# microsoft/ConfigNet

Measured on AMD Instinct MI355X. Metric: train-step images/sec at 256x256 (G+D fwd+bwd), higher is better.
Workload: dtype f32; 1 GPU; ConfigNet second-stage iteration (D + synth-D + latent-D + G + EMA), 256x256, batch 16 per GPU, fp32, Keras-Adam; global_batch=16, resolution=256, latent_dim=145, parallelism=dp1, losses_finite=True

## Files before the change

### confignet_amd/_lib.py

```python
import ctypes
import os

_HERE = os.path.dirname(os.path.abspath(__file__))
LIB_PATH = os.environ.get("CN_LIB") or os.path.join(_HERE, "libconfignet_hip.so")


class CnSumJob(ctypes.Structure):
    _fields_ = [("src", ctypes.c_void_p), ("dst", ctypes.c_void_p), ("count", ctypes.c_longlong), ("parts", ctypes.c_int),
                ("accumulate", ctypes.c_int)]


class CnDepthJob(ctypes.Structure):
    _fields_ = [("a", ctypes.c_void_p), ("b", ctypes.c_void_p), ("c", ctypes.c_void_p), ("m", ctypes.c_int), ("n", ctypes.c_int),
                ("k", ctypes.c_int), ("lda", ctypes.c_int), ("ldb", ctypes.c_int), ("ldc", ctypes.c_int)]


class CnRowsJob(ctypes.Structure):
    _fields_ = [("a", ctypes.c_void_p), ("b", ctypes.c_void_p), ("c", ctypes.c_void_p), ("bias", ctypes.c_void_p), ("mask", ctypes.c_void_p)] + \
               [(n_, ctypes.c_int) for n_ in ("m", "n", "k", "lda", "ldb", "ldc", "tb", "act", "accumulate")] + [("slope", ctypes.c_float)]


class CnGanJob(ctypes.Structure):
    _fields_ = [("s", ctypes.c_void_p), ("out", ctypes.c_void_p), ("gout", ctypes.c_void_p), ("n", ctypes.c_int), ("label", ctypes.c_float)]


class CnConvGeom(ctypes.Structure):
    _fields_ = [(n, ctypes.c_int) for n in (
        "nd", "n", "in_d", "in_h", "in_w", "cin", "out_d", "out_h", "out_w", "cout",
        "k_d", "k_h", "k_w", "s_d", "s_h", "s_w", "dl_d", "dl_h", "dl_w", "p_d", "p_h", "p_w", "up")]


CN_F32, CN_BF16 = 0, 1
CN_U8 = 2
CN_EUNSUPPORTED = -3


class ConfigNetHipError(RuntimeError):
    pass


if not os.path.exists(LIB_PATH):
    raise ImportError(
        "confignet_amd: %s is missing -- build it with `python confignet_amd/build.py` "
        "(or __graft_entry__.build()).  There is no CPU/PyTorch fallback." % LIB_PATH)

lib = ctypes.CDLL(LIB_PATH)

_p = ctypes.c_void_p
_i = ctypes.c_int
_f = ctypes.c_float
_z = ctypes.c_size_t
_G = ctypes.POINTER(CnConvGeom)

SIGNATURES = {
    "cn_version": [],
    "cn_conv_fwd": [_G, _p, _p, _p, _p, _i, _f, _p],
    "cn_conv_fwd_res": [_G, _p, _p, _p, _p, _p, _i, _f, _p],
    "cn_conv_fwd_stats": [_G, _p, _p, _p, _p, _i, _f, _p, _i, _f, _p],
    "cn_scale_columns_segments": [_p, _p, _p, _p, _i, _z, _p],
    "cn_conv_weight_tflip": [_p, _p, _i, _i, _i, _p],
    "cn_conv_dgrad": [_G, _p, _p, _p, _p],
    "cn_conv_dgrad_w": [_G, _p, _p, _p, _p],
    "cn_conv_dgrad_w_res": [_G, _p, _p, _p, _p, _p],
    "cn_bn_fold_bwd_chunks": [],
    "cn_bn_fold_bwd": [_p, _i, _i, _p, _p, _p, _p, _p, _p, _p, _p, _i, _p],
    "cn_conv_wgrad_thin_partials": [],
    "cn_conv_wgrad_thin": [_G, _p, _p, _p, _p, _i, _p],
    "cn_conv_wgrad": [_G, _p, _p, _p, _i, _p],
    "cn_conv_wgrad_workspace_bytes": [_G],
    "cn_conv_wgrad_ws": [_G, _p, _p, _p, _i, _p, _z, _p],
    "cn_conv_wgrad_ws_slabs": [_G, _p, _p, _p, _i, _p, _z, ctypes.POINTER(_i), _p],
    "cn_conv_wgrad_dt_workspace_bytes": [_G, _i, _i, ctypes.POINTER(_z)],
    "cn_conv_wgrad_dt": [_G, _p, _i, _p, _i, _p, _i, _p, _z, ctypes.POINTER(_i), _p],
    "cn_conv_wgrad_plan": [_G, _i, _i, _i, ctypes.c_uint, _i, ctypes.POINTER(ctypes.c_longlong)],
    "cn_conv_wgrad_grouped": [_i, _p, _p, _p, _p, _p, _p, _p, _i, _p, _p],
    "cn_conv_wgrad_grouped_plan": [_i, _p, _i, _p, _p],
    "cn_sum_parts_grouped": [_p, _i, _p],
    "cn_gemm_depth_grouped": [_p, _i, _p],
    "cn_gan_loss_grouped": [_p, _i, _i, _p],
    "cn_gemm_rows_grouped": [_p, _i, _p],
    "cn_gemm_rows_grouped_k": [_p, _i, _p],
    "cn_gemm_rows_grouped_plan": [_p, _i, ctypes.POINTER(_i), _i, ctypes.POINTER(_i)],
    "cn_conv_tune": [_i, _i, ctypes.c_long],
    "cn_conv_fwd_plan": [_G, _i, _i, _i, _i, _i, _i, _i, ctypes.POINTER(ctypes.c_int * 8)],
    "cn_conv_loop_select": [_i, _i, _i, _i],
    "cn_fwd2_col_block": [_i, _i, _i, _i, _i, _i],
    "cn_conv_fwd_dt": [_p, _p, _i, _p, _p, _p, _i, _i, _f, _p],
    "cn_conv_dgrad_dt": [_p, _p, _i, _p, _p, _i, _p],
    "cn_conv_wgrad_c3_partials": [],
    "cn_conv_wgrad_c3": [_p, _p, _p, _i, _p, _p, _i, _p],
    "cn_conv_wino_filter": [_p, _p, _i, _i, _i, _p],
    "cn_conv_fwd_wino": [_i, _i, _i, _i, _i, _p, _p, _p, _p, _i, _f, _p],
    "cn_conv_fwd_wino4": [_i, _i, _i, _i, _i, _p, _p, _p, _p, _i, _f, _p],
    "cn_conv_fwd_wino4_ep": [_i, _i, _i, _i, _i, _p, _p, _p, _p, _i, _f, _i, _p, _p, _p, _p, _i, _f, _p],
    "cn_conv_wino4_filter": [_p, _p, _i, _i, _i, _p],
    "cn_sumpool2": [_p, _p, _i, _i, _i, _i, _i, _i, _i, _p],
    "cn_gemm": [_i, _i, _i, _i, _i, _p, _i, _p, _i, _p, _i, _p, _i, _f, _p],
    "cn_gemm_plan": [_i] * 10 + [ctypes.POINTER(ctypes.c_int * 9)],
    "cn_nc_reduce4": [_p, _p, _i, _i, _i, _f, _i, _i, _p],
    "cn_nc_reduce": [_p, _p, _p, _p, _i, _i, _i, _i, _f, _i, _p],
    "cn_nc_reduce_plan": [_i, _i, _i, _i, _i, _i, ctypes.POINTER(ctypes.c_int * 8)],
    "cn_nc_lin2": [_p, _p, _p, _p, _p, _p, _p, _p, _i, _i, _i, _i, _i, _f, _i, _p],
    "cn_nc_rows_plan": [ctypes.c_longlong, _i, _i, ctypes.POINTER(ctypes.c_int * 2)],
    "cn_norm_coef_fwd": [_i, _p, _p, _p, _p, _p, _p, _p, _p, _i, _i, _i, _f, _p, _i, _p],
    "cn_norm_coef_bwd": [_i, _p, _p, _p, _p, _p, _p, _p, _p, _p, _p, _i, _i, _i, _f, _p],
    "cn_dual_tail_coef_fwd": [_p] * 13 + [_i, _i, _i, _f, _i, _i, _p],
    "cn_dual_tail_coef_bwd": [_p] * 13 + [ctypes.POINTER(ctypes.c_void_p), _i, _i, _i, _f, _i, _i, _p],
    "cn_dual_tail_gx": [_p] * 12 + [_i, _i, _i, _f, _i, _i, _p],
    "cn_dual_tail_gx_tx": [_p] * 18 + [_i, _i, _i, _f, _i, _i, _i, _p],
    "cn_norm_apply": [_i, _i] + [_p] * 13 + [_i, _i, _i, _f, _i, _f, _i, _p],
    "cn_nc_reduce_hxt": [_p, _p, _p, _p, _i, _i, _i, _f, _i, _i, _i, _p],
    "cn_zero": [_p, ctypes.c_size_t, _p],
    "cn_set_deterministic": [_i],
    "cn_get_deterministic": [],
    "cn_det_release_stream": [_p],
    "cn_gemm_acc": [_i, _i, _i, _i, _i, _p, _i, _p, _i, _p, _i, _p],
    "cn_sum_rows_into": [_p, _p, _i, _i, _i, _p],
    "cn_bn_act_bwd": [_p, _p, _p, _p, _p, _p, _p, _p, _i, _i, _i, _i, _i, _i, _p],
    "cn_nc_reduce_dact": [_p, _p, _p, _p, _p, _i, _i, _i, _i, _f, _i, _i, _p],
    "cn_act_fwd": [_p, _p, _z, _i, _f, _i, _p],
    "cn_act_bwd": [_p, _p, _p, _z, _i, _f, _i, _p],
    "cn_act_bwd_bias": [_p, _p, _p, _p, _i, _i, _i, _i, _f, _i, _i, _p],
    "cn_axpby": [_p, _p, _p, _z, _f, _f, _i, _p],
    "cn_mul": [_p, _p, _p, _z, _i, _p],
    "cn_sqdiff_sum": [_p, _p, _p, _z, _f, _i, _p],
    "cn_row_sumsq": [_p, _p, _i, _z, _p],
    "cn_row_scale": [_p, _p, _p, _i, _z, _f, _i, _p],
    "cn_row_scale_diff": [_p, _p, _p, _p, _i, ctypes.c_size_t, _f, _i, _p],
    "cn_tap_bwd": [_p, _p, _p, _p, _p, _i, ctypes.c_size_t, _f, _i, _f, _i, _p],
    "cn_maxpool2_bwd_act": [_p, _p, _p, _p, _f, _p, _i, _i, _i, _i, _i, _i, _p],
    "cn_stream_plan": [_i, _i, ctypes.c_longlong, _z, _i, _i, _i, _i, _i, _i, ctypes.c_uint, _i, ctypes.POINTER(ctypes.c_longlong * 4)],
    "cn_stream_plan_ptrs": [_i, _i, _i, ctypes.c_longlong, _z, _i, _i, _i, _i, _i, _i, ctypes.POINTER(ctypes.c_void_p * 4), _i, ctypes.POINTER(ctypes.c_longlong * 4)],
    "cn_stream_last_plan": [ctypes.POINTER(ctypes.c_longlong * 5)],
    "cn_masked_diff": [_p, _p, _p, _p, _z, _i, _p],
    "cn_maxpool_fwd": [_p, _p, _i, _i, _i, _i, _i, _i, _i, _i, _p],
    "cn_maxpool_bwd": [_p, _p, _p, _i, _i, _i, _i, _i, _i, _i, _i, _p],
    "cn_avgpool3_same": [_p, _p, _i, _i, _i, _i, _i, _p],
    "cn_dwconv3x3_fwd": [_p, _p, _p, _p, _i, _i, _i, _i, _i, _i, _f, _p],
    "cn_image_preprocess": [_p, _i, _p, _i, _i, _i, _i, _i, _i, _f, _f, _p],
    "cn_dwconv3x3_dgrad": [_p, _p, _p, _i, _i, _i, _i, _i, _p],
    "cn_dwconv3x3_wgrad_slices": [_i, _i, _i, _i, _i],
    "cn_dwconv3x3_wgrad": [_p, _p, _p, _i, _i, _i, _i, _i, _i, _p],
    "cn_bn_train_coef": [_p] * 12 + [ctypes.c_longlong, _i, _f, ctypes.c_double, _i, _p],
    "cn_bn_train_apply": [_p, _p, _p, _p, ctypes.c_longlong, _i, _i, _p],
    "cn_bn_train_bwd_slices": [ctypes.c_longlong, _i],
    "cn_chan_slices_plan": [ctypes.c_longlong, _i, _i, ctypes.POINTER(ctypes.c_int * 5)],
    "cn_bn_train_bwd_reduce": [_p] * 6 + [_i, ctypes.c_longlong, _i, _i, _p],
    "cn_bn_train_bwd_apply": [_p] * 8 + [ctypes.c_longlong, _i, _i, _p],
    "cn_chan_affine3_fwd": [_p, _p, _z, ctypes.POINTER(_i), _f, ctypes.POINTER(_f), _p],
    "cn_chan_affine3_bwd": [_p, _p, _z, ctypes.POINTER(_i), _f, _p],
    "cn_gan_loss_fwd": [_p, _p, _i, _f, _p],
    "cn_gan_loss_bwd": [_p, _p, _p, _i, _f, _p],
    "cn_euler_matrix": [_p, _p, _i, _p],
    "cn_euler_matrix_bwd": [_p, _p, _p, _i, _p],
    "cn_rotate3d_fwd": [_p, _p, _p, _i, _i, _i, _p],
    "cn_rotate3d_bwd": [_p, _p, _p, _p, _p, _i, _i, _i, _p],
    "cn_rotate3d_bwd_plan": [_i, _i, _i, _i, ctypes.POINTER(ctypes.c_int * 4)],
    "cn_adam_step": [_p, _p, _p, _p, _p, _z, _p, _f, _f, _f, _f, _p],
    "cn_ema_step": [_p, _p, _z, _f, _p],
    "cn_gather_images_u8": [_p, _p, _p, _p, _i, _i, _i, _i, _p],
    "cn_to_uint8": [_p, _p, _z, _p],
    "cn_hdri_rows_v": [_p, _p, _p, _p, _i, _i, _i, _i, _i, _p],
    "cn_hdri_rows_h": [_p, _p, _p, _p, _p, _p, _p, _i, _i, _i, _i, _i, _i, _p],
    "cn_exp2m1": [_p, _p, _z, _p],
    "cn_warp_affine_u8": [_p] * 6 + [_i] * 6 + [_p],
    "cn_warp_nearest_f32": [_p] * 6 + [_i] * 6 + [_p],
    "cn_eye_mask": [_p, _p, _z, _i] + [_f] * 6 + [_p],
    "cn_spin": [ctypes.c_ulonglong, _p],
    "cn_conv_weight_prep_bf16": [_p, _p, _p, _i, _i, _i, _p],
    "cn_conv_fwd_bf16": [_G, _p, _p, _p, _p, _i, _f, _p],
    "cn_conv_dgrad_bf16": [_G, _p, _p, _p, _p],
    "cn_conv_wgrad_bf16": [_G, _p, _p, _p, _i, _p],
    "cn_cast": [_p, _i, _p, _i, _z, _p],
    "cn_upfold_weights": [_p, _p, _p, _i, ctypes.POINTER(_i), ctypes.POINTER(_i), _i, _i, ctypes.POINTER(_i), ctypes.POINTER(_i), _p],
    "cn_upfold_wgrad": [_p, _p, _i, ctypes.POINTER(_i), ctypes.POINTER(_i), _i, _i, _i, _p],
    "cn_prof_enable": [_i],
    "cn_prof_reset": [],
    "cn_prof_collect": [ctypes.POINTER(_i), ctypes.POINTER(ctypes.c_double), ctypes.POINTER(ctypes.c_double)],
    "cn_prof_collect_by_family": [ctypes.POINTER(_i), ctypes.POINTER(ctypes.c_double), ctypes.POINTER(ctypes.c_double), ctypes.POINTER(ctypes.c_double)],
}

for _name, _args in SIGNATURES.items():
    _fn = getattr(lib, _name)
    _fn.argtypes = _args
    _fn.restype = ctypes.c_int
lib.cn_conv_wgrad_workspace_bytes.restype = ctypes.c_size_t
lib.cn_last_error_string.argtypes = []
lib.cn_last_error_string.restype = ctypes.c_char_p


def check(code, what):
    if code != 0:
        raise ConfigNetHipError("%s failed (%d): %s" % (what, code, lib.cn_last_error_string().decode()))
```

### confignet_amd/csrc/common.h

```cpp
#pragma once
#include <hip/hip_runtime.h>
#include <stdint.h>
#include <stdio.h>
#include "../../include/confignet_hip.h"

void cn_set_error(const char* fmt, ...);

#define CN_CHECK_ARG(cond, ...)            \
    do {                                   \
        if (!(cond)) {                     \
            cn_set_error(__VA_ARGS__);     \
            return CN_EINVAL;              \
        }                                  \
    } while (0)

#define CN_HIP(expr)                                                              \
    do {                                                                          \
        hipError_t e__ = (expr);                                                  \
        if (e__ != hipSuccess) {                                                  \
            cn_set_error("%s failed: %s (%s:%d)", #expr, hipGetErrorString(e__), __FILE__, __LINE__); \
            return CN_EHIP;                                                       \
        }                                                                         \
    } while (0)

#define CN_LAUNCH_CHECK()                                                         \
    do {                                                                          \
        hipError_t e__ = hipGetLastError();                                       \
        if (e__ != hipSuccess) {                                                  \
            cn_set_error("kernel launch failed: %s (%s:%d)", hipGetErrorString(e__), __FILE__, __LINE__); \
            return CN_EHIP;                                                       \
        }                                                                         \
    } while (0)

int cn_zero_async(void* p, size_t bytes, hipStream_t s);

int cn_det();
float* cn_det_ws(hipStream_t s, size_t need_floats);
constexpr size_t CN_DET_WS_FLOATS = (size_t)16 << 20;
int cn_sum_parts(const float* src, float* dst, int parts, long count, int accumulate, float scale, hipStream_t s);

int cn_fwd2(const CnConvGeom* gp, int cfg, int bt, const float* A, const float* B, const float* bias, float* C, long M, int N, int K,
            int act, float slope, int splits, long part_stride, int par, hipStream_t s, const float* res, double x_elems, double w_elems,
            float* stats = nullptr, int stats_mode = 0, float stats_slope = 0.f, int srows = 1, int sper = 1);
void cn_fwd2_tune(int kb, int ns, int np);
void cn_fwd2_grid(int cfg, long M, int N, int par, int splits, int grid[3]);
int cn_igemm_fwd(int cfg, const CnConvGeom& g, bool vec, int par, int splits, const float* x, const float* w, const float* bias, float* y,
                 int act, float slope, hipStream_t s, int bt, long part_stride, const float* res);
void cn_igemm_fwd_grid(int cfg, const CnConvGeom& g, bool vec, int par, int splits, int grid[3]);
int cn_igemm_fwd_thin(const CnConvGeom& g, const float* x, const float* w, const float* bias, float* y, int act, float slope, hipStream_t s);
enum ConvRoute { CN_ROUTE_UP2K4_RGB = 0, CN_ROUTE_S2_IMAGE_DGRAD, CN_ROUTE_S1_IMAGE_DGRAD, CN_ROUTE_THIN_PAR_IGEMM, CN_ROUTE_THIN_COOP,
                 CN_ROUTE_THIN, CN_ROUTE_C3, CN_ROUTE_C7S2, CN_ROUTE_FWD2, CN_ROUTE_IGEMM, CN_ROUTE_UNSUPPORTED };
constexpr int CN_THIN_COOP_PX = 4;
void cn_small_conv(int route, unsigned grid_x, const CnConvGeom& g, bool vec, int par, const void* x, int x_dt, const float* w,
                   const float* bias, void* y, int y_dt, int act, float slope, hipStream_t s);
int cn_fwd2_bf16(const CnConvGeom& g, int cfg, int flip, const void* x, const void* wb, const float* bias, void* y, int act, float slope,
                 int par, hipStream_t s);

enum WgradRoute { CN_WG_C3 = 0, CN_WG_THIN, CN_WG_TINY, CN_WG_WGRAD2, CN_WG_IGEMM, CN_WG_BF16, CN_WG_NONE };
constexpr int CN_C3_WGRAD_TILE = 64, CN_C3_WGRAD_PARTS = 512;
constexpr int CN_THIN_WGRAD_TH = 8, CN_THIN_WGRAD_TW = 32, CN_THIN_WGRAD_PARTS = 512;
struct Wg2Plan {
    int cfg;
    long tiles_x, tiles_y, splits, rows;
};
bool cn_wgrad2_ok(const CnConvGeom& g);
Wg2Plan cn_wgrad2_plan(const CnConvGeom& g, int forced_cfg, long wg_target, bool group = false);
void cn_wgrad2(int cfg, int ns, const CnConvGeom& g, const float* x, const float* gy, float* out, long slab_stride, int rows, int tiles_x,
               int tiles_y, int splits, int accumulate, unsigned grid, hipStream_t s);
constexpr int CN_WG2_GROUP = 24, CN_KERNARG_BYTES = 4096;
struct Wg2Job {
    CnConvGeom g;
    int rows, tiles_x, tiles_y, nsplits, accumulate;
    const float* x;
    const float* gy;
    float* out;
    long slab_stride;
};
struct Wg2Jobs {
    Wg2Job job[CN_WG2_GROUP];
    int blk0[CN_WG2_GROUP + 1];
    int n;
};
static_assert(sizeof(Wg2Jobs) <= CN_KERNARG_BYTES, "the jobs of a grouped launch travel in its kernel arguments");
void cn_wgrad2_grouped(int cfg, const Wg2Jobs& J, unsigned grid, hipStream_t s);
void cn_igemm_wgrad(int cfg, const CnConvGeom& g, const float* x, const float* gy, float* gw, int rows, float* parts, int tx, int ty,
                    int splits, dim3 grid, hipStream_t s);
int cn_tiny_wgrad(const CnConvGeom& g, const float* x, const float* gy, float* gw, int blocks, float* parts, hipStream_t s);
void cn_bf16_wgrad(int cfg, const CnConvGeom& g, const void* x, const void* gy, float* gw, int rows, int tx, int ty, int splits, dim3 grid,
                   hipStream_t s);
int cn_c3_wgrad(const CnConvGeom& g, const float* x, const void* gy, int gy_dt, float* scratch, int tiles_x, int ntiles, int nparts,
                size_t lds, hipStream_t s);
void cn_c3_wgrad_reduce(const float* scratch, float* gw, int nparts, int count, int accumulate, hipStream_t s);
void cn_thin_wgrad(const CnConvGeom& g, const float* x, const float* gy, float* scratch, int nwg, size_t lds, int tiles_y, int tiles_x,
                   int ntiles, hipStream_t s);

enum { CN_FAM_FWD_128x128 = 0, CN_FAM_FWD_128x64, CN_FAM_FWD_64x64, CN_FAM_FWD_128x32, CN_FAM_FWD_128x96, CN_FAM_WGRAD_128x128,
       CN_FAM_WGRAD_128x96, CN_FAM_WGRAD_64x64, CN_FAM_WGRAD_128x32, CN_FAM_WINO, CN_FAM_C3_FWD, CN_FAM_S2_IMAGE_DGRAD,
       CN_FAM_THIN, CN_FAM_C3_WGRAD, CN_FAM_BF16_FWD, CN_FAM_BF16_WGRAD, CN_FAM_WGRAD_256x64, CN_FAM_WGRAD_SLAB_SUM };
void cn_prof_begin(hipStream_t s, double flops, double bytes = 0.0, int family = 31);
void cn_prof_end(hipStream_t s);

__device__ __forceinline__ void divmod_pos(int m, int d, int& q, int& r) {
    if ((d & (d - 1)) == 0) {
        q = m >> (__builtin_ctz(d));
        r = m & (d - 1);
    } else {
        q = m / d;
        r = m - q * d;
    }
}

__device__ __forceinline__ float cn_apply_act(float v, int act, float slope) {
    switch (act) {
        case CN_ACT_LRELU: return v > 0.f ? v : v * slope;
        case CN_ACT_RELU: return v > 0.f ? v : 0.f;
        case CN_ACT_TANH: return tanhf(v);
        default: break;
    }
    if (act == CN_ACT_RELU6) return fminf(fmaxf(v, 0.f), 6.f);
    if (act == CN_ACT_SIGMOID) return __fdividef(1.f, 1.f + __expf(-v));
    return v;
}

__device__ __forceinline__ float act_deriv(float o, int act, float slope) {
    if (act == CN_ACT_LRELU) return o > 0.f ? 1.f : slope;
    if (act == CN_ACT_RELU) return o > 0.f ? 1.f : 0.f;
    if (act == CN_ACT_TANH) return 1.f - o * o;
    return 1.f;
}

static inline int cn_cdiv(long a, long b) { return (int)((a + b - 1) / b); }

int cn_cu_count();
```

### confignet_amd/csrc/conv_dispatch.hip

```cpp
#include "common.h"

#include <algorithm>
#include <vector>

#include "mma_tile.h"
#include "conv_geom.h"

namespace {

int g_tune_cfg = -1;
int g_tune_splits = 0;
long g_tune_wg_blocks = 0;
int g_tune_wg2_ns = 0;
int g_fwd2_sel = -1;
constexpr int g_fwd2_min_nks = 1;
constexpr int g_fwd2_min_c = 48;

struct ConvReq {
    int bt, has_bias, act, has_res, stats_mode, x_dt, y_dt;
};

struct ConvPlan {
    int route = CN_ROUTE_UNSUPPORTED;
    int ret = CN_EUNSUPPORTED;
    int cfg = -1;
    int splits = 1, par = 0;
    bool vec = false;
    bool plain = false;
    int family = -1;
    int srows = 1, sper = 1;
    int grid[3] = {0, 0, 0};
};

int image_route(const CnConvGeom& g, const ConvReq& q) {
    const bool x32 = q.x_dt == CN_F32, y32 = q.y_dt == CN_F32, x16 = q.x_dt == CN_BF16, y16 = q.y_dt == CN_BF16;
    if (x32 && (y32 || y16) && !q.bt && g.nd == 2 && g.cin == 3 && g.dl_h == 1 && g.dl_w == 1 && !g.up && g.cout > 4 && g.cout <= 64) {
        if (g.k_h == 3 && g.k_w == 3 && g.s_h == g.s_w && (g.s_h == 1 || g.s_h == 2)) return CN_ROUTE_C3;
        if (g.k_h == 7 && g.k_w == 7 && g.s_h == 2 && g.s_w == 2 && !q.has_res) return CN_ROUTE_C7S2;
    }
    if (y32 && g.nd == 2 && g.k_h == 3 && g.k_w == 3 && g.s_h == 1 && g.s_w == 1 && !g.up && g.cout == 3 && !q.has_bias &&
        q.act == CN_ACT_NONE && g.p_h >= 0 && g.p_h <= 2 && g.p_w >= 0 && g.p_w <= 2) {
        if ((x32 || x16) && g.dl_h == 2 && g.dl_w == 2 && g.cin == 48 && g.out_h <= 2 * g.in_h && g.out_w <= 2 * g.in_w) return CN_ROUTE_S2_IMAGE_DGRAD;
        if (x32 && g.dl_h == 1 && g.dl_w == 1 && g.cin == 64) return CN_ROUTE_S1_IMAGE_DGRAD;
    }
    return CN_ROUTE_UNSUPPORTED;
}

ConvPlan plan_conv_fwd(const CnConvGeom& g, const ConvReq& q) {
    ConvPlan p;
    const long M = (long)g.n * g.out_d * g.out_h * g.out_w;
    const bool res = q.has_res != 0, stats = q.stats_mode != 0;
    const int bt = q.bt;
    auto small = [&p](int route, int family, long grid_x) {
        p.route = route;
        p.ret = CN_OK;
        p.family = family;
        p.grid[0] = (int)grid_x; p.grid[1] = p.grid[2] = 1;
        return p;
    };
    auto refuse = [&p](int code) {
        p.ret = code;
        return p;
    };
    const int img = image_route(g, q);
    const long img_grid = img == CN_ROUTE_S2_IMAGE_DGRAD ? (long)g.n * cn_cdiv(g.in_h, 8) * cn_cdiv(g.in_w, 32)
                                                         : (long)g.n * cn_cdiv(g.out_h, 8) * cn_cdiv(g.out_w, 32);
    const int img_family = img == CN_ROUTE_C3 || img == CN_ROUTE_C7S2 ? CN_FAM_C3_FWD : CN_FAM_S2_IMAGE_DGRAD;
    if (q.x_dt != CN_F32 || q.y_dt != CN_F32)
        return img != CN_ROUTE_UNSUPPORTED ? small(img, img_family, img_grid) : p;
    if ((res || stats) && (g.cout <= 4 || g.cin == 3 || g.cout % 4 != 0)) return p;
    if (stats && (bt || cn_det() || g.cin % BK != 0)) return p;
    if (bt && (g.cout <= 4 || g.cin % BK != 0 || g.cout % 4 != 0)) return p;
    if (g.cout <= 4) {
        p.vec = g.cin % 4 == 0;
        p.par = parity_ordered(g);
        const size_t lds = sizeof(float) * 4 * (size_t)g.k_d * g.k_h * g.k_w * g.cin;
        if (lds > 64 * 1024) {
            cn_set_error("thin conv: filter of %zu bytes does not fit the LDS stage", lds);
            return refuse(CN_EINVAL);
        }
        const int T = g.k_d * g.k_h * g.k_w, CL = g.cin / 4;
        const bool dl1 = g.dl_d * g.dl_h * g.dl_w == 1;
        if (g.nd == 2 && g.up == 1 && g.k_h == 4 && g.k_w == 4 && g.s_h == 1 && g.s_w == 1 && g.dl_h == 1 && g.dl_w == 1 &&
            g.cout == 3 && g.cin == 32 && g.p_h == 1 && g.p_w == 1 && g.out_h <= 2 * g.in_h && g.out_w <= 2 * g.in_w)
            return small(CN_ROUTE_UP2K4_RGB, CN_FAM_THIN, (long)g.n * cn_cdiv(g.in_h, 8) * cn_cdiv(g.in_w, 16));
        if (img != CN_ROUTE_UNSUPPORTED) return small(img, img_family, img_grid);
        if (p.par && g.cin % BK == 0 && q.act == CN_ACT_NONE && T <= CN_MAX_MASKED_TAPS) return small(CN_ROUTE_THIN_PAR_IGEMM, CN_FAM_FWD_128x32, cn_cdiv(M, 128));
        if (p.vec && g.cout == 3 && CL >= 5 && CL <= 16 && T <= 32 && (p.par || dl1) && g.dl_d * g.dl_h * g.dl_w <= 8)
            return small(CN_ROUTE_THIN_COOP, -1, cn_cdiv(M, (256 / (CL <= 8 ? 8 : 16)) * CN_THIN_COOP_PX));
        return small(CN_ROUTE_THIN, -1, cn_cdiv(M, 256));
    }
    if (img != CN_ROUTE_UNSUPPORTED) return small(img, img_family, img_grid);
    if (g.cout % 4 != 0) {
        cn_set_error("cout=%d: implicit-GEMM path needs cout %% 4 == 0", g.cout);
        return refuse(CN_EINVAL);
    }
    const bool vec = g.cin % BK == 0;
    if (vec && (long)g.k_d * g.k_h * g.k_w > CN_MAX_MASKED_TAPS) {
        cn_set_error("%d taps: the vectorised implicit-GEMM gather takes at most %d", g.k_d * g.k_h * g.k_w, CN_MAX_MASKED_TAPS);
        return refuse(CN_EUNSUPPORTED);
    }
    const int par = parity_ordered(g) && vec;
    const long t128 = (long)cn_cdiv(M, 128) * cn_cdiv(g.cout, 128);
    const long t128x64 = (long)cn_cdiv(M, 128) * cn_cdiv(g.cout, 64);
    int cfg;
    long tiles;
    if (g.cout <= 32) { cfg = 3; tiles = (long)cn_cdiv(M, 128) * cn_cdiv(g.cout, 32); }
    else if (g.cout > 64 && t128 >= 512) { cfg = 0; tiles = t128; }
    else if (t128x64 >= 512) { cfg = 1; tiles = t128x64; }
    else { cfg = 2; tiles = (long)cn_cdiv(M, 64) * cn_cdiv(g.cout, 64); }
    if (g.cout % 96 == 0 && g.cout % 128 != 0 &&
        (long)cn_cdiv(M, 128) * (g.cout / 96) >= (g.cout == 96 ? 256 : 384)) {
        cfg = 4;
        tiles = (long)cn_cdiv(M, 128) * (g.cout / 96);
    }
    int splits = 1;
    const bool par_small = par && cfg == 2;
    const long nks_total = vec ? (long)g.k_d * g.k_h * g.k_w * (g.cin / BK) : 0;
    if (cfg == 0 && vec && !par && nks_total <= 8) { cfg = 1; tiles = t128x64; }
    const bool short_full = !par && tiles >= 256 && nks_total < 64;
    if (vec && tiles < (par_small ? 1024 : 512) && !short_full) {
        long nks = nks_total;
        if (par) nks /= (long)g.dl_d * g.dl_h * g.dl_w;
        long want = ((par_small ? 3072 : 1024) + tiles - 1) / tiles;
        if (want > 16) want = 16;
        const long min_steps = par_small ? 8 : 16;
        if (want > nks / min_steps) want = nks / min_steps;
        if (want > 1) splits = (int)want;
    }
    const bool n32 = g.cout == 32 && g.cin >= 32;
    const bool fwd2_takes = g_fwd2_sel != 0 && vec && nks_total > g_fwd2_min_nks && ((g.cin >= g_fwd2_min_c && g.cout >= g_fwd2_min_c) || n32) &&
                            g.dl_d <= 2 && g.dl_h <= 2 && g.dl_w <= 2 && (double)g.n * g.in_d * g.in_h * g.in_w * g.cin < 5.3e8 &&
                            (double)g.k_d * g.k_h * g.k_w * g.cin * g.cout < 5.3e8;
    if (fwd2_takes) {
        const int T = g.k_d * g.k_h * g.k_w;
        const long Me = (par && T == 1) ? M / ((long)g.dl_d * g.dl_h * g.dl_w) : M;
        long nks = nks_total;
        if (par) nks /= (long)g.dl_d * g.dl_h * g.dl_w;
        splits = 1;
        const bool par_balanced = par && g.k_d % g.dl_d == 0 && g.k_h % g.dl_h == 0 && g.k_w % g.dl_w == 0;
        if (n32) {
            cfg = 3;
            tiles = cn_cdiv(M, 128);
        } else if (par && T > 1 && !par_balanced) {
            cfg = 2;
            tiles = (long)cn_cdiv(M, 64) * cn_cdiv(g.cout, 64);
            if (g.cout % 96 == 0 && g.cout % 64 != 0 && (long)cn_cdiv(M, 128) * (g.cout / 96) >= 512) {
                cfg = 4;
                tiles = (long)cn_cdiv(M, 128) * (g.cout / 96);
            }
            if (cfg == 2 && tiles < 1024) {
                long want = (1536 + tiles / 2) / tiles;
                if (want > 16) want = 16;
                if (want > nks / 8) want = nks / 8;
                if (want > 1) splits = (int)want;
            }
        } else {
            struct Cand { int cfg, bm, bn; double step_us; };
            const Cand cands[2] = {{2, 64, 64, 0.265}, {4, 128, 96, 0.68}};
            double best = 0.0;
            bool have = false;
            for (const Cand& c : cands) {
                if (c.cfg == 4 && (g.cout % 96 != 0 || g.cout % 64 == 0 || (long)cn_cdiv(Me, 128) * (g.cout / 96) < 256)) continue;
                const long tl = (long)cn_cdiv(Me, c.bm) * cn_cdiv(g.cout, c.bn);
                const long smax = nks / 8 > 1 ? (nks / 8 > 16 ? 16 : nks / 8) : 1;
                for (long s_ = 1; s_ <= smax; ++s_) {
                    const double waves = (double)cn_cdiv(tl * s_, cn_cu_count());
                    double t = 10.0 + waves * (double)cn_cdiv(nks, s_) * c.step_us * (waves == 1.0 ? 1.06 : 1.0);
                    if (s_ > 1) t += 9.0 + (double)s_ * (double)M * g.cout * 4.0 / 6.0e6;
                    if (s_ > 1 && (res || stats)) t += 5.0 + 2.0 * (double)M * g.cout * 4.0 / 3.0e6;
                    if (!have || t < best) { have = true; best = t; cfg = c.cfg; tiles = tl; splits = (int)s_; }
                }
            }
        }
    }
    if (g_tune_cfg >= 0) cfg = g_tune_cfg;
    if (g_tune_splits > 0) splits = g_tune_splits;
    if (res && splits > 1) return p;
    if (stats) {
        const int qd = par ? g.out_d / g.dl_d : g.out_d, qh = par ? g.out_h / g.dl_h : g.out_h, qw = par ? g.out_w / g.dl_w : g.out_w;
        p.srows = qd * qh * qw;
        p.sper = par ? g.n * p.srows : (int)M;
        if (!fwd2_takes || splits > 1 || cfg == 3 || p.srows % (cfg == 2 ? 64 : 128) != 0) return p;
    }
    if (cn_det() && splits > 1) {
        const long cap = (long)(CN_DET_WS_FLOATS / ((size_t)M * g.cout));
        if (splits > cap) splits = (int)cap;
        if (splits <= 1 || !vec) splits = 1;
    }
    p.route = fwd2_takes && (cfg != 3 || n32) && cfg >= 0 && cfg <= 4 ? CN_ROUTE_FWD2 : CN_ROUTE_IGEMM;
    if (stats && p.route != CN_ROUTE_FWD2) return refuse(CN_EINVAL);
    p.ret = CN_OK;
    p.cfg = cfg;
    p.splits = splits;
    p.par = par;
    p.vec = vec;
    p.family = cfg == 0 ? CN_FAM_FWD_128x128 : cfg == 1 ? CN_FAM_FWD_128x64 : cfg == 3 ? CN_FAM_FWD_128x32 : cfg == 4 ? CN_FAM_FWD_128x96 : CN_FAM_FWD_64x64;
    if (p.route == CN_ROUTE_FWD2) {
        p.plain = !par && g.k_d * g.k_h * g.k_w == 1 && g.s_d == 1 && g.s_h == 1 && g.s_w == 1 && g.dl_d == 1 && g.dl_h == 1 &&
                  g.dl_w == 1 && !g.up && g.p_d == 0 && g.p_h == 0 && g.p_w == 0 && g.out_d == g.in_d && g.out_h == g.in_h &&
                  g.out_w == g.in_w;
        cn_fwd2_grid(cfg, M, g.cout, par, splits, p.grid);
    } else {
        cn_igemm_fwd_grid(cfg, g, vec, par, splits, p.grid);
    }
    return p;
}

int run_conv_fwd(const ConvPlan& p, const CnConvGeom& g, const ConvReq& q, const void* x, const float* w, const float* bias,
                 const float* res, void* y, float slope, float* stats, float stats_slope, hipStream_t s) {
    if (p.route == CN_ROUTE_UNSUPPORTED) return p.ret;
    const long M = (long)g.n * g.out_d * g.out_h * g.out_w;
    const int splits = p.splits;
    float* parts = nullptr;
    if (cn_det() && splits > 1) {
        parts = cn_det_ws(s, (size_t)splits * M * g.cout);
        if (!parts) return CN_EINVAL;
    }
    const int kact = splits > 1 ? CN_ACT_NONE : q.act;
    if (splits > 1 && !parts) {
        if (int ez__ = cn_zero_async(y, sizeof(float) * M * g.cout, s)) return ez__;
    }
    const long part_stride = parts ? (long)M * g.cout : 0;
    float* const out = parts ? parts : (float*)y;
    if (p.family >= 0) cn_prof_begin(s, conv_flops(g), conv_bytes(g, q.x_dt == CN_BF16 ? 2.0 : 4.0, q.y_dt == CN_BF16 ? 2.0 : 4.0), p.family);
    int e = CN_OK;
    switch (p.route) {
        case CN_ROUTE_FWD2: {
            const double xe = (double)g.n * g.in_d * g.in_h * g.in_w * g.cin, we = (double)g.k_d * g.k_h * g.k_w * g.cin * g.cout;
            e = cn_fwd2(p.plain ? nullptr : &g, p.cfg, q.bt, (const float*)x, w, bias, out, M, g.cout, g.cin, kact, slope, splits, part_stride,
                        p.plain ? 0 : p.par, s, res, xe, we, stats, q.stats_mode, stats_slope, p.srows, p.sper);
            break;
        }
        case CN_ROUTE_IGEMM:
            e = cn_igemm_fwd(p.cfg, g, p.vec, p.par, splits, (const float*)x, w, bias, out, kact, slope, s, q.bt, part_stride, res);
            break;
        case CN_ROUTE_THIN_PAR_IGEMM:
            e = cn_igemm_fwd_thin(g, (const float*)x, w, bias, out, kact, slope, s);
            break;
        default:
            cn_small_conv(p.route, (unsigned)p.grid[0], g, p.vec, p.par, x, q.x_dt, w, bias, y, q.y_dt, kact, slope, s);
            break;
    }
    if (p.family >= 0) cn_prof_end(s);
    CN_CHECK_ARG(e != CN_EUNSUPPORTED, "convolution plan (route %d, tile %d) refused by its kernel", p.route, p.cfg);
    if (e != CN_OK) return e;
    CN_LAUNCH_CHECK();
    if (parts) e = cn_sum_parts(parts, (float*)y, splits, (long)M * g.cout, 0, 1.f, s);
    if (e == CN_OK && splits > 1 && q.act != CN_ACT_NONE) e = cn_act_fwd(y, y, (size_t)M * g.cout, q.act, slope, CN_F32, s);
    return e;
}

int conv_fwd(const CnConvGeom* gp, const ConvReq& q, const void* x, const float* w, const float* bias, const float* res, void* y,
             float slope, float* stats, float stats_slope, void* stream) {
    if (int e = check_geom(gp)) return e;
    CN_CHECK_ARG(x && w && y, "NULL tensor");
    return run_conv_fwd(plan_conv_fwd(*gp, q), *gp, q, x, w, bias, res, y, slope, stats, stats_slope, (hipStream_t)stream);
}

}

extern "C" int cn_conv_fwd(const CnConvGeom* gp, const float* x, const float* w, const float* bias, float* y, int act,
                           float slope, void* stream) {
    return conv_fwd(gp, ConvReq{0, bias != nullptr, act, 0, 0, CN_F32, CN_F32}, x, w, bias, nullptr, y, slope, nullptr, 0.f, stream);
}

extern "C" int cn_conv_fwd_stats(const CnConvGeom* gp, const float* x, const float* w, const float* bias, float* y, int act,
                                 float slope, float* stats, int stats_mode, float stats_slope, void* stream) {
    CN_CHECK_ARG(stats && (stats_mode == 1 || stats_mode == 2), "cn_conv_fwd_stats: stats buffer and mode 1 / 2");
    CN_CHECK_ARG(stats_mode == 1 || act == CN_ACT_NONE, "cn_conv_fwd_stats: mode 2 takes the statistics of the pre-activation output");
    return conv_fwd(gp, ConvReq{0, bias != nullptr, act, 0, stats_mode, CN_F32, CN_F32}, x, w, bias, nullptr, y, slope, stats, stats_slope, stream);
}

extern "C" int cn_conv_fwd_res(const CnConvGeom* gp, const float* x, const float* w, const float* bias, const float* res, float* y,
                               int act, float slope, void* stream) {
    CN_CHECK_ARG(res, "cn_conv_fwd_res: res is NULL");
    return conv_fwd(gp, ConvReq{0, bias != nullptr, act, 1, 0, CN_F32, CN_F32}, x, w, bias, res, y, slope, nullptr, 0.f, stream);
}

extern "C" int cn_conv_fwd_dt(const CnConvGeom* gp, const void* x, int x_dt, const float* w, const float* bias, void* y, int y_dt,
                              int act, float slope, void* stream) {
    if (int e = check_geom(gp)) return e;
    CN_CHECK_ARG(x && w && y, "NULL tensor");
    if (x_dt == CN_F32 && y_dt == CN_F32) return CN_EUNSUPPORTED;
    const ConvReq q{0, bias != nullptr, act, 0, 0, x_dt, y_dt};
    return run_conv_fwd(plan_conv_fwd(*gp, q), *gp, q, x, w, bias, nullptr, y, slope, nullptr, 0.f, (hipStream_t)stream);
}

extern "C" int cn_conv_dgrad(const CnConvGeom* gp, const float* gy, const float* w_tflip, float* gu, void* stream) {
    if (int e = check_geom(gp)) return e;
    CN_CHECK_ARG(gp->dl_d == 1 && gp->dl_h == 1 && gp->dl_w == 1, "dgrad of a dilated-input geometry is not defined here");
    const CnConvGeom d = dgrad_geom(*gp);
    return cn_conv_fwd(&d, gy, w_tflip, nullptr, gu, CN_ACT_NONE, 0.f, stream);
}

extern "C" int cn_conv_dgrad_dt(const CnConvGeom* gp, const void* gy, int gy_dt, const float* w_tflip, void* gu, int gu_dt,
                                void* stream) {
    if (int e = check_geom(gp)) return e;
    if (gp->dl_d != 1 || gp->dl_h != 1 || gp->dl_w != 1) return CN_EUNSUPPORTED;
    const CnConvGeom d = dgrad_geom(*gp);
    return cn_conv_fwd_dt(&d, gy, gy_dt, w_tflip, nullptr, gu, gu_dt, CN_ACT_NONE, 0.f, stream);
}

extern "C" int cn_conv_dgrad_w(const CnConvGeom* gp, const float* gy, const float* w, float* gu, void* stream) {
    if (int e = check_geom(gp)) return e;
    if (gp->dl_d != 1 || gp->dl_h != 1 || gp->dl_w != 1) return CN_EUNSUPPORTED;
    const CnConvGeom d = dgrad_geom(*gp);
    return conv_fwd(&d, ConvReq{1, 0, CN_ACT_NONE, 0, 0, CN_F32, CN_F32}, gy, w, nullptr, nullptr, gu, 0.f, nullptr, 0.f, stream);
}

extern "C" int cn_conv_dgrad_w_res(const CnConvGeom* gp, const float* gy, const float* w, const float* res, float* gu, void* stream) {
    if (int e = check_geom(gp)) return e;
    CN_CHECK_ARG(res, "cn_conv_dgrad_w_res: res is NULL");
    if (gp->dl_d != 1 || gp->dl_h != 1 || gp->dl_w != 1 || gp->up) return CN_EUNSUPPORTED;
    if (gp->s_d != 1 || gp->s_h != 1 || gp->s_w != 1) return CN_EUNSUPPORTED;
    const CnConvGeom d = dgrad_geom(*gp);
    return conv_fwd(&d, ConvReq{1, 0, CN_ACT_NONE, 1, 0, CN_F32, CN_F32}, gy, w, nullptr, res, gu, 0.f, nullptr, 0.f, stream);
}

extern "C" int cn_conv_fwd_plan(const CnConvGeom* gp, int bt, int has_bias, int act, int has_res, int stats_mode, int x_dt, int y_dt,
                                int out[8]) {
    if (int e = check_geom(gp)) return e;
    CN_CHECK_ARG(out, "cn_conv_fwd_plan: out is NULL");
    const ConvPlan p = plan_conv_fwd(*gp, ConvReq{bt, has_bias, act, has_res, stats_mode, x_dt, y_dt});
    const int v[8] = {p.route, p.cfg, p.splits, p.par, p.family, p.grid[0], p.grid[1], p.grid[2]};
    for (int i = 0; i < 8; ++i) out[i] = v[i];
    return p.ret;
}

namespace {

struct WgradReq {
    int x_dt, gy_dt;
    bool caller_slabs;
    unsigned routes;
    bool det = cn_det() != 0;
};
constexpr unsigned wg_bit(int r) { return 1u << r; }
constexpr unsigned WG_ATOMIC = wg_bit(CN_WG_TINY) | wg_bit(CN_WG_IGEMM), WG_FP32_GEMM = wg_bit(CN_WG_WGRAD2) | WG_ATOMIC, WG_ALL = ~0u;

enum { WG_SUM_NONE = 0, WG_SUM_PARTS, WG_SUM_C3, WG_SUM_CALLER };

struct WgradPlan {
    int route = CN_WG_NONE;
    int ret = CN_EUNSUPPORTED;
    int cfg = -1;
    int stages = 0;
    long splits = 1, rows = 0;
    int tx = 0, ty = 0;
    int family = -1;
    int grid[3] = {0, 0, 0};
    size_t lds = 0;
    size_t ws_floats = 0;
    size_t det_floats = 0;
    bool zero = false;
    int sum = WG_SUM_NONE;
};

struct WgTile { int bm, bn; };
WgTile wgrad_tile(int cfg) { return cfg == 3 ? WgTile{128, 32} : cfg == 4 ? WgTile{128, 96} : cfg == 0 ? WgTile{128, 128} : cfg == 5 ? WgTile{256, 64} : WgTile{64, 64}; }
int wgrad_family(int cfg) {
    return cfg == 3 ? CN_FAM_WGRAD_128x32 : cfg == 4 ? CN_FAM_WGRAD_128x96 : cfg == 0 ? CN_FAM_WGRAD_128x128 : cfg == 5 ? CN_FAM_WGRAD_256x64 : CN_FAM_WGRAD_64x64;
}

void sliced_grid(const CnConvGeom& g, WgTile t, WgradPlan& p) {
    const long Ktot = (long)g.k_d * g.k_h * g.k_w * g.cin;
    const int gx = cn_cdiv(Ktot, t.bm), gy = cn_cdiv(g.cout, t.bn);
    p.grid[0] = gx; p.grid[1] = gy; p.grid[2] = (int)p.splits;
    if ((long)gx * gy > 1 && p.splits >= 16) {
        p.tx = gx; p.ty = gy;
        p.grid[0] = cn_cdiv(p.splits, 8) * 8 * gx * gy; p.grid[1] = p.grid[2] = 1;
    }
}

bool igemm_wgrad_slices(const CnConvGeom& g, WgTile t, long wg_target, bool det, WgradPlan& p) {
    const long M = (long)g.n * g.out_d * g.out_h * g.out_w;
    const long Ktot = (long)g.k_d * g.k_h * g.k_w * g.cin;
    const long tiles = (long)cn_cdiv(Ktot, t.bm) * cn_cdiv(g.cout, t.bn);
    const long wg_blocks = wg_target > 0 ? wg_target : 2048;
    long splits = (wg_blocks + tiles - 1) / tiles;
    if (det) {
        const long cap = (long)(CN_DET_WS_FLOATS / ((size_t)Ktot * g.cout));
        if (cap < 1) {
            cn_set_error("deterministic filter gradient: %ld x %d filter does not fit the workspace", Ktot, g.cout);
            return false;
        }
        if (splits > cap) splits = cap;
    }
    long rows = (M + splits - 1) / splits;
    if (rows < 256) rows = 256;
    rows = (rows + BK - 1) / BK * BK;
    p.rows = rows;
    p.splits = (M + rows - 1) / rows;
    return true;
}

void bf16_wgrad_slices(const CnConvGeom& g, WgTile t, WgradPlan& p) {
    constexpr long KS = 32, min_rows = 512;
    const long M = (long)g.n * g.out_d * g.out_h * g.out_w;
    const long Ktot = (long)g.k_d * g.k_h * g.k_w * g.cin;
    const long tiles = (long)cn_cdiv(Ktot, t.bm) * cn_cdiv(g.cout, t.bn);
    const long per_cu = t.bm * t.bn >= 128 * 128 ? 3 : t.bm * t.bn >= 128 * 96 ? 4 : 5;
    const long target = 256 * per_cu * (t.bn >= 96 ? 1 : 2);
    long splits = target / tiles;
    if (splits > M / min_rows) splits = M / min_rows;
    const long fill = std::min<long>(M / 256, (256 + tiles - 1) / tiles);
    if (splits < fill) splits = fill;
    if (splits >= 16) splits &= ~7L;
    if (splits < 1) splits = 1;
    long rows = (M + splits - 1) / splits;
    if (rows < 256) rows = std::min<long>(256, (M + KS - 1) / KS * KS);
    rows = (rows + KS - 1) / KS * KS;
    p.rows = rows;
    p.splits = (M + rows - 1) / rows;
}

WgradPlan plan_conv_wgrad(const CnConvGeom& g, const WgradReq& q) {
    WgradPlan p;
    const long M = (long)g.n * g.out_d * g.out_h * g.out_w;
    const long Ktot = (long)g.k_d * g.k_h * g.k_w * g.cin;
    const size_t count = (size_t)Ktot * g.cout;
    const bool x32 = q.x_dt == CN_F32, y32 = q.gy_dt == CN_F32, x16 = q.x_dt == CN_BF16, y16 = q.gy_dt == CN_BF16;
    auto may = [&q](int route) { return (q.routes & wg_bit(route)) != 0; };
    auto take = [&p](int route, int family) {
        p.route = route;
        p.ret = CN_OK;
        p.family = family;
    };
    if (may(CN_WG_C3) && x32 && (y32 || y16) && g.nd == 2 && g.cin == 3 && g.k_h == 3 && g.k_w == 3 && g.k_d == 1 && g.s_h == g.s_w &&
        (g.s_h == 1 || g.s_h == 2) && g.dl_h == 1 && g.dl_w == 1 && g.up == 0 && g.cout <= 64 && g.cout >= 4 && g.cout % 4 == 0) {
        take(CN_WG_C3, CN_FAM_C3_WGRAD);
        p.tx = cn_cdiv(g.out_w, CN_C3_WGRAD_TILE);
        p.grid[0] = CN_C3_WGRAD_PARTS; p.grid[1] = p.grid[2] = 1;
        const int pw = CN_C3_WGRAD_TILE * g.s_h + 2, gpitch = (g.cout + 3) & ~3;
        p.lds = sizeof(float) * 4 * (size_t)(3 * pw * 3 + CN_C3_WGRAD_TILE * gpitch);
        if (p.lds < sizeof(float) * 4 * 2 * 16 * 64) p.lds = sizeof(float) * 4 * 2 * 16 * 64;
        p.ws_floats = CN_C3_WGRAD_PARTS * count;
        p.sum = WG_SUM_C3;
        return p;
    }
    const int T = g.k_h * g.k_w;
    if (may(CN_WG_THIN) && x32 && y32 && g.nd == 2 && g.cout <= 4 && g.cin % 4 == 0 && g.cin >= 8 && g.cin <= 64 && g.s_h == 1 && g.s_w == 1 &&
        g.dl_h == 1 && g.dl_w == 1 && T <= 16 && T * (g.cin / 4) <= 256) {
        const int PH0 = ((CN_THIN_WGRAD_TH + g.k_h - 1) >> g.up) + 2, PW0 = ((CN_THIN_WGRAD_TW + g.k_w - 1) >> g.up) + 2;
        size_t lds = sizeof(float) * ((size_t)PH0 * PW0 * g.cin + CN_THIN_WGRAD_TH * CN_THIN_WGRAD_TW * 4);
        const size_t red = sizeof(float) * 256 * 4 * g.cout;
        if (lds < red) lds = red;
        if (lds <= 64 * 1024) {
            take(CN_WG_THIN, -1);
            p.ty = cn_cdiv(g.out_h, CN_THIN_WGRAD_TH); p.tx = cn_cdiv(g.out_w, CN_THIN_WGRAD_TW);
            const int ntiles = g.n * p.ty * p.tx;
            p.grid[0] = ntiles < CN_THIN_WGRAD_PARTS ? ntiles : CN_THIN_WGRAD_PARTS; p.grid[1] = p.grid[2] = 1;
            p.lds = lds;
            p.ws_floats = CN_THIN_WGRAD_PARTS * count;
            p.sum = WG_SUM_PARTS;
            return p;
        }
    }
    if (x16 && y16) {
        if (!may(CN_WG_BF16) || g.cin % 8 || g.cout % 8) return p;
        take(CN_WG_BF16, CN_FAM_BF16_WGRAD);
        p.cfg = wgrad_tile_cfg(g);
        bf16_wgrad_slices(g, wgrad_tile(p.cfg), p);
        sliced_grid(g, wgrad_tile(p.cfg), p);
        p.zero = true;
        return p;
    }
    if (!x32 || !y32) return p;
    if (may(CN_WG_WGRAD2) && cn_wgrad2_ok(g) && Ktot >= 64) {
        const int t = g_tune_cfg;
        const Wg2Plan w = cn_wgrad2_plan(g, t == 0 || t == 2 || t == 3 || t == 4 || t == 5 ? t : -1, g_tune_wg_blocks);
        take(CN_WG_WGRAD2, wgrad_family(w.cfg));
        p.cfg = w.cfg;
        p.stages = w.cfg == 3 || g_tune_wg2_ns == 3 ? 3 : 4;
        p.splits = w.splits; p.rows = w.rows;
        p.tx = (int)w.tiles_x; p.ty = (int)w.tiles_y;
        p.grid[0] = (int)((w.splits >= 8 ? cn_cdiv(w.splits, 8) * 8 : w.splits) * w.tiles_x * w.tiles_y); p.grid[1] = p.grid[2] = 1;
        if (w.splits > 1) {
            p.ws_floats = (size_t)w.splits * count;
            p.sum = q.caller_slabs ? WG_SUM_CALLER : WG_SUM_PARTS;
        }
        return p;
    }
    if (may(CN_WG_TINY) && Ktot <= 4 && g.cout <= 4 && g.k_d * g.k_h * g.k_w == 1 && g.s_h == 1 && g.s_w == 1 && g.s_d == 1 && !g.up &&
        g.p_h == 0 && g.p_w == 0 && g.p_d == 0) {
        take(CN_WG_TINY, -1);
        p.grid[0] = cn_cdiv(M, 256) > 1024 ? 1024 : cn_cdiv(M, 256); p.grid[1] = p.grid[2] = 1;
        p.zero = true;
        if (q.det) {
            p.det_floats = (size_t)p.grid[0] * 16;
            p.sum = WG_SUM_PARTS;
        }
        return p;
    }
    if (!may(CN_WG_IGEMM)) return p;
    const int cfg = wgrad_tile_cfg(g);
    if (!igemm_wgrad_slices(g, wgrad_tile(cfg), g_tune_wg_blocks, q.det, p)) {
        p.ret = CN_EINVAL;
        return p;
    }
    take(CN_WG_IGEMM, wgrad_family(cfg));
    p.cfg = cfg;
    sliced_grid(g, wgrad_tile(cfg), p);
    p.zero = true;
    if (q.det) {
        p.det_floats = (size_t)p.splits * count;
        p.sum = WG_SUM_PARTS;
    }
    return p;
}

int sum_conv_wgrad(const WgradPlan& p, int nparts, long count, int mode, float* gw, const float* ws, const float* det, int* parts_out,
                   hipStream_t s) {
    CN_LAUNCH_CHECK();
    const int add = mode != CN_WGRAD_WRITE;
    if (p.sum == WG_SUM_PARTS) return cn_sum_parts(det ? det : ws, gw, nparts, count, det ? 1 : add, 1.f, s);
    if (p.sum == WG_SUM_C3) {
        cn_c3_wgrad_reduce(ws, gw, nparts, (int)count, mode == CN_WGRAD_ADD, s);
        CN_LAUNCH_CHECK();
    }
    if (p.sum == WG_SUM_CALLER) *parts_out = nparts;
    return CN_OK;
}

int run_conv_wgrad(const WgradPlan& p, const CnConvGeom& g, const WgradReq& q, const void* x, const void* gy, float* gw, int mode,
                   float* ws, size_t ws_bytes, int* parts_out, hipStream_t s) {
    if (parts_out) *parts_out = 0;
    if (p.route == CN_WG_NONE) return p.ret;
    CN_CHECK_ARG(mode == CN_WGRAD_WRITE || mode == CN_WGRAD_ADD || mode == CN_WGRAD_ZEROED, "filter gradient: mode %d", mode);
    CN_CHECK_ARG(p.ws_floats == 0 || (ws && ws_bytes >= sizeof(float) * p.ws_floats), "filter gradient: workspace of %zu bytes, %zu needed",
                 ws ? ws_bytes : (size_t)0, sizeof(float) * p.ws_floats);
    CN_CHECK_ARG(p.sum != WG_SUM_CALLER || parts_out, "filter gradient: slabs left to a caller that takes none");
    CN_CHECK_ARG(p.route != CN_WG_BF16 || (((uintptr_t)x | (uintptr_t)gy) & 15) == 0, "bf16 convolution needs 16-byte aligned tensors");
    const long count = (long)g.k_d * g.k_h * g.k_w * g.cin * g.cout;
    const int add = mode != CN_WGRAD_WRITE;
    float* det = nullptr;
    if (p.det_floats) {
        det = cn_det_ws(s, p.det_floats);
        if (!det) return CN_EINVAL;
    }
    if (p.zero && !add) {
        if (int ez__ = cn_zero_async(gw, sizeof(float) * count, s)) return ez__;
    }
    if (p.family >= 0)
        cn_prof_begin(s, p.route == CN_WG_C3 ? 2.0 * 27.0 * g.cout * (double)g.n * g.out_h * g.out_w : conv_flops(g),
                      conv_bytes(g, q.x_dt == CN_BF16 ? 2.0 : 4.0, q.gy_dt == CN_BF16 ? 2.0 : 4.0, 4.0), p.family);
    const dim3 grid(p.grid[0], p.grid[1], p.grid[2]);
    int nparts = (int)p.splits, e = CN_OK;
    switch (p.route) {
        case CN_WG_C3:
            e = cn_c3_wgrad(g, (const float*)x, gy, q.gy_dt, ws, p.tx, g.n * g.out_h * p.tx, nparts = p.grid[0], p.lds, s);
            break;
        case CN_WG_THIN:
            cn_thin_wgrad(g, (const float*)x, (const float*)gy, ws, nparts = p.grid[0], p.lds, p.ty, p.tx, g.n * p.ty * p.tx, s);
            break;
        case CN_WG_TINY:
            nparts = cn_tiny_wgrad(g, (const float*)x, (const float*)gy, gw, p.grid[0], det, s);
            break;
        case CN_WG_WGRAD2:
            cn_wgrad2(p.cfg, p.stages, g, (const float*)x, (const float*)gy, p.splits > 1 ? ws : gw, p.splits > 1 ? count : 0, (int)p.rows,
                      p.tx, p.ty, (int)p.splits, add, grid.x, s);
            break;
        case CN_WG_IGEMM:
            cn_igemm_wgrad(p.cfg, g, (const float*)x, (const float*)gy, gw, (int)p.rows, det, p.tx, p.ty, (int)p.splits, grid, s);
            break;
        default:
            cn_bf16_wgrad(p.cfg, g, x, gy, gw, (int)p.rows, p.tx, p.ty, (int)p.splits, grid, s);
            break;
    }
    const bool sum_in_bracket = p.route != CN_WG_C3;
    if (p.family >= 0 && !sum_in_bracket) cn_prof_end(s);
    if (e == CN_OK) e = sum_conv_wgrad(p, nparts, count, mode, gw, ws, det, parts_out, s);
    if (p.family >= 0 && sum_in_bracket) cn_prof_end(s);
    return e;
}

int conv_wgrad(const CnConvGeom* gp, const WgradReq& q, const void* x, const void* gy, float* gw, int mode, void* ws, size_t ws_bytes,
               int* parts, void* stream) {
    if (int e = check_geom(gp)) return e;
    CN_CHECK_ARG(x && gy && gw, "NULL tensor");
    return run_conv_wgrad(plan_conv_wgrad(*gp, q), *gp, q, x, gy, gw, mode, (float*)ws, ws_bytes, parts, (hipStream_t)stream);
}

}

extern "C" int cn_conv_wgrad(const CnConvGeom* gp, const float* x, const float* gy, float* gw, int accumulate, void* stream) {
    return conv_wgrad(gp, WgradReq{CN_F32, CN_F32, false, WG_ATOMIC}, x, gy, gw, accumulate ? CN_WGRAD_ADD : CN_WGRAD_WRITE, nullptr, 0, nullptr, stream);
}

extern "C" size_t cn_conv_wgrad_workspace_bytes(const CnConvGeom* gp) {
    if (!gp || check_geom(gp) != CN_OK) return 0;
    return sizeof(float) * plan_conv_wgrad(*gp, WgradReq{CN_F32, CN_F32, false, WG_FP32_GEMM}).ws_floats;
}

extern "C" int cn_conv_wgrad_ws(const CnConvGeom* gp, const float* x, const float* gy, float* gw, int accumulate, void* workspace,
                                size_t workspace_bytes, void* stream) {
    return conv_wgrad(gp, WgradReq{CN_F32, CN_F32, false, WG_FP32_GEMM}, x, gy, gw, accumulate ? CN_WGRAD_ADD : CN_WGRAD_WRITE, workspace,
                      workspace_bytes, nullptr, stream);
}

extern "C" int cn_conv_wgrad_ws_slabs(const CnConvGeom* gp, const float* x, const float* gy, float* gw, int accumulate, void* workspace,
                                      size_t workspace_bytes, int* parts, void* stream) {
    CN_CHECK_ARG(parts, "cn_conv_wgrad_ws_slabs: parts is NULL");
    return conv_wgrad(gp, WgradReq{CN_F32, CN_F32, true, WG_FP32_GEMM}, x, gy, gw, accumulate ? CN_WGRAD_ADD : CN_WGRAD_WRITE, workspace,
                      workspace_bytes, parts, stream);
}

extern "C" int cn_conv_wgrad_bf16(const CnConvGeom* gp, const uint16_t* x, const uint16_t* gy, float* gw, int accumulate,
                                  void* stream) {
    return conv_wgrad(gp, WgradReq{CN_BF16, CN_BF16, false, wg_bit(CN_WG_BF16)}, x, gy, gw, accumulate ? CN_WGRAD_ADD : CN_WGRAD_WRITE, nullptr, 0,
                      nullptr, stream);
}

extern "C" int cn_conv_wgrad_c3_partials(void) { return CN_C3_WGRAD_PARTS; }

extern "C" int cn_conv_wgrad_c3(const CnConvGeom* gp, const float* x, const void* gy, int gy_dt, float* scratch, float* gw,
                                int accumulate, void* stream) {
    CN_CHECK_ARG(gp && x && gy && scratch && gw && (gy_dt == CN_F32 || gy_dt == CN_BF16), "conv_wgrad_c3: bad args");
    return conv_wgrad(gp, WgradReq{CN_F32, gy_dt, false, wg_bit(CN_WG_C3)}, x, gy, gw, accumulate ? CN_WGRAD_ADD : CN_WGRAD_WRITE, scratch, SIZE_MAX,
                      nullptr, stream);
}

extern "C" int cn_conv_wgrad_thin_partials(void) { return CN_THIN_WGRAD_PARTS; }

extern "C" int cn_conv_wgrad_thin(const CnConvGeom* gp, const float* x, const float* gy, float* scratch, float* gw, int accumulate,
                                  void* stream) {
    CN_CHECK_ARG(scratch, "conv_wgrad_thin: NULL");
// ... 184 lines not shown
```

### confignet_amd/csrc/fwd2.hip

```cpp
#include "common.h"
#include "mma_tile.h"
#include "conv_geom.h"
#include "typed.h"

#ifndef FWD2_ABLATE
#define FWD2_ABLATE 0
#endif

namespace {

typedef __attribute__((address_space(3))) float lds_float;
typedef float f4 __attribute__((ext_vector_type(4)));
typedef float f2 __attribute__((ext_vector_type(2)));
typedef __bf16 f2_bf16x8 __attribute__((ext_vector_type(8)));

template <int N>
__device__ __forceinline__ void f2_wait_vmcnt() {
    __builtin_amdgcn_s_waitcnt((N & 15) | ((N >> 4) << 14) | (7 << 4) | (15 << 8));
}

template <int N>
__device__ __forceinline__ void f2_wait_lgkm() {
    asm volatile("s_waitcnt lgkmcnt(%0)" : : "n"(N));
    __builtin_amdgcn_sched_barrier(0);
}

template <int N>
struct F2Int {
    static constexpr int value = N;
};

template <int I, int N, class F>
__device__ __forceinline__ void f2_static_for_impl(F&& f) {
    if constexpr (I < N) {
        f(F2Int<I>{});
        f2_static_for_impl<I + 1, N>(f);
    }
}

template <int N, class F>
__device__ __forceinline__ void f2_static_for(F&& f) {
    f2_static_for_impl<0, N>(f);
}

template <int WM, int WN, int TM, int TN, bool BT, bool GATHER, int KB, int NS, int NP, bool BF, int CB = 32>
__device__ __forceinline__ void fwd2_body(const CnConvGeom& g, const float* __restrict__ A, const float* __restrict__ B,
                                          const float* __restrict__ bias, float* __restrict__ C, int M, int N, int K,
                                          int act, float slope, int ntm, int ntn, long part_stride, int par,
                                          const float* __restrict__ res, unsigned a_bytes, unsigned b_bytes, int flip,
                                          float* __restrict__ stats, int stats_mode, float stats_slope, int srows, int sper) {
    static_assert(!BF || BT, "bf16: both operands are K-contiguous rows");
    constexpr int ES = BF ? 2 : 4;
    constexpr int KE = KB * 4 / ES;
    static_assert(WM * WN == 4, "4 waves per workgroup");
    static_assert(KB == 16 || KB == 32, "stage depth");
    static_assert(CB == 32 || (CB == 16 && BT && !BF && KB == 16 && NP == 0), "16-wide MFMA blocks: the fp32 B^T form");
    constexpr int KP = KB / 4;
    constexpr int RPI = 64 / KP;
    constexpr int FSH = KP == 4 ? 2 : 1;
    constexpr int G = CB == 16 ? 1 : KB / 8;
    constexpr int BM = CB * WM * TM, BN = CB * WN * TN;
    constexpr int NL = NP > 0 ? NP : 4;
    constexpr int IA = BM / RPI, JA = IA / NL;
    static_assert(IA % NL == 0, "A pieces divide over the loading waves");
    static_assert(NP == 0 || KB == 16, "loader waves: 16-deep stages");
    constexpr int IB = BT ? BN / RPI : KB * BN / 256;
    constexpr int JB = (IB + NL - 1) / NL;
    constexpr int LPW = JA + JB;
    constexpr int SA = BM * KB, SB = CB == 16 ? IB * 256 : JB * NL * 256;
    constexpr int SX = CB == 16 && IB < JB * NL ? 256 : 0;
    constexpr bool B2 = !BT && TN == 1 && BN == 64;
    constexpr int NB = BT ? TN : B2 ? 2 : 4 * (TN == 2 ? 1 : TN);
    constexpr int RD = TM + NB;
    static_assert((NS - 1) * LPW < 64, "vmcnt range");
    __shared__ __attribute__((aligned(1024))) float SM[NS * (SA + SB) + SX];
    __shared__ int rowmap[GATHER ? BM : 1];

    const int tid = threadIdx.x, lane = tid & 63, l31 = lane & (CB - 1), half = lane / CB;
    const int wave = __builtin_amdgcn_readfirstlane(tid >> 6);
    const bool loader = NP == 0 || wave >= 4, worker = wave < 4;
    const int lw = NP > 0 ? wave - 4 : wave;
    const int wm = (wave & 3) / WN, wn = (wave & 3) % WN;
    int bx, by;
    if (GATHER && par) {
        divmod_pos((int)blockIdx.x, ntm, by, bx);
        if (by >= ntn) return;
    } else {
        const int id = blockIdx.x, xcd = id & 7, j = id >> 3;
        const int nt = ntm * ntn, q = nt >> 3, r = nt & 7;
        if (j >= q + (xcd < r ? 1 : 0)) return;
        const int u = (xcd < r ? xcd * (q + 1) : r * (q + 1) + (xcd - r) * q) + j;
        divmod_pos(u, ntn, bx, by);
    }
    const int m0 = bx * BM, n0 = by * BN;
    const int T = GATHER ? g.k_d * g.k_h * g.k_w : 1;
    const int cpb = K / KE;
    unsigned long long tapmask = T >= 64 ? ~0ull : ((1ull << T) - 1ull);
    if (GATHER && par) {
        int c0, c1;
        par_row(g, m0, M, c0);
        par_row(g, min(m0 + BM, M) - 1, M, c1);
        if (c0 == c1) tapmask = par_tap_mask(g, c0);
    }
    const int nks_all = (GATHER ? __popcll(tapmask) : 1) * cpb;
    const int per_z = (nks_all + gridDim.z - 1) / gridDim.z;
    const int ks_beg = blockIdx.z * per_z, ks_end = min(nks_all, ks_beg + per_z);
    const int nks = max(ks_end - ks_beg, 0);

    constexpr int AR = CB == 16 ? 4 : 16;
    typedef float acc_t __attribute__((ext_vector_type(AR)));
    acc_t acc[TM][TN];
#pragma unroll
    for (int i = 0; i < TM; ++i)
#pragma unroll
        for (int j = 0; j < TN; ++j)
#pragma unroll
            for (int r = 0; r < AR; ++r) acc[i][j][r] = 0.f;

    const __amdgpu_buffer_rsrc_t ares = __builtin_amdgcn_make_buffer_rsrc(const_cast<float*>(A), 0, (int)a_bytes, 0x00020000);
    const __amdgpu_buffer_rsrc_t bres = __builtin_amdgcn_make_buffer_rsrc(const_cast<float*>(B), 0, (int)b_bytes, 0x00020000);
    constexpr unsigned OOB = 0x80000000u;

    RowInfo ri[JA];
    int a_base[JA];
    const int a_piece = 16 * ((lane % KP) ^ ((((lw & 1) * RPI + lane / KP) >> FSH) & (KP - 1)));
#pragma unroll
    for (int j = 0; j < JA; ++j) {
        const int r = (lw + NL * j) * RPI + lane / KP;
        if (!loader) {
            ri[j] = RowInfo{};
            a_base[j] = -1;
        } else if (GATHER) {
            int mrow = m0 + r, cls;
            if (par) mrow = par_row(g, mrow, M, cls);
            ri[j] = decode_row(g, mrow, M);
            if (lane % KP == 0) rowmap[r] = ri[j].ok ? mrow : -1;
            a_base[j] = -1;
        } else {
            a_base[j] = m0 + r < M ? (m0 + r) * K : -1;
        }
    }
    int b_off[JB];
    int b_krow[JB];
#pragma unroll
    for (int j = 0; j < JB; ++j) {
        const int I = lw + NL * j;
        if (BT) {
            const int n = n0 + I * RPI + lane / KP;
            b_off[j] = (I < IB && n < N) ? n * K * ES + a_piece : -1;
            b_krow[j] = 0;
        } else {
            const int idx = I * 64 + lane, col = n0 + 4 * (idx % (BN / 4));
            b_krow[j] = idx / (BN / 4);
            b_off[j] = (I < IB && col < N) ? col : -1;
        }
    }
    if (GATHER) __syncthreads();

    int ld_left = nks;
    int ld_tap = -1, ld_c0 = (ks_beg - (ks_beg / cpb) * cpb) * KE;
    if (GATHER)
        for (int o = ks_beg / cpb; o >= 0; --o) ld_tap += __ffsll((long long)(tapmask >> (ld_tap + 1)));
    else
        ld_tap = 0;
    unsigned a_vo[JA], b_vo[JB];
    int a_so = 0, b_so = 0;
    const int sh_d = g.dl_d - 1, sh_h = g.dl_h - 1, sh_w = g.dl_w - 1;
    const int ext_d = g.in_d << g.up, ext_h = g.in_h << g.up, ext_w = g.in_w << g.up;
    auto retap = [&]() __attribute__((always_inline)) {
        if (GATHER) {
            int kd, kh, kw;
            tap_decode(g, ld_tap, kd, kh, kw);
#pragma unroll
            for (int j = 0; j < JA; ++j) {
                const int vd = ri[j].vd + kd, vh = ri[j].vh + kh, vw = ri[j].vw + kw;
                const int qd = vd >> sh_d, qh = vh >> sh_h, qw = vw >> sh_w;
                const bool ok = ri[j].ok & ((vd | vh | vw) >= 0) & (((vd & sh_d) | (vh & sh_h) | (vw & sh_w)) == 0) &
                                (qd < ext_d) & (qh < ext_h) & (qw < ext_w);
                const int off = (((ri[j].nbase + (qd >> g.up)) * g.in_h + (qh >> g.up)) * g.in_w + (qw >> g.up)) * g.cin;
                a_vo[j] = ok ? (unsigned)(off * ES + a_piece) : OOB;
            }
        }
    };
    auto set_so = [&]() __attribute__((always_inline)) {
        a_so = ld_c0 * ES;
        b_so = BT ? ((flip ? T - 1 - ld_tap : ld_tap) * N * K + ld_c0) * ES : (ld_tap * K + ld_c0) * N * 4;
    };
#pragma unroll
    for (int j = 0; j < JA; ++j) a_vo[j] = (!GATHER && a_base[j] >= 0) ? (unsigned)(a_base[j] * ES + a_piece) : OOB;
#pragma unroll
    for (int j = 0; j < JB; ++j) b_vo[j] = b_off[j] >= 0 ? (BT ? (unsigned)b_off[j] : (unsigned)(b_krow[j] * N + b_off[j]) * 4u) : OOB;
    retap();
    set_so();
    auto issue_piece = [&](int stage, int p) __attribute__((always_inline)) {
        if (p < JA)
            __builtin_amdgcn_raw_ptr_buffer_load_lds(ares, (lds_float*)(SM + stage * SA + (lw + NL * p) * 256), 16, a_vo[p], a_so, 0, 0);
        else if (CB == 16 && lw + NL * (p - JA) >= IB)
            __builtin_amdgcn_raw_ptr_buffer_load_lds(bres, (lds_float*)(SM + NS * (SA + SB)), 16, b_vo[p - JA], b_so, 0, 0);
        else
            __builtin_amdgcn_raw_ptr_buffer_load_lds(bres, (lds_float*)(SM + NS * SA + stage * SB + (lw + NL * (p - JA)) * 256), 16,
                                                     b_vo[p - JA], b_so, 0, 0);
    };
    auto advance = [&]() __attribute__((always_inline)) {
        if (--ld_left > 0) {
            ld_c0 += KE;
            if (ld_c0 == K) {
                ld_c0 = 0;
                if (GATHER) {
                    ld_tap += __ffsll((long long)(tapmask >> (ld_tap + 1)));
                    retap();
                }
            }
            set_so();
        }
    };

    const unsigned lds0 = (unsigned)(unsigned long long)(lds_float*)SM;
    const unsigned fsw = (unsigned)((l31 >> FSH) & (KP - 1));
    const unsigned a_rd = lds0 + 4u * (unsigned)((wm * CB * TM + l31) * KB) + 16u * ((unsigned)half ^ fsw);
    const unsigned bt_rd = lds0 + 4u * (unsigned)(NS * SA + (wn * CB * TN + l31) * KB) + 16u * ((unsigned)half ^ fsw);
    const unsigned bn_rd = lds0 + 4u * (unsigned)(NS * SA + (4 * half) * BN + wn * 32 * TN + TN * l31);
    f4 av[2][TM];
    f4 btv[2][BT ? TN : 1];
    float bnv[2][BT ? 1 : 4][TN];
    unsigned ap_cur = 0, bp_cur = 0;
    auto read_base = [&](int stage, int gq) __attribute__((always_inline)) {
        ap_cur = (a_rd + 4u * (unsigned)(stage * SA)) ^ (32u * (unsigned)gq);
        bp_cur = BT ? (bt_rd + 4u * (unsigned)(stage * SB)) ^ (32u * (unsigned)gq) : bn_rd + 4u * (unsigned)(stage * SB + 8 * gq * BN);
    };
    auto read_op = [&](auto rc, int set) __attribute__((always_inline)) {
        constexpr int r = decltype(rc)::value;
        (void)av; (void)btv; (void)bnv; (void)ap_cur; (void)bp_cur;
        if (FWD2_ABLATE & 4) return;
        if constexpr (r < TM) {
            asm volatile("ds_read_b128 %0, %1 offset:%2" : "=v"(av[set][r]) : "v"(ap_cur), "n"(4 * CB * KB * r));
        } else if constexpr (BT) {
            constexpr int j = r - TM;
            asm volatile("ds_read_b128 %0, %1 offset:%2" : "=v"(btv[set][BT ? j : 0]) : "v"(bp_cur), "n"(4 * CB * KB * j));
        } else if constexpr (B2) {
            constexpr int q = 2 * (r - TM);
            f2 v;
            asm volatile("ds_read2_b32 %0, %1 offset0:%2 offset1:%3" : "=v"(v) : "v"(bp_cur), "n"(BN * q), "n"(BN * (q + 1)));
            bnv[set][BT ? 0 : q][0] = v.x;
            bnv[set][BT ? 0 : q + 1][0] = v.y;
        } else if constexpr (TN == 2) {
            constexpr int q = r - TM;
            f2 v;
            asm volatile("ds_read_b64 %0, %1 offset:%2" : "=v"(v) : "v"(bp_cur), "n"(4 * BN * q));
            bnv[set][BT ? 0 : q][0] = v.x;
            bnv[set][BT ? 0 : q][TN - 1] = v.y;
        } else {
            constexpr int q = (r - TM) / TN, j = (r - TM) % TN;
            asm volatile("ds_read_b32 %0, %1 offset:%2" : "=v"(bnv[set][BT ? 0 : q][j]) : "v"(bp_cur), "n"(4 * BN * q + 4 * j));
        }
    };
    constexpr int NM = (BF ? 1 : 4) * TM * TN;
    auto mfma_one = [&](auto mc, int set) __attribute__((always_inline)) {
        constexpr int m = decltype(mc)::value, q = m / (TM * TN), i = (m % (TM * TN)) / TN, j = m % TN;
        if (FWD2_ABLATE & 1) return;
        if constexpr (BF) {
            (void)q;
            union { f4 f; f2_bf16x8 h; } ua, ub;
            ua.f = av[set][i];
            ub.f = btv[set][BT ? j : 0];
            acc[i][j] = __builtin_amdgcn_mfma_f32_32x32x16_bf16(ua.h, ub.h, acc[i][j], 0, 0, 0);
        } else if constexpr (CB == 16) {
            acc[i][j] = __builtin_amdgcn_mfma_f32_16x16x4f32(av[set][i][q], btv[set][BT ? j : 0][q], acc[i][j], 0, 0, 0);
        } else {
            const float a = av[set][i][q];
            const float b = BT ? btv[set][BT ? j : 0][q] : bnv[set][BT ? 0 : q][j];
            acc[i][j] = __builtin_amdgcn_mfma_f32_32x32x2f32(a, b, acc[i][j], 0, 0, 0);
        }
    };

    if (NP > 0 && !worker) {
        if (nks > 0) {
#pragma unroll 1
            for (int s = 0; s < NS; ++s) {
#pragma unroll
                for (int p = 0; p < LPW; ++p) issue_piece(s, p);
                advance();
            }
            f2_wait_vmcnt<(NS - 1) * LPW>();
            __builtin_amdgcn_s_barrier();
            int st = 0;
#pragma unroll 1
            for (int t = 0; t < nks; ++t) {
                f2_wait_vmcnt<(NS - 2) * LPW>();
                __builtin_amdgcn_s_barrier();
                __builtin_amdgcn_sched_barrier(0);
#pragma unroll
                for (int p = 0; p < LPW; ++p) issue_piece(st, p);
                advance();
                st = st + 1 == NS ? 0 : st + 1;
            }
            f2_wait_vmcnt<0>();
        }
        if (!BF) return;
    }
    if (nks > 0 && worker) {
        if (NP == 0) {
#pragma unroll 1
            for (int s = 0; s < NS; ++s) {
#pragma unroll
                for (int p = 0; p < LPW; ++p) issue_piece(s, p);
                advance();
            }
            f2_wait_vmcnt<(NS - 1) * LPW>();
        }
        __builtin_amdgcn_s_barrier();
        __builtin_amdgcn_sched_barrier(0);
        read_base(0, 0);
        f2_static_for<RD>([&](auto rc) __attribute__((always_inline)) { read_op(rc, 0); });
        int st = 0;
        if constexpr (CB == 16) {
            constexpr int BAR = TM * TN;
            constexpr int P0 = NM - 2 - NM / 4, P1 = NM - 1;
            static_assert(LPW == 2 && BAR + RD <= P0, "slot layout of the 16-wide step");
            auto step = [&](auto sc, int stage, int stage_next) __attribute__((always_inline)) {
                constexpr int set = decltype(sc)::value;
                f2_wait_lgkm<0>();
                f2_static_for<NM>([&](auto mc) __attribute__((always_inline)) {
                    constexpr int m = decltype(mc)::value;
                    if constexpr (m == BAR) {
                        if (!(FWD2_ABLATE & 2)) f2_wait_vmcnt<(NS - 2) * LPW>();
                        __builtin_amdgcn_s_barrier();
                        __builtin_amdgcn_sched_barrier(0);
                        read_base(stage_next, 0);
                    }
                    mfma_one(mc, set);
                    __builtin_amdgcn_sched_barrier(0);
                    if constexpr (m >= BAR && m < BAR + RD) read_op(F2Int<m - BAR>{}, set ^ 1);
                    if constexpr (m == P0 || m == P1) {
                        if (!(FWD2_ABLATE & 2)) {
                            issue_piece(stage, m == P0 ? 0 : 1);
                            if (m == P1) advance();
                        }
                    }
                    __builtin_amdgcn_sched_barrier(0);
                });
            };
            for (int t = 0; t < nks; t += 2) {
                int st_next = st + 1 == NS ? 0 : st + 1;
                step(F2Int<0>{}, st, st_next);
                st = st_next;
                if (t + 1 == nks) break;
                st_next = st + 1 == NS ? 0 : st + 1;
                step(F2Int<1>{}, st, st_next);
                st = st_next;
            }
        }
        if constexpr (CB == 32)
        for (int t = 0; t < nks; ++t) {
            const int st_next = st + 1 == NS ? 0 : st + 1;
            f2_wait_lgkm<0>();
#pragma unroll
            for (int gq = 0; gq + 1 < G; ++gq) {
                read_base(st, gq + 1);
                f2_static_for<NM>([&](auto mc) __attribute__((always_inline)) {
                    constexpr int m = decltype(mc)::value;
                    constexpr int NSL = NM > 1 ? NM / 2 : 1;
                    mfma_one(mc, gq & 1);
                    __builtin_amdgcn_sched_barrier(0);
                    f2_static_for<RD>([&](auto rc) __attribute__((always_inline)) {
                        constexpr int r = decltype(rc)::value;
                        if constexpr (m < NSL && r >= (m * RD + NSL - 1) / NSL && r < ((m + 1) * RD + NSL - 1) / NSL) read_op(rc, (gq + 1) & 1);
                    });
                    __builtin_amdgcn_sched_barrier(0);
                });
                if (gq + 2 < G) f2_wait_lgkm<0>();
            }
            f2_wait_lgkm<0>();
            if (NP == 0 && !(FWD2_ABLATE & 2)) f2_wait_vmcnt<(NS - 2) * LPW>();
            __builtin_amdgcn_s_barrier();
            __builtin_amdgcn_sched_barrier(0);
            read_base(st_next, 0);
            f2_static_for<NM>([&](auto mc) __attribute__((always_inline)) {
                constexpr int m = decltype(mc)::value;
                constexpr int NSL = NM > 1 ? NM / 2 : 1;
                mfma_one(mc, (G - 1) & 1);
                __builtin_amdgcn_sched_barrier(0);
                f2_static_for<RD>([&](auto rc) __attribute__((always_inline)) {
                    constexpr int r = decltype(rc)::value;
                    if constexpr (m < NSL && r >= (m * RD + NSL - 1) / NSL && r < ((m + 1) * RD + NSL - 1) / NSL) read_op(rc, G & 1);
                });
                f2_static_for<LPW>([&](auto pc) __attribute__((always_inline)) {
                    constexpr int pp = decltype(pc)::value;
                    constexpr int slot_ = LPW <= NM - NSL ? NM - LPW + pp : NSL + pp * (NM - NSL) / LPW;
                    constexpr int slot = slot_ < NM ? slot_ : NM - 1;
                    if constexpr (slot == m && NP == 0) {
                        if (!(FWD2_ABLATE & 2)) {
                            issue_piece(st, pp);
                            if (pp == LPW - 1) advance();
                        }
                    }
                });
                __builtin_amdgcn_sched_barrier(0);
            });
            st = st_next;
        }
        f2_wait_lgkm<0>();
        if (NP == 0) f2_wait_vmcnt<0>();
    }


    if constexpr (BF) {
        constexpr int LDC = BN + 8;
        static_assert(BM * LDC * 2 <= NS * (SA + SB) * 4, "output tile fits the operand stages");
        bf16_t* const Cs = reinterpret_cast<bf16_t*>(SM);
        bf16_t* const Y = reinterpret_cast<bf16_t*>(C);
        __syncthreads();
        if (worker) {
#pragma unroll
            for (int j = 0; j < TN; ++j) {
                const int ct = wn * 32 * TN + 32 * j + l31, col = n0 + ct;
                const float bv = (bias && col < N) ? bias[col] : 0.f;
#pragma unroll
                for (int i = 0; i < TM; ++i)
#pragma unroll
                    for (int r = 0; r < 16; ++r)
                        Cs[(wm * 32 * TM + 32 * i + 4 * half + (r & 3) + 8 * (r >> 2)) * LDC + ct] =
                            f32_to_bf16(cn_apply_act(acc[i][j][r] + bv, act, slope));
            }
        }
        __syncthreads();
        constexpr int NPC = BN / 8;
        for (int idx = tid; idx < BM * NPC; idx += 256 + 64 * NP) {
            const int row = idx / NPC, pc = idx - row * NPC;
            const int orow = GATHER ? rowmap[row] : (m0 + row < M ? m0 + row : -1), col = n0 + pc * 8;
            if (orow >= 0 && col < N)
                *reinterpret_cast<uint4*>(Y + (long)orow * N + col) = *reinterpret_cast<const uint4*>(Cs + row * LDC + pc * 8);
        }
        return;
    }
    if constexpr (CB == 16) {
        const bool split16 = gridDim.z > 1;
        static_assert(WN == 1, "a wave owns whole rows of the tile");
        constexpr int LDC = BN + 4, C4 = BN / 4;
        static_assert(BM * LDC <= NS * (SA + SB) && (16 * TM * C4) % 64 == 0, "the tile fits the operand stages");
        __syncthreads();
        float* const Cs = SM + wm * 16 * TM * LDC;
#pragma unroll
        for (int i = 0; i < TM; ++i)
#pragma unroll
            for (int j = 0; j < TN; ++j) {
                const int col = n0 + 16 * j + l31;
                const float bv = (bias && blockIdx.z == 0 && col < N) ? bias[col] : 0.f;
#pragma unroll
                for (int r = 0; r < 4; ++r) Cs[(16 * i + 4 * half + r) * LDC + 16 * j + l31] = acc[i][j][r] + bv;
            }
        __builtin_amdgcn_wave_barrier();
#pragma unroll
        for (int k = 0; k < 16 * TM * C4 / 64; ++k) {
            const int f = lane + 64 * k, rr = f / C4, c4 = f - rr * C4;
            const int lrow = wm * 16 * TM + rr, col = n0 + 4 * c4;
            const int row = GATHER ? rowmap[lrow] : m0 + lrow;
            if (row < 0 || row >= M || col >= N) continue;
            f4 v = *reinterpret_cast<const f4*>(Cs + rr * LDC + 4 * c4);
            float* dst = C + (long)row * N + col;
            if (part_stride) *reinterpret_cast<f4*>(dst + (long)blockIdx.z * part_stride) = v;
            else if (split16) {
#pragma unroll
                for (int e = 0; e < 4; ++e) unsafeAtomicAdd(dst + e, v[e]);
            } else {
                if (res) v += *reinterpret_cast<const f4*>(res + (long)row * N + col);
#pragma unroll
                for (int e = 0; e < 4; ++e) v[e] = cn_apply_act(v[e], act, slope);
                *reinterpret_cast<f4*>(dst) = v;
            }
        }
        return;
    }
    const bool split = gridDim.z > 1;
    float sacc[TN][4];
#pragma unroll
    for (int j = 0; j < TN; ++j)
#pragma unroll
        for (int k = 0; k < 4; ++k) sacc[j][k] = 0.f;
    auto stat = [&](int j, float v, float a) __attribute__((always_inline)) {
        if (stats_mode == 1) {
            sacc[j][0] += a;
            sacc[j][1] += a * a;
        } else {
            const float l = v > 0.f ? v : v * stats_slope;
            sacc[j][0] += v;
            sacc[j][1] += v * v;
            sacc[j][2] += l;
            sacc[j][3] += l * l;
        }
    };
#pragma unroll
    for (int i = 0; i < TM; ++i)
#pragma unroll
        for (int r = 0; r < 16; ++r) {
            const int lrow = wm * 32 * TM + 32 * i + 4 * half + (r & 3) + 8 * (r >> 2);
            const int row = GATHER ? rowmap[lrow] : m0 + lrow;
            if (row < 0 || row >= M) continue;
            if (!BT && TN == 2) {
                const int col = n0 + wn * 64 + 2 * l31;
                if (col >= N) continue;
                float v0 = acc[i][0][r], v1 = acc[i][TN - 1][r];
                if (bias && blockIdx.z == 0) { v0 += bias[col]; v1 += bias[col + 1]; }
                float* dst = C + (long)row * N + col;
                if (part_stride) *reinterpret_cast<f2*>(dst + (long)blockIdx.z * part_stride) = f2{v0, v1};
                else if (split) { unsafeAtomicAdd(dst, v0); unsafeAtomicAdd(dst + 1, v1); }
                else {
                    if (res) { const f2 rv = *reinterpret_cast<const f2*>(res + (long)row * N + col); v0 += rv.x; v1 += rv.y; }
                    const float a0 = cn_apply_act(v0, act, slope), a1 = cn_apply_act(v1, act, slope);
                    *reinterpret_cast<f2*>(dst) = f2{a0, a1};
                    if (stats) { stat(0, v0, a0); stat(TN - 1, v1, a1); }
                }
            } else {
#pragma unroll
                for (int j = 0; j < TN; ++j) {
                    const int col = n0 + wn * 32 * TN + (BT ? 32 * j + l31 : TN * l31 + j);
                    if (col >= N) continue;
                    const float v = acc[i][j][r] + ((bias && blockIdx.z == 0) ? bias[col] : 0.f);
                    float* dst = C + (long)row * N + col;
                    if (part_stride) dst[(long)blockIdx.z * part_stride] = v;
                    else if (split) unsafeAtomicAdd(dst, v);
                    else {
                        const float vr = res ? v + res[(long)row * N + col] : v, a = cn_apply_act(vr, act, slope);
                        *dst = a;
                        if (stats) stat(j, vr, a);
                    }
                }
            }
        }
    if (stats && !split && !part_stride) {
        const int sample = (m0 - (m0 / sper) * sper) / srows;
        const int nsamp = sper / srows;
        const int nk = stats_mode == 1 ? 2 : 4;
#pragma unroll
        for (int j = 0; j < TN; ++j) {
            const int col = n0 + wn * 32 * TN + (BT ? 32 * j + l31 : TN * l31 + j);
#pragma unroll
            for (int k = 0; k < 4; ++k) {
                if (k >= nk) break;
                const float t = sacc[j][k] + __shfl_xor(sacc[j][k], 32);
                if (half == 0 && col < N) unsafeAtomicAdd(stats + ((long)k * nsamp + sample) * N + col, t);
            }
        }
    }
}

template <int WM, int WN, int TM, int TN, bool BT, bool GATHER, int KB, int NS, int NP, bool BF>
__global__ __launch_bounds__(256 + 64 * NP) void fwd2_kernel(CnConvGeom g, const float* __restrict__ A, const float* __restrict__ B,
                                                   const float* __restrict__ bias, float* __restrict__ C, int M, int N, int K,
                                                   int act, float slope, int ntm, int ntn, long part_stride, int par,
                                                   const float* __restrict__ res, unsigned a_bytes, unsigned b_bytes, int flip,
                                                   float* __restrict__ stats, int stats_mode, float stats_slope, int srows, int sper) {
    fwd2_body<WM, WN, TM, TN, BT, GATHER, KB, NS, NP, BF>(g, A, B, bias, C, M, N, K, act, slope, ntm, ntn, part_stride, par, res, a_bytes,
                                                          b_bytes, flip, stats, stats_mode, stats_slope, srows, sper);
}

template <int NS>
__global__ __launch_bounds__(256) void fwd2_n48_kernel(CnConvGeom g, const float* __restrict__ A, const float* __restrict__ B,
                                                       const float* __restrict__ bias, float* __restrict__ C, int M, int N, int K,
                                                       int act, float slope, int ntm, int ntn, long part_stride, int par,
                                                       const float* __restrict__ res, unsigned a_bytes, unsigned b_bytes, int flip) {
    fwd2_body<4, 1, 1, 3, true, true, 16, NS, 0, false, 16>(g, A, B, bias, C, M, N, K, act, slope, ntm, ntn, part_stride, par, res, a_bytes,
                                                            b_bytes, flip, nullptr, 0, 0.f, 1, 1);
}

inline unsigned fwd2_grid_x(int ntm, int ntn, int par) { return (unsigned)(par ? ntm * ntn : 8 * cn_cdiv((long)ntm * ntn, 8)); }

template <int NS>
int launch2_n48(const CnConvGeom& g, const float* A, const float* B, const float* bias, float* C, long M, int N, int K, int act, float slope,
                int splits, long part_stride, int par, hipStream_t s, const float* res, unsigned a_bytes, unsigned b_bytes) {
    const int ntm = cn_cdiv(M, 64), ntn = cn_cdiv(N, 48);
    dim3 grid(fwd2_grid_x(ntm, ntn, par), 1, (unsigned)splits);
    hipLaunchKernelGGL((fwd2_n48_kernel<NS>), grid, dim3(256), 0, s, g, A, B, bias, C, (int)M, N, K, act, slope, ntm, ntn, part_stride, par, res,
                       a_bytes, b_bytes, 1);
    CN_LAUNCH_CHECK();
    return CN_OK;
}

template <int WM, int WN, int TM, int TN, bool BT, bool GATHER, int KB, int NS, int NP, bool BF = false>
int launch2(const CnConvGeom& g, const float* A, const float* B, const float* bias, float* C, long M, int N, int K, int act, float slope,
            int splits, long part_stride, int par, hipStream_t s, const float* res, unsigned a_bytes, unsigned b_bytes, int flip = 1,
            float* stats = nullptr, int stats_mode = 0, float stats_slope = 0.f, int srows = 1, int sper = 1) {
    constexpr int BM = 32 * WM * TM, BN = 32 * WN * TN;
    const int ntm = cn_cdiv(M, BM), ntn = cn_cdiv(N, BN);
    dim3 grid(fwd2_grid_x(ntm, ntn, par), 1, (unsigned)splits);
    hipLaunchKernelGGL((fwd2_kernel<WM, WN, TM, TN, BT, GATHER, KB, NS, NP, BF>), grid, dim3(256 + 64 * NP), 0, s, g, A, B, bias, C, (int)M, N, K, act,
                       slope, ntm, ntn, part_stride, par, res, a_bytes, b_bytes, flip, stats, stats_mode, stats_slope, srows, sper);
    CN_LAUNCH_CHECK();
    return CN_OK;
}

int g_fwd2_kb = 0;
int g_fwd2_ns = 0;
int g_fwd2_np = -1;

}

void cn_fwd2_tune(int kb, int ns, int np) {
    g_fwd2_kb = kb;
    g_fwd2_ns = ns;
    g_fwd2_np = np;
}

void cn_fwd2_grid(int cfg, long M, int N, int par, int splits, int grid[3]) {
    const int bm = cfg == 2 ? 64 : 128, bn = cfg == 0 ? 128 : cfg == 4 ? 96 : cfg == 3 ? 32 : 64;
    grid[0] = (int)fwd2_grid_x(cn_cdiv(M, bm), cn_cdiv(N, bn), par);
    grid[1] = 1;
    grid[2] = splits;
}

extern "C" int cn_fwd2_col_block(int cfg, int bt, int gathered, int n, int kb, int np) {
    return (cfg == 2 && bt && gathered && n == 48 && kb == 16 && np == 0) ? 16 : 32;
}

int cn_fwd2(const CnConvGeom* gp, int cfg, int bt, const float* A, const float* B, const float* bias, float* C, long M, int N, int K,
            int act, float slope, int splits, long part_stride, int par, hipStream_t s, const float* res, double x_elems, double w_elems,
            float* stats, int stats_mode, float stats_slope, int srows, int sper) {
    if ((res || stats) && (splits > 1 || part_stride)) return CN_EUNSUPPORTED;
    if (stats && bt) return CN_EUNSUPPORTED;
    if (K % 16 != 0 || N % 4 != 0 || M <= 0 || M > 0x7fffffffL || (par && !gp)) return CN_EUNSUPPORTED;
    if (gp && (gp->dl_d > 2 || gp->dl_h > 2 || gp->dl_w > 2)) return CN_EUNSUPPORTED;
    if (x_elems * 4.0 >= 2147483647.0 || w_elems * 4.0 >= 2147483647.0) return CN_EUNSUPPORTED;
    const unsigned ab = (unsigned)(x_elems * 4.0), bb = (unsigned)(w_elems * 4.0);
    static const CnConvGeom none = {};
    int kb = g_fwd2_kb ? g_fwd2_kb : 16;
    int ns = g_fwd2_ns ? g_fwd2_ns : 4;
    if (kb == 32 && (K % 32 != 0 || cfg != 2)) kb = 16;
    if (kb == 32) ns = 3;
    int np = g_fwd2_np >= 0 ? g_fwd2_np : 0;
    if (cfg != 2 || kb == 32) np = 0;
#define L3(WM, WN, TM, TN, KB_, NS_, NP_)                                                                                                          \
    return gp ? (bt ? launch2<WM, WN, TM, TN, true, true, KB_, NS_, NP_>(*gp, A, B, bias, C, M, N, K, act, slope, splits, part_stride, par, s, res, ab, bb, 1, stats, stats_mode, stats_slope, srows, sper)   \
                    : launch2<WM, WN, TM, TN, false, true, KB_, NS_, NP_>(*gp, A, B, bias, C, M, N, K, act, slope, splits, part_stride, par, s, res, ab, bb, 1, stats, stats_mode, stats_slope, srows, sper)) \
              : (bt ? launch2<WM, WN, TM, TN, true, false, KB_, NS_, NP_>(none, A, B, bias, C, M, N, K, act, slope, splits, part_stride, 0, s, res, ab, bb, 1, stats, stats_mode, stats_slope, srows, sper)   \
                    : launch2<WM, WN, TM, TN, false, false, KB_, NS_, NP_>(none, A, B, bias, C, M, N, K, act, slope, splits, part_stride, 0, s, res, ab, bb, 1, stats, stats_mode, stats_slope, srows, sper))
#define L2(WM, WN, TM, TN)                 \
    if (ns == 3) { L3(WM, WN, TM, TN, 16, 3, 0); } \
    else { L3(WM, WN, TM, TN, 16, 4, 0); }
    switch (cfg) {
        case 0: L2(2, 2, 2, 2);
        case 1: L2(2, 2, 2, 1);
        case 2:
            if (cn_fwd2_col_block(cfg, bt, gp != nullptr, N, kb, np) == 16) {
                if (ns == 3) return launch2_n48<3>(*gp, A, B, bias, C, M, N, K, act, slope, splits, part_stride, par, s, res, ab, bb);
                return launch2_n48<4>(*gp, A, B, bias, C, M, N, K, act, slope, splits, part_stride, par, s, res, ab, bb);
            }
            if (kb == 32) { L3(2, 2, 1, 1, 32, 3, 0); }
            if (np == 1) { if (ns == 3) { L3(2, 2, 1, 1, 16, 3, 1); } else { L3(2, 2, 1, 1, 16, 4, 1); } }
            if (np == 2) { if (ns == 3) { L3(2, 2, 1, 1, 16, 3, 2); } else { L3(2, 2, 1, 1, 16, 4, 2); } }
            L2(2, 2, 1, 1);
        case 3: L2(4, 1, 1, 1);
        case 4: L2(4, 1, 1, 3);
        default: return CN_EUNSUPPORTED;
    }
#undef L2
#undef L3
}

int cn_fwd2_bf16(const CnConvGeom& g, int cfg, int flip, const void* x, const void* wb, const float* bias, void* y, int act, float slope,
                 int par, hipStream_t s) {
    const long M = (long)g.n * g.out_d * g.out_h * g.out_w;
    const int N = g.cout, K = g.cin;
    if (K % 32 != 0 || N % 8 != 0 || M <= 0 || M > 0x7fffffffL) return CN_EUNSUPPORTED;
    if (g.dl_d > 2 || g.dl_h > 2 || g.dl_w > 2) return CN_EUNSUPPORTED;
    const double xe = (double)g.n * g.in_d * g.in_h * g.in_w * g.cin, we = (double)g.k_d * g.k_h * g.k_w * g.cin * g.cout;
    if (xe * 2.0 >= 2147483647.0 || we * 2.0 >= 2147483647.0) return CN_EUNSUPPORTED;
    const unsigned ab = (unsigned)(xe * 2.0), bb = (unsigned)(we * 2.0);
    const float* A = reinterpret_cast<const float*>(x);
    const float* B = reinterpret_cast<const float*>(wb);
    float* C = reinterpret_cast<float*>(y);
    const long wgs = (long)cn_cdiv(M, cfg == 2 ? 64 : 128) * cn_cdiv(N, cfg == 0 ? 128 : cfg == 4 ? 96 : 64);
    const int np = g_fwd2_np >= 0 ? g_fwd2_np : 0;
    const int ns = g_fwd2_ns ? g_fwd2_ns : ((cfg == 0 || cfg == 4 || wgs >= 2048) ? 3 : 4);
#define LB(WM, WN, TM, TN, NS_, NP_) \
    return launch2<WM, WN, TM, TN, true, true, 16, NS_, NP_, true>(g, A, B, bias, C, M, N, K, act, slope, 1, 0, par, s, nullptr, ab, bb, flip)
#define LB2(WM, WN, TM, TN, NP_)   \
    if (ns == 3) { LB(WM, WN, TM, TN, 3, NP_); } \
    else { LB(WM, WN, TM, TN, 4, NP_); }
    constexpr int kb_env = 32;
    constexpr long kb_wgs = 1024;
#define LB32(WM, WN, TM, TN) \
    return launch2<WM, WN, TM, TN, true, true, 32, 3, 0, true>(g, A, B, bias, C, M, N, K, act, slope, 1, 0, par, s, nullptr, ab, bb, flip)
    if (kb_env == 32 && K % 64 == 0 && wgs <= kb_wgs && (long)K * g.k_d * g.k_h * g.k_w >= 128) {
        switch (cfg) {
            case 1: LB32(2, 2, 2, 1);
            case 2: LB32(2, 2, 1, 1);
            default: break;
        }
    }
#undef LB32
    switch (cfg) {
        case 0: if (np) { LB2(2, 2, 2, 2, 2); } LB2(2, 2, 2, 2, 0);
        case 1: if (np) { LB2(2, 2, 2, 1, 2); } LB2(2, 2, 2, 1, 0);
        case 2: if (np) { LB2(2, 2, 1, 1, 2); } LB2(2, 2, 1, 1, 0);
        case 4: if (np) { LB2(4, 1, 1, 3, 2); } LB2(4, 1, 1, 3, 0);
        default: return CN_EUNSUPPORTED;
    }
#undef LB2
#undef LB
}
```

### confignet_amd/csrc/winograd.hip

```cpp
#include "common.h"

#include "mma_tile.h"

namespace {

constexpr int WKB = 8;
typedef float f32x2 __attribute__((ext_vector_type(2)));

struct WinoGeom {
    int n, h, w, cin, cout, th, tw, bh, bw;
};

__global__ void wino_filter_kernel(const float* __restrict__ W, float* __restrict__ U, int cin, int cout, int dgrad) {
    const long total = (long)cin * cout;
    for (long i = (long)blockIdx.x * blockDim.x + threadIdx.x; i < total; i += (long)gridDim.x * blockDim.x) {
        const int co = (int)(i % cout), ci = (int)(i / cout);
        float g[3][3];
#pragma unroll
        for (int a = 0; a < 3; ++a)
#pragma unroll
            for (int b = 0; b < 3; ++b)
                g[a][b] = dgrad ? W[((long)((2 - a) * 3 + (2 - b)) * cin + ci) * cout + co] : W[((long)(a * 3 + b) * cin + ci) * cout + co];
        float t[4][3];
#pragma unroll
        for (int b = 0; b < 3; ++b) {
            t[0][b] = g[0][b];
            t[1][b] = 0.5f * (g[0][b] + g[1][b] + g[2][b]);
            t[2][b] = 0.5f * (g[0][b] - g[1][b] + g[2][b]);
            t[3][b] = g[2][b];
        }
        const long k = dgrad ? co : ci, nn = dgrad ? ci : co;
        const long kdim = dgrad ? cout : cin, ndim = dgrad ? cin : cout;
#pragma unroll
        for (int a = 0; a < 4; ++a) {
            const float u0 = t[a][0], u1 = 0.5f * (t[a][0] + t[a][1] + t[a][2]), u2 = 0.5f * (t[a][0] - t[a][1] + t[a][2]), u3 = t[a][2];
            U[((long)(a * 4 + 0) * kdim + k) * ndim + nn] = u0;
            U[((long)(a * 4 + 1) * kdim + k) * ndim + nn] = u1;
            U[((long)(a * 4 + 2) * kdim + k) * ndim + nn] = u2;
            U[((long)(a * 4 + 3) * kdim + k) * ndim + nn] = u3;
        }
    }
}

__global__ __launch_bounds__(512, 1) void wino_fwd_kernel(WinoGeom g, const float* __restrict__ X, const float* __restrict__ U,
                                                          const float* __restrict__ bias, float* __restrict__ Y, int act, float slope) {
    constexpr int BT = 64, BC = 64, LDV = BT + 4, LDU = BC;
    constexpr int RAW_SLOTS = 324, RAW_FLOATS = 12 * 64 * 4;
    extern __shared__ __attribute__((aligned(16))) float smem[];
    float (*Vs)[16][WKB][LDV] = reinterpret_cast<float (*)[16][WKB][LDV]>(smem);
    float (*Us)[16][WKB][LDU] = reinterpret_cast<float (*)[16][WKB][LDU]>(smem + 2 * 16 * WKB * LDV);
    __shared__ __attribute__((aligned(16))) float Raw0[RAW_FLOATS], Raw1[RAW_FLOATS];
    int* tilebase = reinterpret_cast<int*>(smem + 2 * 16 * WKB * (LDV + LDU));
    int* tilehw = tilebase + BT;
    const int tid = threadIdx.x, lane = tid & 63, wave = tid >> 6;
    const int ph = wave >> 2, wt = (wave >> 1) & 1, wc = wave & 1, half = lane >> 5, l31 = lane & 31;

    const int nblk = g.n * g.bh * g.bw, total = nblk * (g.cout / BC);
    int wg = blockIdx.x;
    if (total % 8 == 0) wg = (wg & 7) * (total >> 3) + (wg >> 3);
    const int blk = wg % nblk, c0 = (wg / nblk) * BC;
    int img, brem, bty, btx;
    divmod_pos(blk, g.bh * g.bw, img, brem);
    divmod_pos(brem, g.bw, bty, btx);

    const int gt = tid >> 3, ch = tid & 7, ty = gt >> 3, tx = gt & 7;
    if (ch == 0) {
        const int th = bty * 8 + ty, tw = btx * 8 + tx;
        const bool valid = th < g.th && tw < g.tw;
        tilebase[gt] = valid ? (img * g.h + 2 * th) * g.w + 2 * tw : -1;
        tilehw[gt] = ((2 * th) << 16) | (2 * tw);
    }
    const __amdgpu_buffer_rsrc_t xres = __builtin_amdgcn_make_buffer_rsrc(const_cast<float*>(X), 0, g.n * g.h * g.w * g.cin * 4, 0x00020000);
    const __amdgpu_buffer_rsrc_t ures = __builtin_amdgcn_make_buffer_rsrc(const_cast<float*>(U), 0, 16 * g.cin * g.cout * 4, 0x00020000);
    typedef float f32x4 __attribute__((ext_vector_type(4)));
    unsigned uoff[4];
    f32x4 ru[4];
#pragma unroll
    for (int j = 0; j < 4; ++j) {
        const int piece = wave * 4 + j, p = piece >> 1, k0 = (piece & 1) * 4;
        uoff[j] = (unsigned)((p * g.cin + k0 + (lane >> 4)) * g.cout + c0 + (lane & 15) * 4) * 4u;
    }
    auto load_filter_piece = [&](int j, int ks) { ru[j] = __builtin_amdgcn_raw_buffer_load_b128(ures, uoff[j], ks * WKB * g.cout * 4, 0); };
    auto store_filter_piece = [&](int j, int buf) {
        const int piece = wave * 4 + j, p = piece >> 1, k0 = (piece & 1) * 4;
        *reinterpret_cast<f32x4*>(&Us[buf][p][k0 + (lane >> 4)][(lane & 15) * 4]) = ru[j];
    };
    unsigned xoff[2];
#pragma unroll
    for (int j = 0; j < 2; ++j) {
        const int q = (j * 8 + wave) * 64 + lane, slot = q >> 1;
        const int r = slot / 18, rem = slot - r * 18, par = rem >= 9, c = 2 * (rem - 9 * par) + par;
        const int yy = bty * 16 - 1 + r, xx = btx * 16 - 1 + c;
        const bool in = slot < RAW_SLOTS && yy >= 0 && yy < g.h && xx >= 0 && xx < g.w;
        xoff[j] = in ? (unsigned)(((img * g.h + yy) * g.w + xx) * g.cin + (q & 1) * 4) * 4u : 0x80000000u;
    }
    auto load_input_piece = [&](int j, int ks, int rbuf) {
        if (j == 1 && wave >= 4) return;
        __builtin_amdgcn_raw_ptr_buffer_load_lds(xres, (__attribute__((address_space(3))) float*)&(rbuf ? Raw1 : Raw0)[(j * 8 + wave) * 256], 16,
                                                 xoff[j], ks * WKB * 4, 0, 0);
    };
    float dd[16], tt[16], vv = 0.f;
    const int rawt = ((4 * ty) * 9 + tx) * 8 + ch;
    auto transform_item = [&](int rbuf, int vbuf, int it) {
        if (it < 16) {
            const int i = it >> 2, j = it & 3;
            dd[it] = (rbuf ? Raw1 : Raw0)[rawt + (i * 18 + (j & 1) * 9 + (j >> 1)) * 8];
        } else if (it < 32) {
            const int j = (it - 16) >> 2, s_ = it & 3;
            tt[s_ * 4 + j] = s_ == 0 ? dd[0 * 4 + j] - dd[2 * 4 + j] : s_ == 1 ? dd[1 * 4 + j] + dd[2 * 4 + j]
                           : s_ == 2 ? dd[2 * 4 + j] - dd[1 * 4 + j] : dd[1 * 4 + j] - dd[3 * 4 + j];
        } else {
            const int k = (it - 32) >> 1, i = k >> 2, s_ = k & 3;
            if ((it & 1) == 0)
                vv = s_ == 0 ? tt[i * 4 + 0] - tt[i * 4 + 2] : s_ == 1 ? tt[i * 4 + 1] + tt[i * 4 + 2]
                   : s_ == 2 ? tt[i * 4 + 2] - tt[i * 4 + 1] : tt[i * 4 + 1] - tt[i * 4 + 3];
            else
                Vs[vbuf][k][ch][gt] = vv;
        }
    };

    f32x16 acc[8];
#pragma unroll
    for (int p = 0; p < 8; ++p)
#pragma unroll
        for (int r = 0; r < 16; ++r) acc[p][r] = 0.f;

    const int nks = g.cin / WKB;
    const int trow = wt * 32 + l31, ccol = wc * 32 + l31;
    auto step = [&](int ks, int buf) {
        const int ksf = ks + 1 < nks ? ks + 1 : nks - 1, ksx = ks + 2 < nks ? ks + 2 : nks - 2 + buf;
        __builtin_amdgcn_s_waitcnt(0x0F70);
        __syncthreads();
        float a[2][4], b[2][4];
#pragma unroll
        for (int e = 0; e < 4; ++e) {
            a[0][e] = Vs[buf][8 * ph + e][half][trow];
            b[0][e] = Us[buf][8 * ph + e][half][ccol];
        }
#pragma unroll
        for (int m = 0; m < 32; ++m) {
            const int grp = m >> 2, e = m & 3, cur = grp & 1, q = m & 7;
            __builtin_amdgcn_sched_barrier(0);
            acc[q] = __builtin_amdgcn_mfma_f32_32x32x2f32(a[cur][e], b[cur][e], acc[q], 0, 0, 0);
            if (grp + 1 < 8) {
                const int kk = ((grp + 1) >> 1) * 2, pn = 8 * ph + 4 * ((grp + 1) & 1) + e;
                a[cur ^ 1][e] = Vs[buf][pn][kk + half][trow];
                b[cur ^ 1][e] = Us[buf][pn][kk + half][ccol];
            }
            transform_item(buf ^ 1, buf ^ 1, 2 * m);
            transform_item(buf ^ 1, buf ^ 1, 2 * m + 1);
            if (m < 4) load_filter_piece(m, ksf);
            else if (m < 6) load_input_piece(m - 4, ksx, buf);
            else if (m >= 28) store_filter_piece(m - 28, buf ^ 1);
        }
        __builtin_amdgcn_sched_barrier(0);
    };

#pragma unroll
    for (int j = 0; j < 4; ++j) load_filter_piece(j, 0);
#pragma unroll
    for (int j = 0; j < 2; ++j) load_input_piece(j, 0, 0);
#pragma unroll
    for (int j = 0; j < 2; ++j) load_input_piece(j, 1, 1);
#pragma unroll
    for (int j = 0; j < 4; ++j) store_filter_piece(j, 0);
    __builtin_amdgcn_s_waitcnt(0x0F70);
    __syncthreads();
#pragma unroll
    for (int it = 0; it < 64; ++it) transform_item(0, 0, it);
    for (int ks = 0; ks < nks; ks += 2) {
        step(ks, 0);
        step(ks + 1, 1);
    }
    __builtin_amdgcn_s_waitcnt(0x0F70);
    __syncthreads();

    float* xchg = smem + ((wt * 2 + wc) * 2) * 16 * 2 * 64;
    float keep[16][2];
#pragma unroll
    for (int r = 0; r < 16; ++r) {
        __builtin_amdgcn_sched_barrier(0);
        float tm[2][4];
#pragma unroll
        for (int j = 0; j < 4; ++j) {
            const float m0 = acc[j][r], m1 = acc[4 + j][r];
            tm[0][j] = ph ? m0 : m0 + m1;
            tm[1][j] = ph ? -m0 - m1 : m1;
        }
#pragma unroll
        for (int i = 0; i < 2; ++i) {
            const float y0 = tm[i][0] + tm[i][1] + tm[i][2], y1 = tm[i][1] - tm[i][2] - tm[i][3];
            if (i == ph) {
                keep[r][0] = y0;
                keep[r][1] = y1;
            } else {
                xchg[((ph * 16 + r) * 2 + 0) * 64 + lane] = y0;
                xchg[((ph * 16 + r) * 2 + 1) * 64 + lane] = y1;
            }
        }
    }
    __syncthreads();
    const int co = c0 + wc * 32 + l31;
    const float bv = bias ? bias[co] : 0.f;
#pragma unroll
    for (int r = 0; r < 16; ++r) {
        const int tl = wt * 32 + 4 * half + (r & 3) + 8 * (r >> 2);
        const int base = tilebase[tl];
        const int hw = tilehw[tl], oy = hw >> 16, ox = hw & 0xffff;
        const float y0 = keep[r][0] + xchg[(((ph ^ 1) * 16 + r) * 2 + 0) * 64 + lane];
        const float y1 = keep[r][1] + xchg[(((ph ^ 1) * 16 + r) * 2 + 1) * 64 + lane];
        if (base < 0 || oy + ph >= g.h) continue;
        float* dst = Y + ((long)base + ph * g.w) * g.cout + co;
        dst[0] = cn_apply_act(y0 + bv, act, slope);
        if (ox + 1 < g.w) dst[g.cout] = cn_apply_act(y1 + bv, act, slope);
    }
}

}

extern "C" int cn_conv_wino_filter(const float* w, float* u, int cin, int cout, int dgrad, void* stream) {
    CN_CHECK_ARG(w && u && cin > 0 && cout > 0, "wino_filter: bad args");
    const long total = (long)cin * cout;
    const int blocks = (int)((total + 255) / 256 > 4096 ? 4096 : (total + 255) / 256);
    hipLaunchKernelGGL(wino_filter_kernel, dim3(blocks), dim3(256), 0, (hipStream_t)stream, w, u, cin, cout, dgrad);
    CN_LAUNCH_CHECK();
    return CN_OK;
}

extern "C" int cn_conv_fwd_wino(int n, int h, int w, int cin, int cout, const float* x, const float* u, const float* bias,
                                float* y, int act, float slope, void* stream) {
    CN_CHECK_ARG(x && u && y && n > 0 && h > 0 && w > 0, "conv_fwd_wino: bad args");
    if (cin % (2 * WKB) || cout % 64) return CN_EUNSUPPORTED;
    CN_CHECK_ARG((double)n * h * w * (cin > cout ? cin : cout) * 4.0 < 2147483647.0 && 64.0 * cin * cout < 2147483647.0, "tensor exceeds 2^31 bytes (buffer descriptors, 32-bit offsets)");
    WinoGeom g{n, h, w, cin, cout, (h + 1) / 2, (w + 1) / 2, (h + 15) / 16, (w + 15) / 16};
    const long ntiles = (long)n * g.th * g.tw, nblk = (long)n * g.bh * g.bw;
    constexpr size_t lds = sizeof(float) * (2 * 16 * WKB * (68 + 64)) + sizeof(int) * 128;
    static bool attr_set = false;
    if (!attr_set) {
        CN_HIP(hipFuncSetAttribute(reinterpret_cast<const void*>(wino_fwd_kernel), hipFuncAttributeMaxDynamicSharedMemorySize, (int)lds));
        attr_set = true;
    }
    hipStream_t s = (hipStream_t)stream;
    cn_prof_begin(s, 2.0 * 16.0 * (double)ntiles * cin * cout,
                  4.0 * ((double)n * h * w * (cin + cout) + 16.0 * cin * cout), CN_FAM_WINO);
    hipLaunchKernelGGL(wino_fwd_kernel, dim3((unsigned)(nblk * (cout / 64))), dim3(512), lds, s, g, x, u, bias, y, act, slope);
    cn_prof_end(s);
    CN_LAUNCH_CHECK();
    return CN_OK;
}
```

### confignet_amd/dnn_models/real_encoder.py

```python
import numpy as np
import torch

from .. import functional as F
from ..nn import Net, glorot_uniform, he_normal
from ..ops import ACT_TANH, ConvSpec

RESNET50_STACKS = [(64, 3, 1), (128, 4, 2), (256, 6, 2), (512, 3, 2)]
BN_EPS = 1.001e-5
C7 = ConvSpec((7, 7), stride=2, explicit_pad=3)
C1 = {1: ConvSpec((1, 1)), 2: ConvSpec((1, 1), stride=2)}
C3 = ConvSpec((3, 3))


def resnet50_layers():
    yield "conv1_conv", "conv", 3, 64, 7
    yield "conv1_bn", "bn", 0, 64, 0
    cin = 64
    for si, (f, blocks, _) in enumerate(RESNET50_STACKS):
        for bi in range(blocks):
            n = "conv%d_block%d" % (si + 2, bi + 1)
            yield n + "_1_conv", "conv", cin, f, 1
            yield n + "_1_bn", "bn", 0, f, 0
            yield n + "_2_conv", "conv", f, f, 3
            yield n + "_2_bn", "bn", 0, f, 0
            if bi == 0:
                yield n + "_0_conv", "conv", cin, 4 * f, 1
                yield n + "_3_conv", "conv", f, 4 * f, 1
                yield n + "_0_bn", "bn", 0, 4 * f, 0
                yield n + "_3_bn", "bn", 0, 4 * f, 0
            else:
                yield n + "_3_conv", "conv", f, 4 * f, 1
                yield n + "_3_bn", "bn", 0, 4 * f, 0
            cin = 4 * f


class RealEncoder(Net):
    def __init__(self, latent_dim, input_shape, rotation_ranges, rng=None):
        super().__init__()
        rng = rng or np.random.default_rng()
        where = {}
        for name, kind, cin, cout, k in resnet50_layers():
            where[name] = len(self._entries)
            if kind == "conv":
                self.add_weight(name + "/kernel", he_normal(rng, (k, k, cin, cout)))
                self.add_weight(name + "/bias", np.zeros(cout, np.float32))
            else:
                self.add_weight(name + "/gamma", np.full(cout, 0.25 if name.endswith("_3_bn") else 1.0, np.float32))
                self.add_weight(name + "/beta", np.zeros(cout, np.float32))
                self.add_weight(name + "/moving_mean", np.zeros(cout, np.float32), trainable=False)
                self.add_weight(name + "/moving_variance", np.ones(cout, np.float32), trainable=False)
        self._convs = []

        def conv_bn(prefix, spec):
            self._convs.append((where[prefix + "_conv"], where[prefix + "_bn"], spec))

        conv_bn("conv1", C7)
        for si, (filters, blocks, stride1) in enumerate(RESNET50_STACKS):
            for bi in range(blocks):
                n = "conv%d_block%d" % (si + 2, bi + 1)
                s = stride1 if bi == 0 else 1
                if bi == 0:
                    conv_bn(n + "_0", C1[s])
                conv_bn(n + "_1", C1[s])
                conv_bn(n + "_2", C3)
                conv_bn(n + "_3", C1[1])
        self.resnet_feature_dim = 2048
        self.add_weight("rotation_regressor/kernel", glorot_uniform(rng, (2048, 3)))
        self.add_weight("rotation_regressor/bias", np.zeros(3, np.float32))
        self.add_weight("feature_to_latent_mlp/kernel", glorot_uniform(rng, (2048, latent_dim)))
        self.add_weight("feature_to_latent_mlp/bias", np.zeros(latent_dim, np.float32))
        self.finalize()
        mult = np.pi * np.array([rotation_ranges[0][1], rotation_ranges[1][1], rotation_ranges[2][1]]) / 180.0
        self.rotation_range_multiplier = torch.tensor(mult, dtype=torch.float32, device=self.device)

    def _bn_coefficients(self, cat=False):
        ws = self.weights
        ks = [k for k, _, _ in self._convs]
        bs = [b for _, b, _ in self._convs]
        sizes = [ws[k + 1].shape[0] for k in ks]
        bias = torch.cat([ws[k + 1] for k in ks])
        gamma = torch.cat([ws[b] for b in bs])
        beta = torch.cat([ws[b + 1] for b in bs])
        if getattr(self, "_stat_cache", None) is None:
            self._stat_cache = (torch.cat([ws[b + 2] for b in bs]), torch.cat([ws[b + 3] for b in bs]))
        mean, var = self._stat_cache
        a = gamma * torch.rsqrt(var + BN_EPS)
        shift = beta + a * (bias - mean)
        if cat:
            return a, torch.split(shift, sizes)
        return torch.split(a, sizes), torch.split(shift, sizes)

    def non_trainable_changed(self):
        cache = getattr(self, "_stat_cache", None)
        if cache is not None:
            bs = [b for _, b, _ in self._convs]
            with torch.no_grad():
                cache[0].copy_(torch.cat([self.weights[b + 2] for b in bs]))
                cache[1].copy_(torch.cat([self.weights[b + 3] for b in bs]))

    def _fold_table(self):
        if getattr(self, "_fold_tab", None) is None:
            rows, views, dst, aoff = [], [], 0, 0
            base = self.arena.data_ptr()
            for kidx, _, _ in self._convs:
                w = self.weights[kidx]
                src = (w.data_ptr() - base) // 4
                assert 0 <= src and src % 4 == 0 and w.numel() % 4 == 0 and w.shape[-1] % 4 == 0 and w.is_contiguous()
                rows.append((src, dst, w.numel(), w.shape[-1], aoff))
                views.append((dst, tuple(w.shape)))
                dst += w.numel()
                aoff += w.shape[-1]
            self._fold_tab = (torch.tensor(rows, dtype=torch.int32, device=self.device), dst, views)
        return self._fold_tab

    def _folded_filters(self, a_cat):
        from ..nn import WEIGHTS_EPOCH
        from .. import ops
        stream = torch.cuda.current_stream().cuda_stream
        key = (WEIGHTS_EPOCH[0], self.epoch)
        cache = self.__dict__.setdefault("_fold_cache", {})
        c = cache.get(stream)
        if c is None or c[0] != key:
            for k in [k for k, v in cache.items() if v[0] != key]:
                del cache[k]
            seg, total, views = self._fold_table()
            packed = ops.scale_columns_segments(self.arena, seg, a_cat, total)
            c = cache[stream] = (key, [packed[o:o + int(np.prod(shp))].view(shp) for o, shp in views], packed)
        if ops._keepalive is not None:
            ops._keepalive.append(c[2])
        return c[1]

    def _features_folded(self, img):
        from .. import ops
        from ..ops import ACT_NONE, ACT_RELU
        a, shift = self._bn_coefficients(cat=True)
        wf = self._folded_filters(a)

        def conv(ci, x, res=None, relu=True):
            spec = self._convs[ci][2]
            g = spec.geom(tuple(x.shape), wf[ci].shape[-1])
            if res is None:
                return ops.conv_fwd(x, wf[ci], shift[ci], g, ACT_RELU if relu else ACT_NONE)
            return ops.conv_fwd_res(x, wf[ci], shift[ci], res, g, ACT_RELU)

        x = F.caffe_preprocess(img)
        x = conv(0, x)
        x = F.maxpool(x, 3, 2, 1)
        ci = 1
        for filters, blocks, stride1 in RESNET50_STACKS:
            for bi in range(blocks):
                if bi == 0:
                    sc = conv(ci, x, relu=False)
                    ci += 1
                else:
                    sc = x
                y = conv(ci, x)
                y = conv(ci + 1, y)
                x = conv(ci + 2, y, res=sc)
                ci += 3
        return F.global_avg_pool(x)

    def _fold_table9(self):
        if getattr(self, "_fold_tab9", None) is None:
            seg = self._fold_table()[0].cpu().numpy()
            base = self.arena.data_ptr()
            rows, blk = [], 0
            for (kidx, bidx, _), r in zip(self._convs, seg):
                cout = int(r[3])
                assert cout % 64 == 0
                offs = [(self.weights[i].data_ptr() - base) // 4 for i in (kidx + 1, bidx, bidx + 1)]
                assert all(o >= 0 and o % 4 == 0 for o in offs)
                rows.append(list(map(int, r)) + offs + [blk])
                blk += cout // 64
            self._fold_tab9 = (torch.tensor(rows, dtype=torch.int32, device=self.device), blk)
        return self._fold_tab9

    def _fold_coefficients(self):
        ws = self.weights
        ks = [k for k, _, _ in self._convs]
        bs = [b for _, b, _ in self._convs]
        with torch.no_grad():
            if getattr(self, "_stat_cache", None) is None:
                self._stat_cache = (torch.cat([ws[b + 2] for b in bs]), torch.cat([ws[b + 3] for b in bs]))
            mean, var = self._stat_cache
            rs = torch.rsqrt(var + BN_EPS)
            a = torch.cat([ws[b] for b in bs]) * rs
            bm = torch.cat([ws[k + 1] for k in ks]) - mean
            shift = torch.addcmul(torch.cat([ws[b + 1] for b in bs]), a, bm)
        return a, shift, rs, bm

    def _trunk_params(self):
        return [w for w in self.weights[:-4] if w.requires_grad]

    folded_tape = True

    def _conv_bn(self, ci, x, coef, res=None, relu=True):
        kidx, _, spec = self._convs[ci]
        z = F.conv(x, self.weights[kidx], None, spec)
        return F.channel_affine_act(z, coef[0][ci], coef[1][ci], res, relu)

    fold_inference = True

    def features(self, img):
        if self.fold_inference and not torch.is_grad_enabled() and img.dtype == torch.float32:
            from .. import ops
            if ops.ACT_DTYPE == torch.float32:
                return self._features_folded(img)
        from .. import ops as _ops
        if self.folded_tape and torch.is_grad_enabled() and (_ops.ACT_DTYPE == torch.float32 or self.folded_tape == "always"):
            params = self._trunk_params()
            if len(params) == sum(1 for i in self._trainable_idx if i < len(self.weights) - 4) or (not params and img.requires_grad):
                x = F.caffe_preprocess(img)
                return F.global_avg_pool(ResNetTrunkFn.apply(self, x, *params))
        coef = self._bn_coefficients()
        x = F.caffe_preprocess(img)
        x = self._conv_bn(0, x, coef)
        x = F.maxpool(x, 3, 2, 1)
        ci = 1
        for filters, blocks, stride1 in RESNET50_STACKS:
            for bi in range(blocks):
                if bi == 0:
                    sc = self._conv_bn(ci, x, coef, relu=False)
                    ci += 1
                else:
                    sc = x
                y = self._conv_bn(ci, x, coef)
                y = self._conv_bn(ci + 1, y, coef)
                x = self._conv_bn(ci + 2, y, coef, res=sc, relu=True)
                ci += 3
        return F.global_avg_pool(x)

    def __call__(self, input_img):
        feat = self.features(self.to_device(input_img))
        w = self.weights
        rot = F.linear(feat, w[-4], w[-3], ACT_TANH) * self.rotation_range_multiplier
        return F.linear(feat, w[-2], w[-1]), rot

    def predict(self, imgs, batch_size=32):
        embs, rots = [], []
        with torch.no_grad():
            for s in range(0, len(imgs), batch_size):
                e, r = self(imgs[s:s + batch_size])
                embs.append(e.cpu().numpy())
                rots.append(r.cpu().numpy())
        return np.concatenate(embs), np.concatenate(rots)


class ResNetTrunkFn(torch.autograd.Function):

    @staticmethod
    def forward(ctx, enc, x, *params):
        from .. import ops
        from ..ops import ACT_NONE, ACT_RELU
        a, shift, rs, bm = enc._fold_coefficients()
        wf = enc._folded_filters(a)
        sizes = [wf[ci].shape[-1] for ci in range(len(enc._convs))]
        offs = [0]
        for c in sizes:
            offs.append(offs[-1] + c)
        sh = [shift[offs[i]:offs[i + 1]] for i in range(len(sizes))]
        x = x.contiguous()

        def conv(ci, t, res=None, relu=True):
            g = enc._convs[ci][2].geom(tuple(t.shape), sizes[ci])
            if res is None:
                return ops.conv_fwd(t, wf[ci], sh[ci], g, ACT_RELU if relu else ACT_NONE)
            return ops.conv_fwd_res(t, wf[ci], sh[ci], res, g, ACT_RELU)

        saved = [x]
        y0 = conv(0, x)
        t = ops.maxpool_fwd(y0, 3, 2, 1)
        saved += [y0, t]
        ci = 1
        for filters, blocks, stride1 in RESNET50_STACKS:
            for bi in range(blocks):
                sc = t
                if bi == 0:
                    sc = conv(ci, t, relu=False)
                    ci += 1
                y1 = conv(ci, t)
                y2 = conv(ci + 1, y1)
                t = conv(ci + 2, y2, res=sc)
                saved += [y1, y2, t]
                ci += 3
        ctx.enc, ctx.coef, ctx.wf, ctx.offs = enc, (a, rs, bm), wf, offs
        ctx.save_for_backward(*saved)
        return t

    @staticmethod
    def backward(ctx, gy):
        from .. import ops
        from ..ops import ACT_RELU
        if torch.is_grad_enabled():
            raise RuntimeError("ResNetTrunkFn is first-order only")
        enc, wf, offs = ctx.enc, ctx.wf, ctx.offs
        a, rs, bm = ctx.coef
        saved = list(ctx.saved_tensors)
        seg5, total, views = enc._fold_table()
        seg9, blocks = enc._fold_table9()
        dev = gy.device
        params = enc._trunk_params()
        want_w = any(ctx.needs_input_grad[2:]) and not F._INPUT_GRADS_ONLY
        sunk = want_w and ops.sink_for(params[0]) is not None
        gwf = gsh = None
        if want_w:
            gwf = torch.empty(total, device=dev, dtype=torch.float32)
            gsh = ops.zero_pool_alloc((offs[-1],), dev)
            if gsh is None:
                gsh = torch.zeros(offs[-1], device=dev, dtype=torch.float32)

        def geom(ci, t):
            return enc._convs[ci][2].geom(tuple(t.shape), wf[ci].shape[-1])

        later = []

        def wgrad(ci, t_in, gu):
            o, shp = views[ci]
            if not want_w:
                return
            g_, dst = geom(ci, t_in), gwf[o:o + int(np.prod(shp))].view(shp)
            if ops.wgrad_groupable(t_in, gu, g_):
                later.append((t_in, gu, g_, dst, 0))
            else:
                ops.sink_conv_wgrad_to(t_in, gu, g_, shp, dst, defer=sunk)

        def relu_bwd(ci, g, y, also=None):
            if not want_w:
                return ops.act_bwd(g, y, ACT_RELU)
            gu, part = ops.act_bwd_partials(g, y, ACT_RELU)
            ops.sum_rows_into(part, gsh[offs[ci]:offs[ci + 1]], defer=sunk)
            if also is not None:
                ops.sum_rows_into(part, gsh[offs[also]:offs[also + 1]], defer=sunk)
            return gu

        g = gy.contiguous()
        layout = []
        ci = 1
        for filters, blocks_, stride1 in RESNET50_STACKS:
            for bi in range(blocks_):
                layout.append((ci, bi == 0))
                ci += 4 if bi == 0 else 3
        pos = len(saved)
        for first, has_sc in reversed(layout):
            y1, y2, t_out = saved[pos - 3], saved[pos - 2], saved[pos - 1]
            pos -= 3
            t_in = saved[pos - 1]
            c1 = first + 1 if has_sc else first
            gu3 = relu_bwd(c1 + 2, g, t_out, also=first if has_sc else None)
            wgrad(c1 + 2, y2, gu3)
            gu2 = relu_bwd(c1 + 1, ops.conv_dgrad(gu3, wf[c1 + 2], geom(c1 + 2, y2)), y2)
            wgrad(c1 + 1, y1, gu2)
            gu1 = relu_bwd(c1, ops.conv_dgrad(gu2, wf[c1 + 1], geom(c1 + 1, y1)), y1)
            wgrad(c1, t_in, gu1)
            if has_sc:
                wgrad(first, t_in, gu3)
                skip = ops.conv_dgrad(gu3, wf[first], geom(first, t_in))
            else:
                skip = gu3
            g = ops.conv_dgrad_res(gu1, wf[c1], geom(c1, t_in), skip)
        x, y0, t = saved[0], saved[1], saved[2]
        g = ops.maxpool_bwd(y0, g, 3, 2, 1)
        gu0 = relu_bwd(0, g, y0)
        wgrad(0, x, gu0)
        gx = ops.conv_dgrad(gu0, wf[0], geom(0, x)) if ctx.needs_input_grad[1] else None
        if not want_w:
            return (None, gx) + (None,) * len(params)
        if sunk:
            ops.sink_conv_wgrad_group(later)
            gout = enc.grad_arena
            ops.sink_post(lambda: ops.bn_fold_bwd(seg9, blocks, gwf, gsh, enc.arena, a, rs, bm, gout), keep=(gwf, gsh, a, rs, bm))
            return (None, gx) + (None,) * len(params)
        ops._sum_slabs_grouped(ops.conv_wgrad_grouped(later))
        gout = torch.zeros_like(enc.arena)
        ops.bn_fold_bwd(seg9, blocks, gwf, gsh, enc.arena, a, rs, bm, gout)
        base = enc.arena.data_ptr()
        grads = []
        for p_ in params:
            o = (p_.data_ptr() - base) // 4
            grads.append(gout[o:o + p_.numel()].view(p_.shape))
        return (None, gx) + tuple(grads)
```

### confignet_amd/ops.py

```python
import contextlib
import ctypes
import math
import os
import threading

import torch

from ._lib import CN_BF16, CN_EUNSUPPORTED, CN_F32, CN_U8, CnConvGeom, CnDepthJob, CnGanJob, CnRowsJob, CnSumJob, check, lib

ACT_NONE, ACT_LRELU, ACT_RELU, ACT_TANH, ACT_RELU6, ACT_SIGMOID = 0, 1, 2, 3, 4, 5

ACT_DTYPE = torch.float32


def set_activation_dtype(dtype):
    global ACT_DTYPE
    if isinstance(dtype, str):
        dtype = {"f32": torch.float32, "fp32": torch.float32, "float32": torch.float32, "bf16": torch.bfloat16,
                 "bfloat16": torch.bfloat16}[dtype]
    assert dtype in (torch.float32, torch.bfloat16)
    ACT_DTYPE = dtype


def _stream():
# ... 176 lines not shown
    return ACT_DTYPE == torch.bfloat16 and g.cin % 8 == 0 and g.cout % 8 == 0


UPFOLD = True
UPFOLD_MAX_CLASS_TAPS = 64


def upfold_class_taps(g):
    ks = (g.k_d, g.k_h, g.k_w) if g.nd == 3 else (g.k_h, g.k_w)
    return math.prod(k + 1 if k >= 3 else 3 for k in ks)


def upfold_ok(g):
    return (UPFOLD and g.up == 1 and g.cin > 4 and g.cout > 4 and g.s_d * g.s_h * g.s_w == 1 and g.dl_d * g.dl_h * g.dl_w == 1
            and all(2 <= k <= 4 for k in ((g.k_d, g.k_h, g.k_w) if g.nd == 3 else (g.k_h, g.k_w)))
            and upfold_class_taps(g) <= UPFOLD_MAX_CLASS_TAPS
            and g.out_h == 2 * g.in_h and g.out_w == 2 * g.in_w and (g.nd == 2 or g.out_d == 2 * g.in_d))


def _copy_geom(g, **kw):
    out = CnConvGeom()
    for name, _ in CnConvGeom._fields_:
        setattr(out, name, getattr(g, name))
    for k, v in kw.items():
        setattr(out, k, v)
    return out


def upfold_prepare(w, g):
    def make(wd_):
        k3 = (ctypes.c_int * 3)(g.k_d, g.k_h, g.k_w)
        p3 = (ctypes.c_int * 3)(g.p_d, g.p_h, g.p_w)
        k2, p2 = (ctypes.c_int * 3)(), (ctypes.c_int * 3)()
        wd_ = _c(wd_)
        ks = [g.k_d, g.k_h, g.k_w]
        sizes = [1 if (g.nd == 2 and i == 0) else (ks[i] + 1 if ks[i] >= 3 else 3) for i in range(3)]
        t2 = sizes[0] * sizes[1] * sizes[2]
        both = torch.empty((2, t2 * g.cin * g.cout), device=wd_.device, dtype=torch.float32)
        check(lib.cn_upfold_weights(_fptr(wd_), _ptr(both[0]), _ptr(both[1]), g.nd, k3, p3, g.cin, g.cout, k2, p2, _stream()),
              "cn_upfold_weights")
        assert list(k2) == sizes, (list(k2), sizes)
        return both[0], both[1], tuple(k2), tuple(p2)
    wf, wd, (kd, kh, kw), (pd, ph, pw) = _weight_cache(w, "_cn_upfold_%d_%d%d%d_%d%d%d" % (g.nd, g.k_d, g.k_h, g.k_w, g.p_d, g.p_h, g.p_w), make)
    gd = _copy_geom(g, k_d=kd, k_h=kh, k_w=kw, dl_d=(2 if g.nd == 3 else 1), dl_h=2, dl_w=2,
                    p_d=kd - 1 - pd, p_h=kh - 1 - ph, p_w=kw - 1 - pw, up=0)
    g2 = _copy_geom(g, in_d=g.out_d, in_h=g.out_h, in_w=g.out_w, cin=g.cout, out_d=g.in_d, out_h=g.in_h, out_w=g.in_w,
                    cout=g.cin, k_d=kd, k_h=kh, k_w=kw, s_d=(2 if g.nd == 3 else 1), s_h=2, s_w=2, p_d=pd, p_h=ph, p_w=pw, up=0)
    taps = (kd, kh, kw) if g.nd == 3 else (kh, kw)
    return wf.view(taps + (g.cin, g.cout)), wd.view(taps + (g.cout, g.cin)), gd, g2


def upfold_wgrad(gw2, g, w_shape, out=None, single_writer=False):
    gw = out if out is not None else torch.empty(w_shape, device=gw2.device, dtype=torch.float32)
    k3 = (ctypes.c_int * 3)(g.k_d, g.k_h, g.k_w)
    p3 = (ctypes.c_int * 3)(g.p_d, g.p_h, g.p_w)
    mode = 0 if out is None else (2 if single_writer else 1)
    check(lib.cn_upfold_wgrad(_fptr(_c(gw2)), _ptr(gw), g.nd, k3, p3, g.cin, g.cout, mode, _stream()), "cn_upfold_wgrad")
    return gw


WINOGRAD = True
WINO_MIN_WGS = 32
WINO_MIN_FILL = 0.7


def _wino_ok(g, cin, cout):
    if not (WINOGRAD and g.nd == 2 and g.k_h == 3 and g.k_w == 3 and g.s_h == 1 and g.s_w == 1 and g.dl_h == 1 and g.dl_w == 1
            and g.up == 0 and g.p_h == 1 and g.p_w == 1 and g.out_h == g.in_h and g.out_w == g.in_w):
        return False
    if cin % 16 or cout % 64:
        return False
    th, tw = (g.in_h + 1) // 2, (g.in_w + 1) // 2
    bh, bw = (th + 7) // 8, (tw + 7) // 8
    if th * tw < WINO_MIN_FILL * (bh * bw * 64):
        return False
    return g.n * bh * bw * (cout // 64) >= WINO_MIN_WGS


WINO4 = True
WINO4_MIN_WGS = 128


def _wino4_ok(g, cin, cout):
    if not (WINO4 and WINOGRAD and g.nd == 2 and g.k_h == 3 and g.k_w == 3 and g.s_h == 1 and g.s_w == 1 and g.dl_h == 1 and g.dl_w == 1
            and g.up == 0 and g.p_h == 1 and g.p_w == 1 and g.out_h == g.in_h and g.out_w == g.in_w):
        return False
    if g.in_h % 16 or g.in_w % 32 or cin % 16 or cout % 64:
        return False
    return g.n * (g.in_h // 16) * (g.in_w // 32) * (cout // 64) >= WINO4_MIN_WGS


def _wino4_filter(w, dgrad):
    def make(wd_):
        wd_ = _c(wd_)
        cin, cout = wd_.shape[-2], wd_.shape[-1]
        u = torch.empty((36, cout, cin) if dgrad else (36, cin, cout), device=wd_.device, dtype=torch.float32)
        check(lib.cn_conv_wino4_filter(_fptr(wd_), _ptr(u), cin, cout, int(dgrad), _stream()), "cn_conv_wino4_filter")
        return u
    return _weight_cache(w, "_cn_wino4_d" if dgrad else "_cn_wino4_f", make)


def wino4_saved_flops(g):
    tiles = g.n * (g.in_h // 4) * (g.in_w // 4)
    return 2.0 * g.cin * g.cout * (9.0 * g.n * g.in_h * g.in_w - 36.0 * tiles)


def _wino_filter(w, dgrad):
    def make(wd_):
        wd_ = _c(wd_)
        cin, cout = wd_.shape[-2], wd_.shape[-1]
        u = torch.empty((16, cout, cin) if dgrad else (16, cin, cout), device=wd_.device, dtype=torch.float32)
        check(lib.cn_conv_wino_filter(_fptr(wd_), _ptr(u), cin, cout, int(dgrad), _stream()), "cn_conv_wino_filter")
        return u
    return _weight_cache(w, "_cn_wino_d" if dgrad else "_cn_wino_f", make)


class _StatsSlot(threading.local):
    request = None
    ready = None


_stats = _StatsSlot()
STATS_FUSION = True


class request_stats:
    def __init__(self, kind, slope=0.0):
        self.req = (kind, float(slope))

    def __enter__(self):
        self.prev, _stats.request = _stats.request, (self.req if STATS_FUSION and not DETERMINISTIC else None)

    def __exit__(self, *exc):
        _stats.request = self.prev


def take_stats(y, kind):
    ent, _stats.ready = _stats.ready, None
    if ent is not None and ent[0] == y.data_ptr() and ent[1] == tuple(y.shape) and ent[2] == kind:
        return ent[3]
    return None


def conv_fwd(x, w, bias, g, act=ACT_NONE, slope=0.0):
    req, _stats.request = _stats.request, None
    _stats.ready = None
    out_dtype = _act_out_dtype(g.cout)
    if ACT_DTYPE == torch.float32 and x.dtype == torch.float32 and _wino4_ok(g, g.cin, g.cout):
        y = torch.empty(geom_out_shape(g), device=x.device, dtype=torch.float32)
        check(lib.cn_conv_fwd_wino4(g.n, g.in_h, g.in_w, g.cin, g.cout, _ptr(_c(x)), _ptr(_wino4_filter(w, False)), _fptr(bias), _ptr(y),
                                    act, slope, _stream()), "cn_conv_fwd_wino4")
        prof_note_saved(wino4_saved_flops(g))
        return y
    if ACT_DTYPE == torch.float32 and x.dtype == torch.float32 and _wino_ok(g, g.cin, g.cout):
        y = torch.empty(geom_out_shape(g), device=x.device, dtype=torch.float32)
        check(lib.cn_conv_fwd_wino(g.n, g.in_h, g.in_w, g.cin, g.cout, _ptr(x), _ptr(_wino_filter(w, False)), _fptr(bias), _ptr(y),
                                   act, slope, _stream()), "cn_conv_fwd_wino")
        prof_note_saved(wino_saved_flops(g))
        return y
    if _bf16_conv_ok(g):
        x = cast(x, torch.bfloat16)
        y = torch.empty(geom_out_shape(g), device=x.device, dtype=torch.bfloat16)
        wf, _ = weight_prep_bf16(w)
        check(lib.cn_conv_fwd_bf16(ctypes.byref(g), _ptr(x), _ptr(wf), _fptr(bias), _ptr(y), act, slope, _stream()), "cn_conv_fwd_bf16")
        return y
    x = f32(x)
    if out_dtype == torch.bfloat16 and MIXED_FIRST_LAYERS and g.cin == 3:
        y = torch.empty(geom_out_shape(g), device=x.device, dtype=torch.bfloat16)
        rc = lib.cn_conv_fwd_dt(ctypes.byref(g), _ptr(x), CN_F32, _fptr(w), _fptr(bias), _ptr(y), CN_BF16, act, slope, _stream())
        if rc == 0:
            return y
        if rc != CN_EUNSUPPORTED:
            check(rc, "cn_conv_fwd_dt")
    y = torch.empty(geom_out_shape(g), device=x.device, dtype=torch.float32)
    if req is not None and out_dtype == torch.float32 and g.cout % 4 == 0 and (req[0] == "act" or act == ACT_NONE):
        nk = 2 if req[0] == "act" else 4
        mark = _active_pool.cur if _active_pool is not None else None
        st = zero_pool_alloc((nk, g.n, g.cout), x.device)
        if st is not None:
            rc = lib.cn_conv_fwd_stats(ctypes.byref(g), _ptr(_c(x)), _fptr(w), _fptr(bias), _ptr(y), act, slope, _ptr(st), 1 if nk == 2 else 2,
                                       req[1], _stream())
            if rc == 0:
                _stats.ready = (y.data_ptr(), tuple(y.shape), req[0], tuple(st[k] for k in range(nk)))
                return y
            if rc != CN_EUNSUPPORTED:
                check(rc, "cn_conv_fwd_stats")
            _active_pool.cur = mark
    check(lib.cn_conv_fwd(ctypes.byref(g), _ptr(x), _fptr(w), _fptr(bias), _ptr(y), act, slope, _stream()), "cn_conv_fwd")
    return cast(y, out_dtype)


W4_EP_POOL, W4_EP_POOL_ONLY, W4_EP_MASK = 1, 2, 3


def conv_fwd_pool(x, w, bias, g, act=ACT_NONE, slope=0.0, keep_full=True):
    if not (ACT_DTYPE == torch.float32 and x.dtype == torch.float32 and _wino4_ok(g, g.cin, g.cout)):
        return None
    _stats.request = _stats.ready = None
    y = torch.empty(geom_out_shape(g), device=x.device, dtype=torch.float32) if keep_full else None
    pooled = torch.empty((g.n, g.in_h // 2, g.in_w // 2, g.cout), device=x.device, dtype=torch.float32)
    check(lib.cn_conv_fwd_wino4_ep(g.n, g.in_h, g.in_w, g.cin, g.cout, _ptr(_c(x)), _ptr(_wino4_filter(w, False)), _fptr(bias), _ptr(y),
                                   act, slope, W4_EP_POOL if keep_full else W4_EP_POOL_ONLY, _ptr(pooled), None, None, None, 1, 0.0,
                                   _stream()), "cn_conv_fwd_wino4_ep")
    prof_note_saved(wino4_saved_flops(g))
    return y, pooled


def conv_dgrad_masked(gy, w, g, y, target=None, s=None, k=0.0):
    if not (ACT_DTYPE == torch.float32 and gy.dtype == torch.float32 and y.dtype == torch.float32 and _wino4_ok(g, g.cout, g.cin)):
        return None
    if target is not None and (target.dtype != torch.float32 or s is None or s.numel() not in (1, g.n)):
        return None
    _log_mask(y, ACT_RELU)
    gu = torch.empty(geom_in_shape(g, upsampled=True), device=gy.device, dtype=torch.float32)
    check(lib.cn_conv_fwd_wino4_ep(g.n, g.in_h, g.in_w, g.cout, g.cin, _ptr(_c(gy)), _ptr(_wino4_filter(w, True)), None, _ptr(gu),
                                   ACT_NONE, 0.0, W4_EP_MASK, None, _ptr(_c(y)), None if target is None else _ptr(_c(target)),
                                   None if target is None else _fptr(s), 1 if target is None else s.numel(), k, _stream()),
          "cn_conv_fwd_wino4_ep")
    prof_note_saved(wino4_saved_flops(g))
    return gu


def conv_fwd_res(x, w, bias, res, g, act=ACT_NONE, slope=0.0):
    assert act in (ACT_NONE, ACT_RELU)
    if ACT_DTYPE == torch.float32 and x.dtype == torch.float32 and res.dtype == torch.float32 and not _wino_ok(g, g.cin, g.cout):
        x, res = _c(x), _c(res)
        y = torch.empty(geom_out_shape(g), device=x.device, dtype=torch.float32)
        rc = lib.cn_conv_fwd_res(ctypes.byref(g), _ptr(x), _fptr(w), _fptr(bias), _ptr(res), _ptr(y), act, slope, _stream())
        if rc == 0:
            return y
        if rc != CN_EUNSUPPORTED:
            check(rc, "cn_conv_fwd_res")
    y = conv_fwd(x, w, bias, g)
    return nc_lin2(tuple(y.shape), y, None, res, None, None, flags=8 if act == ACT_RELU else 0)


def scale_columns_segments(src, seg, a, total):
    dst = torch.empty(total, device=src.device, dtype=torch.float32)
    check(lib.cn_scale_columns_segments(_fptr(src), _ptr(dst), _ptr(seg), _fptr(_c(a)), seg.shape[0], total, _stream()),
          "cn_scale_columns_segments")
    return dst


def weight_tflip(w):
    w = _c(w)
    taps = int(math.prod(w.shape[:-2]))
    wt = torch.empty(w.shape[:-2] + (w.shape[-1], w.shape[-2]), device=w.device, dtype=torch.float32)
    check(lib.cn_conv_weight_tflip(_fptr(w), _ptr(wt), taps, w.shape[-2], w.shape[-1], _stream()), "cn_conv_weight_tflip")
    return wt


def conv_dgrad(gy, w, g):
    shape = geom_in_shape(g, upsampled=True)
    if _bf16_conv_ok(g):
        gy = cast(gy, torch.bfloat16)
        gu = torch.empty(shape, device=gy.device, dtype=torch.bfloat16)
        _, wd = weight_prep_bf16(w)
        check(lib.cn_conv_dgrad_bf16(ctypes.byref(g), _ptr(gy), _ptr(wd), _ptr(gu), _stream()), "cn_conv_dgrad_bf16")
        return gu
    if gy.dtype == torch.bfloat16 and MIXED_FIRST_LAYERS and g.cin == 3:
        gu = torch.empty(shape, device=gy.device, dtype=torch.float32)
        wt = _weight_cache(w, "_cn_tflip", weight_tflip)
        rc = lib.cn_conv_dgrad_dt(ctypes.byref(g), _ptr(_c(gy)), CN_BF16, _fptr(wt), _ptr(gu), CN_F32, _stream())
        if rc == 0:
            return cast(gu, _act_out_dtype(g.cin))
        if rc != CN_EUNSUPPORTED:
            check(rc, "cn_conv_dgrad_dt")
    gy = f32(gy)
    gu = torch.empty(shape, device=gy.device, dtype=torch.float32)
    if ACT_DTYPE == torch.float32 and _wino4_ok(g, g.cout, g.cin):
        check(lib.cn_conv_fwd_wino4(g.n, g.in_h, g.in_w, g.cout, g.cin, _ptr(_c(gy)), _ptr(_wino4_filter(w, True)), None, _ptr(gu),
                                    ACT_NONE, 0.0, _stream()), "cn_conv_fwd_wino4")
        prof_note_saved(wino4_saved_flops(g))
        return gu
    if ACT_DTYPE == torch.float32 and _wino_ok(g, g.cout, g.cin):
        check(lib.cn_conv_fwd_wino(g.n, g.in_h, g.in_w, g.cout, g.cin, _ptr(gy), _ptr(_wino_filter(w, True)), None, _ptr(gu),
                                   ACT_NONE, 0.0, _stream()), "cn_conv_fwd_wino")
        prof_note_saved(wino_saved_flops(g))
        return gu
    if DGRAD_FROM_W:
        rc = lib.cn_conv_dgrad_w(ctypes.byref(g), _ptr(gy), _fptr(_c(w)), _ptr(gu), _stream())
        if rc == 0:
            return cast(gu, _act_out_dtype(g.cin))
        if rc != CN_EUNSUPPORTED:
            check(rc, "cn_conv_dgrad_w")
    wt = _weight_cache(w, "_cn_tflip", weight_tflip)
    check(lib.cn_conv_dgrad(ctypes.byref(g), _ptr(gy), _fptr(wt), _ptr(gu), _stream()), "cn_conv_dgrad")
    return cast(gu, _act_out_dtype(g.cin))


def conv_dgrad_res(gy, w, g, res):
    if (ACT_DTYPE == torch.float32 and gy.dtype == torch.float32 and res.dtype == torch.float32 and DGRAD_FROM_W and not g.up
            and not _wino4_ok(g, g.cout, g.cin) and not _wino_ok(g, g.cout, g.cin)):
        gu = torch.empty(geom_in_shape(g, upsampled=True), device=gy.device, dtype=torch.float32)
        rc = lib.cn_conv_dgrad_w_res(ctypes.byref(g), _ptr(_c(gy)), _fptr(_c(w)), _ptr(_c(res)), _ptr(gu), _stream())
        if rc == 0:
            return gu
        if rc != CN_EUNSUPPORTED:
            check(rc, "cn_conv_dgrad_w_res")
    gu = conv_dgrad(gy, w, g)
    return nc_lin2(tuple(gu.shape), gu, None, res, None, None)


DGRAD_FROM_W = True
MIXED_FIRST_LAYERS = True
WGRAD_WRITE, WGRAD_ADD, WGRAD_ZEROED = 0, 1, 2


def conv_wgrad(x, gy, g, w_shape, out=None, accumulate=True, defer=True, ws=None):
    gw, mode = out, WGRAD_ADD if accumulate else WGRAD_WRITE
    if out is None:
        gw, mode = zero_pool_alloc(w_shape, x.device), WGRAD_ZEROED
        if gw is None:
            gw, mode = torch.empty(w_shape, device=x.device, dtype=torch.float32), WGRAD_WRITE
    x = _c(cast(x, torch.bfloat16 if _bf16_conv_ok(g) else torch.float32))
    nbytes = ctypes.c_size_t(0)
    rc = lib.cn_conv_wgrad_dt_workspace_bytes(ctypes.byref(g), _dt(x), _dt(gy), ctypes.byref(nbytes))
    if rc == CN_EUNSUPPORTED and gy.dtype != x.dtype:
        gy = cast(gy, x.dtype)
        rc = lib.cn_conv_wgrad_dt_workspace_bytes(ctypes.byref(g), _dt(x), _dt(gy), ctypes.byref(nbytes))
    check(rc, "cn_conv_wgrad_dt_workspace_bytes")
    gy, nbytes = _c(gy), nbytes.value
    if ws is None:
        ws = torch.empty(nbytes // 4, device=x.device, dtype=torch.float32) if nbytes else None
    else:
        assert ws.dtype == torch.float32 and ws.numel() * 4 >= nbytes, "conv_wgrad: workspace of %d bytes, %d needed" % (ws.numel() * 4, nbytes)
    parts = ctypes.c_int(0) if nbytes and out is not None and _SINK is not None and defer else None
    check(lib.cn_conv_wgrad_dt(ctypes.byref(g), _ptr(x), _dt(x), _ptr(gy), _dt(gy), _fptr(gw), mode, _ptr(ws), nbytes,
                               None if parts is None else ctypes.byref(parts), _stream()), "cn_conv_wgrad_dt")
    if parts is not None and parts.value:
        _SINK.slabs.append((ws, gw, parts.value, gw.numel(), int(mode != WGRAD_WRITE)))
    return gw


WGRAD_GROUPED = True


def wgrad_groupable(x, gy, g):
    if not WGRAD_GROUPED or DETERMINISTIC or ACT_DTYPE != torch.float32 or x.dtype != torch.float32 or gy.dtype != torch.float32:
        return False
    out = (ctypes.c_longlong * 12)()
    return lib.cn_conv_wgrad_plan(ctypes.byref(g), CN_F32, CN_F32, 1, 0xffffffff, -1, out) == 0 and out[0] == 3


def conv_wgrad_grouped_plan(geoms, solo=False):
    n = len(geoms)
    arr = (CnConvGeom * n)(*geoms)
    out, info = (ctypes.c_longlong * (10 * n))(), (ctypes.c_longlong * 4)()
    check(lib.cn_conv_wgrad_grouped_plan(n, arr, int(solo), out, info), "cn_conv_wgrad_grouped_plan")
    return [tuple(out[10 * j:10 * j + 10]) for j in range(n)], tuple(info)


def conv_wgrad_grouped(jobs, solo=False):
    if not jobs:
        return []
    n = len(jobs)
    xs, gys = [_c(j[0]) for j in jobs], [_c(j[1]) for j in jobs]
    plan, _ = conv_wgrad_grouped_plan([j[2] for j in jobs], solo)
    total = sum(p[9] for p in plan)
    ws_all = torch.empty(total, device=xs[0].device, dtype=torch.float32) if total else None
    ws, o = [], 0
    for p in plan:
        ws.append(ws_all[o:o + p[9]] if p[9] else None)
        o += p[9]
    vp = ctypes.c_void_p * n
    parts = (ctypes.c_int * n)()
    check(lib.cn_conv_wgrad_grouped(n, (CnConvGeom * n)(*[j[2] for j in jobs]), vp(*[_fptr(t).value for t in xs]),
                                    vp(*[_fptr(t).value for t in gys]), vp(*[_fptr(j[3]).value for j in jobs]),
                                    vp(*[None if w is None else w.data_ptr() for w in ws]),
                                    (ctypes.c_size_t * n)(*[4 * p[9] for p in plan]), (ctypes.c_int * n)(*[int(bool(j[4])) for j in jobs]),
                                    int(solo), parts, _stream()), "cn_conv_wgrad_grouped")
    return [(ws[k], jobs[k][3], parts[k], jobs[k][3].numel(), int(bool(jobs[k][4]))) for k in range(n) if parts[k]]


GRAD_SINK = True
_SINK = None


def sink_rounds(jobs, key):
    rounds, seen = [], {}
    for job in jobs:
        k = key(job)
        r = seen.get(k, 0)
        seen[k] = r + 1
        if r == len(rounds):
            rounds.append([])
        rounds[r].append(job)
    return rounds


class _Sink:

    def __init__(self, params):
        self.slots = {p.data_ptr(): p.grad for p in params if p.grad is not None}
        self.touched = []
        self.wgrads = []
        self.slabs = []
        self.depth = []
        self.upfold = {}
        self.post = []
        self.post_keep = []

    def note_stream(self):
        cur = torch.cuda.current_stream()
        if all(cur != s_ for s_ in self.touched):
            self.touched.append(cur)


def _sum_slabs_grouped(slabs):
    for batch in sink_rounds(slabs, lambda job: job[1].data_ptr()):
        jobs = (CnSumJob * len(batch))()
        for q, (ws, dst, parts, count, acc) in zip(jobs, batch):
            q.src, q.dst, q.count, q.parts, q.accumulate = ws.data_ptr(), dst.data_ptr(), count, parts, acc
        check(lib.cn_sum_parts_grouped(jobs, len(batch), _stream()), "cn_sum_parts_grouped")


def _gemm_depth_grouped(depth):
    for batch in sink_rounds(depth, lambda job: job[2].data_ptr()):
        jobs = (CnDepthJob * len(batch))()
        for q, (a, b, slot) in zip(jobs, batch):
            q.a, q.b, q.c = a.data_ptr(), b.data_ptr(), slot.data_ptr()
            q.m, q.n, q.k, q.lda, q.ldb, q.ldc = a.shape[1], b.shape[1], a.shape[0], a.shape[1], b.shape[1], b.shape[1]
        check(lib.cn_gemm_depth_grouped(jobs, len(batch), _stream()), "cn_gemm_depth_grouped")


def _release_operands(cur, others, operands):
    if not torch.cuda.is_current_stream_capturing():
        for t in operands:
            t.record_stream(cur)
    for s_ in others:
        s_.wait_stream(cur)


class grad_sink:
    def __init__(self, params):
        self.params = params

    def __enter__(self):
        global _SINK
        assert _SINK is None, "nested gradient sinks"
        if GRAD_SINK and self.params:
            _SINK = _Sink(self.params)
        return self

    def join(self):
        st = _SINK
        if st is None:
            return
        cur = torch.cuda.current_stream()
        others = [s_ for s_ in st.touched if s_ != cur]
        for s_ in others:
            cur.wait_stream(s_)
        wgrads, slabs, depth, upfold, post, post_keep = st.wgrads, st.slabs, st.depth, st.upfold, st.post, st.post_keep
        st.touched, st.wgrads, st.slabs, st.depth, st.upfold, st.post, st.post_keep = [], [], [], [], {}, [], []
        slabs = slabs + conv_wgrad_grouped(wgrads)
        _sum_slabs_grouped(slabs)
        _gemm_depth_grouped(depth)
        if wgrads or slabs or depth:
            _release_operands(cur, others, [t for j in wgrads for t in j[:2]] + [j[0] for j in slabs] + [t for j in depth for t in j[:2]])
        for gw2, g, w_shape, slot in upfold.values():
            upfold_wgrad(gw2, g, w_shape, out=slot, single_writer=True)
        for fn in post:
            fn()
        if post:
            _release_operands(cur, others, post_keep)
        if st.wgrads or st.slabs or st.depth or st.upfold or st.post:
            raise RuntimeError("a sink_post function queued work on the gradient sink after its join")

    def __exit__(self, exc_type, exc, tb):
        global _SINK
        try:
            if exc_type is None:
                self.join()
        finally:
            _SINK = None


def sink_for(w):
    if _SINK is None or w is None:
        return None
    return _SINK.slots.get(w.data_ptr())


def sink_conv_wgrad(x, gy, g, w_shape, slot):
    if _SINK is not None:
        _SINK.note_stream()
    conv_wgrad(x, gy, g, w_shape, out=slot)


def sink_conv_wgrad_to(x, gy, g, w_shape, dst, defer=True):
    if _SINK is not None:
        _SINK.note_stream()
    conv_wgrad(x, gy, g, w_shape, out=dst, accumulate=False, defer=defer)


def sink_conv_wgrad_group(jobs):
    st = _SINK
    if st is None:
        _sum_slabs_grouped(conv_wgrad_grouped(jobs))
        return
    st.note_stream()
    st.wgrads.extend(jobs)


def sink_post(fn, keep=()):
    st = _SINK
    if st is None:
        fn()
        return
    st.note_stream()
    st.post_keep.extend(t for t in keep if t is not None)
    st.post.append(fn)


def bn_fold_bwd(seg9, blocks, gwf, gshift, arena, a, rs, bm, gout, chunked=True):
    scratch = None
    if chunked and not DETERMINISTIC:
        scratch = torch.empty(lib.cn_bn_fold_bwd_chunks() * a.numel(), device=a.device, dtype=torch.float32)
    check(lib.cn_bn_fold_bwd(_ptr(seg9), seg9.shape[0], blocks, _fptr(gwf), _fptr(gshift), _fptr(arena), _fptr(a), _fptr(rs), _fptr(bm),
                             _fptr(gout), _fptr(scratch), a.numel(), _stream()), "cn_bn_fold_bwd")


def sink_upfold_wgrad(gy, x, g2, wd_shape, g, w_shape, slot):
    st = _SINK
    ent = st.upfold.get(slot.data_ptr())
    if ent is None:
        gw2 = zero_pool_alloc(wd_shape, x.device)
        if gw2 is None:
            gw2 = torch.zeros(wd_shape, device=x.device, dtype=torch.float32)
        ent = st.upfold[slot.data_ptr()] = (gw2, g, w_shape, slot)
    st.note_stream()
    conv_wgrad(gy, x, g2, wd_shape, out=ent[0])


def sink_gemm(a, b, slot, trans_a=False, trans_b=False):
    st = _SINK
    if st is not None:
        st.note_stream()
        if (trans_a and not trans_b and a.shape[0] <= 32 and a.dtype == torch.float32 and b.dtype == torch.float32
                and a.is_contiguous() and b.is_contiguous() and slot.is_contiguous()):
            st.depth.append((a, b, slot))
            return
    gemm_acc(a, b, slot, trans_a, trans_b)


class _ZeroPool:
    def __init__(self, device, numel):
        self.buf = torch.zeros(numel, device=device, dtype=torch.float32)
        self.cur = 0
        self.dirty = 0


_pools = {}
_active_pool = None
ZERO_POOL_FLOATS = 96 * 1024 * 1024


def zero_pool_begin(name, device):
    global _active_pool
    p = _pools.get((name, device))
    if p is None:
        p = _pools[(name, device)] = _ZeroPool(device, ZERO_POOL_FLOATS)
    if p.dirty:
        p.buf[:p.dirty].zero_()
    p.cur = 0
    _active_pool = p


def zero_pool_end():
    global _active_pool
    if _active_pool is not None:
        _active_pool.dirty = max(_active_pool.dirty, _active_pool.cur)
    _active_pool = None


def zero_pool_alloc(shape, device):
    p = _active_pool
    if p is None or p.buf.device != device:
        return None
    n = int(math.prod(shape))
    n4 = (n + 3) // 4 * 4
    if p.cur + n4 > p.buf.numel():
        return None
    out = p.buf[p.cur:p.cur + n].view(shape)
    p.cur += n4
    return out


def _sums(shape, device):
    t = zero_pool_alloc(shape, device)
    if t is not None:
        return t, 16
    return torch.empty(shape, device=device, dtype=torch.float32), 0


def zero_(t):
    check(lib.cn_zero(_fptr(t), t.numel() * 4, _stream()), "cn_zero")
    return t


def sumpool2(gu):
    nd = gu.dim() - 2
    sp = [s // 2 for s in gu.shape[1:-1]]
    gx = torch.empty((gu.shape[0], *sp, gu.shape[-1]), device=gu.device, dtype=gu.dtype)
    d, h, w = ([1] + sp) if nd == 2 else sp
    check(lib.cn_sumpool2(_ptr(gu), _ptr(gx), nd, gu.shape[0], d, h, w, gu.shape[-1], _dt(gu), _stream()), "cn_sumpool2")
# ... 784 lines not shown
```

### include/confignet_hip.h

```cpp
#ifndef CONFIGNET_HIP_H
#define CONFIGNET_HIP_H
#include <stddef.h>
#include <stdint.h>

#ifdef __cplusplus
extern "C" {
#endif

#define CN_OK 0
#define CN_EINVAL (-1)
#define CN_EHIP (-2)
#define CN_EUNSUPPORTED (-3)

#define CN_F32 0
#define CN_BF16 1
#define CN_U8 2

#define CN_ACT_NONE 0
#define CN_ACT_LRELU 1
#define CN_ACT_RELU 2
#define CN_ACT_TANH 3
#define CN_ACT_RELU6 4
#define CN_ACT_SIGMOID 5

typedef struct CnConvGeom {
    int nd, n;
    int in_d, in_h, in_w, cin;
    int out_d, out_h, out_w, cout;
    int k_d, k_h, k_w;
    int s_d, s_h, s_w;
    int dl_d, dl_h, dl_w;
    int p_d, p_h, p_w;
    int up;
} CnConvGeom;

const char* cn_last_error_string(void);
int cn_version(void);

int cn_conv_fwd(const CnConvGeom* g, const float* x, const float* w, const float* bias,
                float* y, int act, float slope, void* stream);
int cn_conv_fwd_stats(const CnConvGeom* g, const float* x, const float* w, const float* bias, float* y, int act, float slope,
                      float* stats, int stats_mode, float stats_slope, void* stream);
int cn_conv_fwd_res(const CnConvGeom* g, const float* x, const float* w, const float* bias, const float* res, float* y,
                    int act, float slope, void* stream);
int cn_conv_weight_tflip(const float* w, float* w_tflip, int taps, int cin, int cout, void* stream);
int cn_conv_dgrad(const CnConvGeom* g, const float* gy, const float* w_tflip, float* gu, void* stream);
int cn_conv_dgrad_w(const CnConvGeom* g, const float* gy, const float* w, float* gu, void* stream);
int cn_conv_dgrad_w_res(const CnConvGeom* g, const float* gy, const float* w, const float* res, float* gu, void* stream);
int cn_conv_wgrad(const CnConvGeom* g, const float* x, const float* gy, float* gw, int accumulate, void* stream);
size_t cn_conv_wgrad_workspace_bytes(const CnConvGeom* g);
int cn_conv_wgrad_ws(const CnConvGeom* g, const float* x, const float* gy, float* gw, int accumulate, void* workspace,
                     size_t workspace_bytes, void* stream);
int cn_conv_wgrad_ws_slabs(const CnConvGeom* g, const float* x, const float* gy, float* gw, int accumulate, void* workspace,
                           size_t workspace_bytes, int* parts, void* stream);
#define CN_WGRAD_WRITE 0
#define CN_WGRAD_ADD 1
#define CN_WGRAD_ZEROED 2
int cn_conv_wgrad_dt_workspace_bytes(const CnConvGeom* g, int x_dt, int gy_dt, size_t* bytes);
int cn_conv_wgrad_dt(const CnConvGeom* g, const void* x, int x_dt, const void* gy, int gy_dt, float* gw, int mode, void* workspace,
                     size_t workspace_bytes, int* parts, void* stream);
int cn_conv_wgrad_plan(const CnConvGeom* g, int x_dt, int gy_dt, int caller_slabs, unsigned routes, int det, long long out[12]);
int cn_conv_wgrad_grouped(int njobs, const CnConvGeom* geoms, const float* const* x, const float* const* gy, float* const* out,
                          float* const* ws, const size_t* ws_bytes, const int* accumulate, int solo, int* parts, void* stream);
int cn_conv_wgrad_grouped_plan(int njobs, const CnConvGeom* geoms, int solo, long long* out, long long info[4]);
typedef struct CnSumJob {
    const float* src;
    float* dst;
    long long count;
    int parts;
    int accumulate;
} CnSumJob;
int cn_sum_parts_grouped(const CnSumJob* jobs, int njobs, void* stream);
typedef struct CnDepthJob {
    const float* a;
    const float* b;
    float* c;
    int m, n, k, lda, ldb, ldc;
} CnDepthJob;
int cn_gemm_depth_grouped(const CnDepthJob* jobs, int njobs, void* stream);
typedef struct CnRowsJob {
    const float* a;
    const float* b;
    float* c;
    const float* bias;
    const float* mask;
    int m, n, k, lda, ldb, ldc, tb, act, accumulate;
    float slope;
} CnRowsJob;
int cn_gemm_rows_grouped(const CnRowsJob* jobs, int njobs, void* stream);
int cn_gemm_rows_grouped_k(const CnRowsJob* jobs, int njobs, void* stream);
int cn_gemm_rows_grouped_plan(const CnRowsJob* jobs, int njobs, int* out, int cap, int* nlaunches);
typedef struct CnGanJob {
    const float* s;
    float* out;
    const float* gout;
    int n;
    float label;
} CnGanJob;
int cn_gan_loss_grouped(const CnGanJob* jobs, int njobs, int backward, void* stream);
int cn_conv_fwd_dt(const CnConvGeom* g, const void* x, int x_dt, const float* w, const float* bias, void* y, int y_dt, int act,
                   float slope, void* stream);
int cn_conv_dgrad_dt(const CnConvGeom* g, const void* gy, int gy_dt, const float* w_tflip, void* gu, int gu_dt, void* stream);
int cn_conv_wgrad_c3_partials(void);
int cn_conv_wgrad_c3(const CnConvGeom* g, const float* x, const void* gy, int gy_dt, float* scratch, float* gw, int accumulate,
                     void* stream);
int cn_conv_wgrad_thin_partials(void);
int cn_conv_wgrad_thin(const CnConvGeom* g, const float* x, const float* gy, float* scratch, float* gw, int accumulate, void* stream);
int cn_conv_wino_filter(const float* w, float* u, int cin, int cout, int dgrad, void* stream);
int cn_conv_fwd_wino(int n, int h, int w, int cin, int cout, const float* x, const float* u, const float* bias, float* y,
                     int act, float slope, void* stream);
int cn_conv_wino4_filter(const float* w, float* u, int cin, int cout, int dgrad, void* stream);
int cn_conv_fwd_wino4(int n, int h, int w, int cin, int cout, const float* x, const float* u, const float* bias,
                      float* y, int act, float slope, void* stream);
#define CN_W4_EP_POOL 1
#define CN_W4_EP_POOL_ONLY 2
#define CN_W4_EP_MASK 3
int cn_conv_fwd_wino4_ep(int n, int h, int w, int cin, int cout, const float* x, const float* u, const float* bias, float* y,
                         int act, float slope, int mode, float* pooled, const float* ym, const float* target, const float* s,
                         int s_rows, float k, void* stream);
int cn_conv_tune(int cfg, int splits, long wg_blocks);
int cn_conv_fwd_plan(const CnConvGeom* g, int bt, int has_bias, int act, int has_res, int stats_mode, int x_dt, int y_dt, int out[8]);
int cn_conv_loop_select(int loop, int kb, int ns, int np);
int cn_fwd2_col_block(int cfg, int bt, int gathered, int n, int kb, int np);
int cn_sumpool2(const void* gu, void* gx, int nd, int n, int d, int h, int w, int c, int dt, void* stream);

int cn_conv_weight_prep_bf16(const float* w, uint16_t* wf, uint16_t* wd, int taps, int cin, int cout, void* stream);
int cn_conv_fwd_bf16(const CnConvGeom* g, const uint16_t* x, const uint16_t* wf, const float* bias, uint16_t* y,
                     int act, float slope, void* stream);
int cn_conv_dgrad_bf16(const CnConvGeom* g, const uint16_t* gy, const uint16_t* wd, uint16_t* gu, void* stream);
int cn_conv_wgrad_bf16(const CnConvGeom* g, const uint16_t* x, const uint16_t* gy, float* gw, int accumulate, void* stream);
int cn_upfold_weights(const float* w, float* wf, float* wd, int nd, const int* k3, const int* pad_lo3, int cin, int cout,
                      int* k2_out3, int* pad2_out3, void* stream);
int cn_upfold_wgrad(const float* gw2, float* gw, int nd, const int* k3, const int* pad_lo3, int cin, int cout,
                    int accumulate, void* stream);
int cn_cast(const void* src, int src_dt, void* dst, int dst_dt, size_t numel, void* stream);

int cn_gemm(int trans_a, int trans_b, int m, int n, int k, const float* a, int lda,
            const float* b, int ldb, float* c, int ldc, const float* bias, int act, float slope,
            void* stream);
int cn_gemm_plan(int trans_a, int trans_b, int m, int n, int k, int ldc, int has_bias, int act, int accumulate, int deterministic,
                 int out[9]);

int cn_set_deterministic(int on);
int cn_get_deterministic(void);
int cn_det_release_stream(void* stream);
int cn_zero(void* p, size_t bytes, void* stream);
int cn_gemm_acc(int trans_a, int trans_b, int m, int n, int k, const float* a, int lda, const float* b, int ldb,
                float* c, int ldc, void* stream);
int cn_sum_rows_into(const float* src, float* dst, int rows, int cols, int accumulate, void* stream);

int cn_nc_reduce_plan(int n, int s, int c, int nsums, int prezeroed, int det, int out[8]);
int cn_nc_reduce4(const void* x, float* out, int n, int s, int c, float slope, int flags, int dt, void* stream);
int cn_nc_reduce(const void* x1, const void* x2, float* sum1, float* sum2, int n, int s, int c,
                 int flags, float slope, int dt, void* stream);
int cn_nc_reduce_dact(const void* x1, const void* x2, float* sum1, float* sum2, void* dact_out, int n, int s, int c,
                      int flags, float slope, int act, int dt, void* stream);
int cn_bn_act_bwd(const void* gy, const void* y, const void* x, const float* a, void* g_out, void* gx, float* sum_g,
                  float* sum_gx, int n, int s, int c, int act, int flags, int dt, void* stream);
int cn_nc_lin2(const void* x1, const float* a1, const void* x2, const float* a2, const float* bb,
               const float* a3, const float* b3, void* y, int n, int s, int c, int cstride, int flags,
               float slope, int dt, void* stream);
int cn_nc_rows_plan(long long G, int CG, int ny, int out[2]);

int cn_norm_coef_fwd(int mode, const float* s1, const float* s2, const float* p1, const float* p2, float* A,
                     float* B, float* save_mean, float* save_r, int n, int c, int S, float eps, const void* x, int dt,
                     void* stream);
int cn_norm_coef_bwd(int mode, const float* t1, const float* t2, const float* save_mean, const float* save_r,
                     const float* p1, float* c1, float* c2, float* c0, float* gp1, float* gp2, int n, int c,
                     int S, float eps, void* stream);
int cn_norm_apply(int mode, int dir, const void* x1, const void* x2, const float* sa, const float* sb, const float* p1,
                  const float* p2, float* save_mean, float* save_r, float* gp1, float* gp2, const float* a3, const float* b3,
                  void* y, int n, int s, int c, float eps, int flags, float slope, int dt, void* stream);

int cn_dual_tail_coef_fwd(const float* T1, const float* T2, const float* U1, const float* U2, const float* mean,
                          const float* q, const float* sm, const float* ssd, const float* gamma, float* C1,
                          float* C2, float* C0, float* tstyle, int n, int c, int S, float eps, int n_style, int period,
                          void* stream);
int cn_dual_tail_coef_bwd(const float* H1, const float* H2p, const float* E, const float* u, const float* T1,
                          const float* T2, const float* U1, const float* U2, const float* mean, const float* q,
                          const float* sm, const float* ssd, const float* gamma, float* const* out13, int n, int c,
                          int S, float eps, int n_style, int period, void* stream);
int cn_dual_tail_gx(const void* h, const void* ta, const void* tx, const void* x, const float* kh,
                    const float* kt, const float* ka, const float* kc, const float* et, const float* ex,
                    const float* e0, void* out, int n, int s, int c, float slope, int nrep, int dt, void* stream);
int cn_dual_tail_gx_tx(const void* h, const void* ta, const void* tx, const void* x, const float* kh, const float* kt,
                       const float* ka, const float* kc, const float* et, const float* ex, const float* e0,
                       const float* K1, const float* K2, const float* K0, const float* D2, const float* D0, void* out,
                       void* out_tx, int n, int s, int c, float slope, int nrep, int ta_is_tx, int dt, void* stream);
int cn_nc_reduce_hxt(const void* h, const void* x, const void* ta, float* out, int n, int s, int c, float slope, int period,
                     int flags, int dt, void* stream);

int cn_act_fwd(const void* x, void* y, size_t numel, int act, float slope, int dt, void* stream);
int cn_act_bwd(const void* gy, const void* y, void* gx, size_t numel, int act, float slope, int dt, void* stream);
int cn_act_bwd_bias(const void* gy, const void* y, void* gx, float* gb, int n, int s, int c, int act, float slope, int flags,
                    int dt, void* stream);
int cn_axpby(const void* x, const void* y, void* out, size_t numel, float a, float b, int dt, void* stream);
int cn_mul(const void* x, const void* y, void* out, size_t numel, int dt, void* stream);
int cn_sqdiff_sum(const void* a, const void* b, float* out, size_t numel, float scale, int dt, void* stream);
int cn_row_sumsq(const float* x, float* out, int n, size_t row, void* stream);
int cn_row_scale(const void* x, const float* s, void* out, int n, size_t row, float k, int dt, void* stream);
int cn_row_scale_diff(const void* x, const void* x2, const float* s, void* out, int n, size_t row, float k, int dt, void* stream);
int cn_tap_bwd(const void* y, const void* target, const void* g, const float* s, void* out, int n, size_t row, float k,
               int act, float slope, int dt, void* stream);
int cn_maxpool2_bwd_act(const void* x, const void* gy, const void* target, const float* s, float k, void* gx, int n, int h,
                        int w, int c, int s_rows, int dt, void* stream);
int cn_stream_plan(int op, int dt, long long rows, size_t row, int c, int h, int w, int k, int s, int pad, unsigned aligned, int det,
                   long long out[4]);
int cn_stream_plan_ptrs(int op, int dt, int dst_dt, long long rows, size_t row, int c, int h, int w, int k, int s, int pad,
                        const void* const ptrs[4], int det, long long out[4]);
int cn_stream_last_plan(long long out[5]);
int cn_masked_diff(const float* a, const float* b, const uint8_t* mask, float* out, size_t pixels, int c, void* stream);
int cn_maxpool_fwd(const void* x, void* y, int n, int h, int w, int c, int k, int s, int pad, int dt, void* stream);
int cn_maxpool_bwd(const void* x, const void* gy, void* gx, int n, int h, int w, int c, int k, int s, int pad, int dt, void* stream);
int cn_avgpool3_same(const void* x, void* y, int n, int h, int w, int c, int dt, void* stream);
int cn_dwconv3x3_fwd(const float* x, const float* w, const float* bias, float* y, int n, int h, int wd, int c, int stride,
                     int act, float slope, void* stream);
int cn_image_preprocess(const void* x, int x_dt, float* y, int n, int h, int wd, int c, int oh, int ow, float in_mul, float in_add,
                        void* stream);
int cn_dwconv3x3_dgrad(const float* gy, const float* w, float* gx, int n, int h, int wd, int c, int stride, void* stream);
int cn_dwconv3x3_wgrad_slices(int n, int h, int wd, int c, int stride);
int cn_dwconv3x3_wgrad(const float* x, const float* gy, float* part, int slices, int n, int h, int wd, int c, int stride, void* stream);
int cn_bn_train_coef(const float* s1, const float* s2, const float* gamma, const float* beta, const float* x, float* mean, float* var,
                     float* r, float* a, float* b, float* moving_mean, float* moving_var, long long m, int c, float eps,
                     double momentum, int bessel, void* stream);
int cn_bn_train_apply(const float* x, const float* a, const float* b, float* y, long long m, int c, int act, void* stream);
int cn_bn_train_bwd_slices(long long m, int c);
int cn_chan_slices_plan(long long rows, int c, int min_rows, int out[5]);
int cn_bn_train_bwd_reduce(const float* gy, const float* y, const float* x, const float* mean, const float* r, float* part, int slices,
                           long long m, int c, int act, void* stream);
int cn_bn_train_bwd_apply(const float* gy, const float* y, const float* x, const float* mean, const float* r, const float* a,
                          const float* sums, float* gx, long long m, int c, int act, void* stream);
int cn_chan_affine3_fwd(const float* x, float* y, size_t pixels, const int* perm, float scale, const float* off, void* stream);
int cn_chan_affine3_bwd(const float* gy, float* gx, size_t pixels, const int* perm, float scale, void* stream);
int cn_gan_loss_fwd(const float* s, float* out, int n, float label, void* stream);
int cn_gan_loss_bwd(const float* s, const float* gout, float* gs, int n, float label, void* stream);

int cn_euler_matrix(const float* angles, float* rot, int n, void* stream);
int cn_euler_matrix_bwd(const float* angles, const float* grot, float* gangles, int n, void* stream);
int cn_rotate3d_fwd(const float* grid, const float* rot , float* out, int n, int g, int c, void* stream);
int cn_rotate3d_bwd(const float* grid, const float* rot, const float* gout, float* ggrid, float* grot,
                    int n, int g, int c, void* stream);
int cn_rotate3d_bwd_plan(int n, int g, int c, int det, int out[4]);

int cn_adam_step(float* theta, const float* grad, float* m, float* v, float* ema, size_t numel,
                 const float* lr_t, float beta1, float beta2, float eps, float ema_alpha, void* stream);
int cn_ema_step(float* ema, const float* theta, size_t numel, float alpha, void* stream);

int cn_gather_images_u8(const uint8_t* pool, const int64_t* idx, const uint8_t* flip, float* out,
                        int n, int h, int w, int c, void* stream);
int cn_to_uint8(const float* x, uint8_t* out, size_t numel, void* stream);
int cn_scale_columns_segments(const float* src, float* dst, const int* seg, const float* a, int nseg, size_t total, void* stream);
int cn_bn_fold_bwd_chunks(void);
int cn_bn_fold_bwd(const int* seg, int nseg, int blocks, const float* gwf, const float* gshift, const float* arena,
                   const float* a, const float* rs, const float* bm, float* gout, float* scratch, int ncols, void* stream);

int cn_hdri_rows_v(const float* x, float* v, const int* y0, const float* wy, int pool, int h, int w, int oh, int t_len,
                   void* stream);
int cn_hdri_rows_h(const float* v, float* out, const int* idx, const int* shift, const int* x0, const float* wx,
                   const float* mean, int n, int pool, int w, int oh, int ow, int t_len, void* stream);
int cn_exp2m1(const float* x, float* y, size_t numel, void* stream);

int cn_warp_affine_u8(const uint8_t* src, uint8_t* dst, const int* x0, const int* y0, const int* adelta, const int* bdelta,
                      int n, int sh, int sw, int c, int oh, int ow, void* stream);
int cn_warp_nearest_f32(const float* src, float* dst, const int* x0, const int* y0, const int* adelta, const int* bdelta,
                        int n, int sh, int sw, int c, int oh, int ow, void* stream);
int cn_eye_mask(const float* uv, uint8_t* mask, size_t pixels, int c, float l_min, float l_max, float r_min, float r_max,
                float y_min, float y_max, void* stream);

int cn_prof_enable(int on);
int cn_prof_reset(void);
int cn_prof_collect(int* launches, double* total_ms, double* total_flops);
int cn_prof_collect_by_family(int* launches, double* ms, double* flops, double* bytes);

int cn_spin(unsigned long long ticks, void* stream);

#ifdef __cplusplus
}
#endif
#endif
```

Baseline: 443.9 images/sec.

## Fuse ReLU backward mask and column sums into encoder conv dgrad epilogues

Adds mask epilogues to the fwd2 implicit-GEMM and Winograd dgrad kernels. They apply the ReLU derivative from the saved activation, optionally add the residual, and atomically accumulate per-channel gradient column sums. The real encoder backward now uses this fused path, so the separate relu_bwd/act_bwd_partials passes and their extra reads and writes of the data gradient go away. The cost is a second mask read inside the GEMM epilogue, non-deterministic atomics, and extra kernel variants that may fall back to the old path when unsupported.

```diff
diff --git a/confignet_amd/_lib.py b/confignet_amd/_lib.py
--- a/confignet_amd/_lib.py
+++ b/confignet_amd/_lib.py
@@ -62,6 +62,7 @@
     "cn_conv_dgrad": [_G, _p, _p, _p, _p],
     "cn_conv_dgrad_w": [_G, _p, _p, _p, _p],
     "cn_conv_dgrad_w_res": [_G, _p, _p, _p, _p, _p],
+    "cn_conv_dgrad_w_mask": [_G, _p, _p, _p, _p, _p, _p, _p, _p],
     "cn_bn_fold_bwd_chunks": [],
     "cn_bn_fold_bwd": [_p, _i, _i, _p, _p, _p, _p, _p, _p, _p, _p, _i, _p],
     "cn_conv_wgrad_thin_partials": [],
@@ -83,6 +84,7 @@
     "cn_gemm_rows_grouped_plan": [_p, _i, ctypes.POINTER(_i), _i, ctypes.POINTER(_i)],
     "cn_conv_tune": [_i, _i, ctypes.c_long],
     "cn_conv_fwd_plan": [_G, _i, _i, _i, _i, _i, _i, _i, ctypes.POINTER(ctypes.c_int * 8)],
+    "cn_conv_fwd_plan_ep": [_G, _i, _i, _i, _i, _i, _i, _i, _i, ctypes.POINTER(ctypes.c_int * 8)],
     "cn_conv_loop_select": [_i, _i, _i, _i],
     "cn_fwd2_col_block": [_i, _i, _i, _i, _i, _i],
     "cn_conv_fwd_dt": [_p, _p, _i, _p, _p, _p, _i, _i, _f, _p],
@@ -91,6 +93,7 @@
     "cn_conv_wgrad_c3": [_p, _p, _p, _i, _p, _p, _i, _p],
     "cn_conv_wino_filter": [_p, _p, _i, _i, _i, _p],
     "cn_conv_fwd_wino": [_i, _i, _i, _i, _i, _p, _p, _p, _p, _i, _f, _p],
+    "cn_conv_fwd_wino_ep": [_i, _i, _i, _i, _i, _p, _p, _p, _p, _p, _p, _p],
     "cn_conv_fwd_wino4": [_i, _i, _i, _i, _i, _p, _p, _p, _p, _i, _f, _p],
     "cn_conv_fwd_wino4_ep": [_i, _i, _i, _i, _i, _p, _p, _p, _p, _i, _f, _i, _p, _p, _p, _p, _i, _f, _p],
     "cn_conv_wino4_filter": [_p, _p, _i, _i, _i, _p],
diff --git a/confignet_amd/csrc/common.h b/confignet_amd/csrc/common.h
--- a/confignet_amd/csrc/common.h
+++ b/confignet_amd/csrc/common.h
@@ -41,7 +41,9 @@
 
 int cn_fwd2(const CnConvGeom* gp, int cfg, int bt, const float* A, const float* B, const float* bias, float* C, long M, int N, int K,
             int act, float slope, int splits, long part_stride, int par, hipStream_t s, const float* res, double x_elems, double w_elems,
-            float* stats = nullptr, int stats_mode = 0, float stats_slope = 0.f, int srows = 1, int sper = 1);
+            float* stats = nullptr, int stats_mode = 0, float stats_slope = 0.f, int srows = 1, int sper = 1, const float* mask = nullptr,
+            float* colsum = nullptr, float* colsum2 = nullptr);
+bool cn_fwd2_takes_mask(int cfg, int bt, int gathered, int n, int has_bias, int act, int has_stats);
 void cn_fwd2_tune(int kb, int ns, int np);
 void cn_fwd2_grid(int cfg, long M, int N, int par, int splits, int grid[3]);
 int cn_igemm_fwd(int cfg, const CnConvGeom& g, bool vec, int par, int splits, const float* x, const float* w, const float* bias, float* y,
diff --git a/confignet_amd/csrc/conv_dispatch.hip b/confignet_amd/csrc/conv_dispatch.hip
--- a/confignet_amd/csrc/conv_dispatch.hip
+++ b/confignet_amd/csrc/conv_dispatch.hip
@@ -17,7 +17,13 @@
 constexpr int g_fwd2_min_c = 48;
 
 struct ConvReq {
-    int bt, has_bias, act, has_res, stats_mode, x_dt, y_dt;
+    int bt, has_bias, act, has_res, stats_mode, x_dt, y_dt, has_mask = 0;
+};
+
+struct ConvEp {
+    const float* mask = nullptr;
+    float* colsum = nullptr;
+    float* colsum2 = nullptr;
 };
 
 struct ConvPlan {
@@ -49,7 +55,8 @@
 ConvPlan plan_conv_fwd(const CnConvGeom& g, const ConvReq& q) {
     ConvPlan p;
     const long M = (long)g.n * g.out_d * g.out_h * g.out_w;
-    const bool res = q.has_res != 0, stats = q.stats_mode != 0;
+    const bool mask = q.has_mask != 0;
+    const bool res = q.has_res != 0 || mask, stats = q.stats_mode != 0;
     const int bt = q.bt;
     auto small = [&p](int route, int family, long grid_x) {
         p.route = route;
@@ -67,7 +74,7 @@
                                                          : (long)g.n * cn_cdiv(g.out_h, 8) * cn_cdiv(g.out_w, 32);
     const int img_family = img == CN_ROUTE_C3 || img == CN_ROUTE_C7S2 ? CN_FAM_C3_FWD : CN_FAM_S2_IMAGE_DGRAD;
     if (q.x_dt != CN_F32 || q.y_dt != CN_F32)
-        return img != CN_ROUTE_UNSUPPORTED ? small(img, img_family, img_grid) : p;
+        return img != CN_ROUTE_UNSUPPORTED && !mask ? small(img, img_family, img_grid) : p;
     if ((res || stats) && (g.cout <= 4 || g.cin == 3 || g.cout % 4 != 0)) return p;
     if (stats && (bt || cn_det() || g.cin % BK != 0)) return p;
     if (bt && (g.cout <= 4 || g.cin % BK != 0 || g.cout % 4 != 0)) return p;
@@ -190,6 +197,10 @@
     }
     p.route = fwd2_takes && (cfg != 3 || n32) && cfg >= 0 && cfg <= 4 ? CN_ROUTE_FWD2 : CN_ROUTE_IGEMM;
     if (stats && p.route != CN_ROUTE_FWD2) return refuse(CN_EINVAL);
+    if (mask && p.route != CN_ROUTE_FWD2) {
+        p.route = CN_ROUTE_UNSUPPORTED;
+        return p;
+    }
     p.ret = CN_OK;
     p.cfg = cfg;
     p.splits = splits;
@@ -208,7 +219,7 @@
 }
 
 int run_conv_fwd(const ConvPlan& p, const CnConvGeom& g, const ConvReq& q, const void* x, const float* w, const float* bias,
-                 const float* res, void* y, float slope, float* stats, float stats_slope, hipStream_t s) {
+                 const float* res, void* y, float slope, float* stats, float stats_slope, hipStream_t s, const ConvEp& ep = ConvEp{}) {
     if (p.route == CN_ROUTE_UNSUPPORTED) return p.ret;
     const long M = (long)g.n * g.out_d * g.out_h * g.out_w;
     const int splits = p.splits;
@@ -223,13 +234,15 @@
     }
     const long part_stride = parts ? (long)M * g.cout : 0;
     float* const out = parts ? parts : (float*)y;
-    if (p.family >= 0) cn_prof_begin(s, conv_flops(g), conv_bytes(g, q.x_dt == CN_BF16 ? 2.0 : 4.0, q.y_dt == CN_BF16 ? 2.0 : 4.0), p.family);
+    const double ep_bytes = ep.mask ? 4.0 * (double)M * g.cout : 0.0;
+    if (p.family >= 0)
+        cn_prof_begin(s, conv_flops(g), conv_bytes(g, q.x_dt == CN_BF16 ? 2.0 : 4.0, q.y_dt == CN_BF16 ? 2.0 : 4.0) + ep_bytes, p.family);
     int e = CN_OK;
     switch (p.route) {
         case CN_ROUTE_FWD2: {
             const double xe = (double)g.n * g.in_d * g.in_h * g.in_w * g.cin, we = (double)g.k_d * g.k_h * g.k_w * g.cin * g.cout;
             e = cn_fwd2(p.plain ? nullptr : &g, p.cfg, q.bt, (const float*)x, w, bias, out, M, g.cout, g.cin, kact, slope, splits, part_stride,
-                        p.plain ? 0 : p.par, s, res, xe, we, stats, q.stats_mode, stats_slope, p.srows, p.sper);
+                        p.plain ? 0 : p.par, s, res, xe, we, stats, q.stats_mode, stats_slope, p.srows, p.sper, ep.mask, ep.colsum, ep.colsum2);
             break;
         }
         case CN_ROUTE_IGEMM:
@@ -318,11 +331,36 @@
     return conv_fwd(&d, ConvReq{1, 0, CN_ACT_NONE, 1, 0, CN_F32, CN_F32}, gy, w, nullptr, res, gu, 0.f, nullptr, 0.f, stream);
 }
 
+extern "C" int cn_conv_dgrad_w_mask(const CnConvGeom* gp, const float* gy, const float* w, const float* res, const float* mask, float* gu,
+                                    float* colsum, float* colsum2, void* stream) {
+    if (int e = check_geom(gp)) return e;
+    CN_CHECK_ARG(gy && w && mask && gu, "cn_conv_dgrad_w_mask: NULL tensor");
+    if (gp->dl_d != 1 || gp->dl_h != 1 || gp->dl_w != 1 || gp->up) return CN_EUNSUPPORTED;
+    if (gp->s_d != 1 || gp->s_h != 1 || gp->s_w != 1) return CN_EUNSUPPORTED;
+    if ((colsum || colsum2) && cn_det()) return CN_EUNSUPPORTED;
+    const CnConvGeom d = dgrad_geom(*gp);
+    const ConvReq q{1, 0, CN_ACT_NONE, res != nullptr, 0, CN_F32, CN_F32, 1};
+    const ConvPlan p = plan_conv_fwd(d, q);
+    if (p.route == CN_ROUTE_UNSUPPORTED) return p.ret;
+    if (p.splits > 1 || !cn_fwd2_takes_mask(p.cfg, 1, !p.plain, d.cout, 0, CN_ACT_NONE, 0)) return CN_EUNSUPPORTED;
+    return run_conv_fwd(p, d, q, gy, w, nullptr, res, gu, 0.f, nullptr, 0.f, (hipStream_t)stream, ConvEp{mask, colsum, colsum2});
+}
+
 extern "C" int cn_conv_fwd_plan(const CnConvGeom* gp, int bt, int has_bias, int act, int has_res, int stats_mode, int x_dt, int y_dt,
                                 int out[8]) {
     if (int e = check_geom(gp)) return e;
     CN_CHECK_ARG(out, "cn_conv_fwd_plan: out is NULL");
     const ConvPlan p = plan_conv_fwd(*gp, ConvReq{bt, has_bias, act, has_res, stats_mode, x_dt, y_dt});
+    const int v[8] = {p.route, p.cfg, p.splits, p.par, p.family, p.grid[0], p.grid[1], p.grid[2]};
+    for (int i = 0; i < 8; ++i) out[i] = v[i];
+    return p.ret;
+}
+
+extern "C" int cn_conv_fwd_plan_ep(const CnConvGeom* gp, int bt, int has_bias, int act, int has_res, int stats_mode, int has_mask, int x_dt,
+                                   int y_dt, int out[8]) {
+    if (int e = check_geom(gp)) return e;
+    CN_CHECK_ARG(out, "cn_conv_fwd_plan_ep: out is NULL");
+    const ConvPlan p = plan_conv_fwd(*gp, ConvReq{bt, has_bias, act, has_res, stats_mode, x_dt, y_dt, has_mask != 0});
     const int v[8] = {p.route, p.cfg, p.splits, p.par, p.family, p.grid[0], p.grid[1], p.grid[2]};
     for (int i = 0; i < 8; ++i) out[i] = v[i];
     return p.ret;
diff --git a/confignet_amd/csrc/fwd2.hip b/confignet_amd/csrc/fwd2.hip
--- a/confignet_amd/csrc/fwd2.hip
+++ b/confignet_amd/csrc/fwd2.hip
@@ -43,13 +43,16 @@
     f2_static_for_impl<0, N>(f);
 }
 
-template <int WM, int WN, int TM, int TN, bool BT, bool GATHER, int KB, int NS, int NP, bool BF, int CB = 32>
+template <int WM, int WN, int TM, int TN, bool BT, bool GATHER, int KB, int NS, int NP, bool BF, int CB = 32, bool MASK = false>
 __device__ __forceinline__ void fwd2_body(const CnConvGeom& g, const float* __restrict__ A, const float* __restrict__ B,
                                           const float* __restrict__ bias, float* __restrict__ C, int M, int N, int K,
                                           int act, float slope, int ntm, int ntn, long part_stride, int par,
                                           const float* __restrict__ res, unsigned a_bytes, unsigned b_bytes, int flip,
-                                          float* __restrict__ stats, int stats_mode, float stats_slope, int srows, int sper) {
+                                          float* __restrict__ stats, int stats_mode, float stats_slope, int srows, int sper,
+                                          const float* __restrict__ mask = nullptr, float* __restrict__ colsum = nullptr,
+                                          float* __restrict__ colsum2 = nullptr) {
     static_assert(!BF || BT, "bf16: both operands are K-contiguous rows");
+    static_assert(!MASK || (BT && !BF && CB == 32 && NP == 0), "mask epilogue: the fp32 B^T form on 32-wide blocks");
     constexpr int ES = BF ? 2 : 4;
     constexpr int KE = KB * 4 / ES;
     static_assert(WM * WN == 4, "4 waves per workgroup");
@@ -471,6 +474,55 @@
         }
         return;
     }
+    if constexpr (MASK) {
+        float csum[TN];
+#pragma unroll
+        for (int j = 0; j < TN; ++j) csum[j] = 0.f;
+#pragma unroll
+        for (int i = 0; i < TM; ++i)
+#pragma unroll
+            for (int j = 0; j < TN; ++j) {
+                const int col = n0 + wn * 32 * TN + 32 * j + l31;
+                long o[16];
+                float mk[16], rv[16];
+#pragma unroll
+                for (int r = 0; r < 16; ++r) {
+                    const int lrow = wm * 32 * TM + 32 * i + 4 * half + (r & 3) + 8 * (r >> 2);
+                    const int row = GATHER ? rowmap[lrow] : m0 + lrow;
+                    o[r] = (row >= 0 && row < M && col < N) ? (long)row * N + col : -1;
+                    const long oo = o[r] < 0 ? 0 : o[r];
+                    mk[r] = mask[oo];
+                    rv[r] = res ? res[oo] : 0.f;
+                }
+#pragma unroll
+                for (int r = 0; r < 16; ++r) {
+                    if (o[r] < 0) continue;
+                    const float v = acc[i][j][r] + 0.f;
+                    const float vr = res ? v + rv[r] : v;
+                    const float a = vr * act_deriv(mk[r], CN_ACT_RELU, 0.f);
+                    C[o[r]] = a;
+                    csum[j] += a;
+                }
+            }
+        if (colsum || colsum2) {
+            static_assert(WM * BN <= NS * (SA + SB) && BN <= 256, "the column sums fit the operand stages, a thread per column");
+            __syncthreads();
+#pragma unroll
+            for (int j = 0; j < TN; ++j) {
+                const float t = csum[j] + __shfl_xor(csum[j], 32);
+                if (half == 0) SM[wm * BN + wn * 32 * TN + 32 * j + l31] = t;
+            }
+            __syncthreads();
+            if (tid < BN && n0 + tid < N) {
+                float t = SM[tid];
+#pragma unroll
+                for (int w_ = 1; w_ < WM; ++w_) t += SM[w_ * BN + tid];
+                if (colsum) unsafeAtomicAdd(colsum + n0 + tid, t);
+                if (colsum2) unsafeAtomicAdd(colsum2 + n0 + tid, t);
+            }
+        }
+        return;
+    }
     const bool split = gridDim.z > 1;
     float sacc[TN][4];
 #pragma unroll
@@ -563,6 +615,16 @@
                                                             b_bytes, flip, nullptr, 0, 0.f, 1, 1);
 }
 
+template <int WM, int WN, int TM, int TN, bool GATHER>
+__global__ __launch_bounds__(256) void fwd2_mask_kernel(CnConvGeom g, const float* __restrict__ A, const float* __restrict__ B,
+                                                        float* __restrict__ C, int M, int N, int K, int ntm, int ntn, int par,
+                                                        const float* __restrict__ res, unsigned a_bytes, unsigned b_bytes,
+                                                        const float* __restrict__ mask, float* __restrict__ colsum,
+                                                        float* __restrict__ colsum2) {
+    fwd2_body<WM, WN, TM, TN, true, GATHER, 16, 4, 0, false, 32, true>(g, A, B, nullptr, C, M, N, K, CN_ACT_NONE, 0.f, ntm, ntn, 0, par, res,
+                                                                       a_bytes, b_bytes, 1, nullptr, 0, 0.f, 1, 1, mask, colsum, colsum2);
+}
+
 inline unsigned fwd2_grid_x(int ntm, int ntn, int par) { return (unsigned)(par ? ntm * ntn : 8 * cn_cdiv((long)ntm * ntn, 8)); }
 
 template <int NS>
@@ -589,6 +651,23 @@
     return CN_OK;
 }
 
+template <int WM, int WN, int TM, int TN>
+int launch2_mask(const CnConvGeom* gp, const float* A, const float* B, float* C, long M, int N, int K, int par, hipStream_t s, const float* res,
+                 unsigned a_bytes, unsigned b_bytes, const float* mask, float* colsum, float* colsum2) {
+    constexpr int BM = 32 * WM * TM, BN = 32 * WN * TN;
+    static const CnConvGeom none = {};
+    const int ntm = cn_cdiv(M, BM), ntn = cn_cdiv(N, BN);
+    const dim3 grid(fwd2_grid_x(ntm, ntn, gp ? par : 0));
+    if (gp)
+        hipLaunchKernelGGL((fwd2_mask_kernel<WM, WN, TM, TN, true>), grid, dim3(256), 0, s, *gp, A, B, C, (int)M, N, K, ntm, ntn, par, res, a_bytes,
+                           b_bytes, mask, colsum, colsum2);
+    else
+        hipLaunchKernelGGL((fwd2_mask_kernel<WM, WN, TM, TN, false>), grid, dim3(256), 0, s, none, A, B, C, (int)M, N, K, ntm, ntn, 0, res, a_bytes,
+                           b_bytes, mask, colsum, colsum2);
+    CN_LAUNCH_CHECK();
+    return CN_OK;
+}
+
 int g_fwd2_kb = 0;
 int g_fwd2_ns = 0;
 int g_fwd2_np = -1;
@@ -612,15 +691,28 @@
     return (cfg == 2 && bt && gathered && n == 48 && kb == 16 && np == 0) ? 16 : 32;
 }
 
+bool cn_fwd2_takes_mask(int cfg, int bt, int gathered, int n, int has_bias, int act, int has_stats) {
+    return bt && !has_bias && act == CN_ACT_NONE && !has_stats && (cfg == 2 || cfg == 3 || cfg == 4) &&
+           cn_fwd2_col_block(cfg, bt, gathered, n, 16, 0) == 32;
+}
+
 int cn_fwd2(const CnConvGeom* gp, int cfg, int bt, const float* A, const float* B, const float* bias, float* C, long M, int N, int K,
             int act, float slope, int splits, long part_stride, int par, hipStream_t s, const float* res, double x_elems, double w_elems,
-            float* stats, int stats_mode, float stats_slope, int srows, int sper) {
-    if ((res || stats) && (splits > 1 || part_stride)) return CN_EUNSUPPORTED;
+            float* stats, int stats_mode, float stats_slope, int srows, int sper, const float* mask, float* colsum, float* colsum2) {
+    if ((res || stats || mask) && (splits > 1 || part_stride)) return CN_EUNSUPPORTED;
     if (stats && bt) return CN_EUNSUPPORTED;
+    if ((colsum || colsum2) && !mask) return CN_EUNSUPPORTED;
+    if (mask && !cn_fwd2_takes_mask(cfg, bt, gp != nullptr, N, bias != nullptr, act, stats != nullptr)) return CN_EUNSUPPORTED;
     if (K % 16 != 0 || N % 4 != 0 || M <= 0 || M > 0x7fffffffL || (par && !gp)) return CN_EUNSUPPORTED;
     if (gp && (gp->dl_d > 2 || gp->dl_h > 2 || gp->dl_w > 2)) return CN_EUNSUPPORTED;
     if (x_elems * 4.0 >= 2147483647.0 || w_elems * 4.0 >= 2147483647.0) return CN_EUNSUPPORTED;
     const unsigned ab = (unsigned)(x_elems * 4.0), bb = (unsigned)(w_elems * 4.0);
+    if (mask) {
+        const int mpar = gp ? par : 0;
+        if (cfg == 2) return launch2_mask<2, 2, 1, 1>(gp, A, B, C, M, N, K, mpar, s, res, ab, bb, mask, colsum, colsum2);
+        if (cfg == 3) return launch2_mask<4, 1, 1, 1>(gp, A, B, C, M, N, K, mpar, s, res, ab, bb, mask, colsum, colsum2);
+        return launch2_mask<4, 1, 1, 3>(gp, A, B, C, M, N, K, mpar, s, res, ab, bb, mask, colsum, colsum2);
+    }
     static const CnConvGeom none = {};
     int kb = g_fwd2_kb ? g_fwd2_kb : 16;
     int ns = g_fwd2_ns ? g_fwd2_ns : 4;
diff --git a/confignet_amd/csrc/winograd.hip b/confignet_amd/csrc/winograd.hip
--- a/confignet_amd/csrc/winograd.hip
+++ b/confignet_amd/csrc/winograd.hip
@@ -42,8 +42,11 @@
     }
 }
 
+template <bool EP>
 __global__ __launch_bounds__(512, 1) void wino_fwd_kernel(WinoGeom g, const float* __restrict__ X, const float* __restrict__ U,
-                                                          const float* __restrict__ bias, float* __restrict__ Y, int act, float slope) {
+                                                          const float* __restrict__ bias, float* __restrict__ Y, int act, float slope,
+                                                          const float* __restrict__ mask, float* __restrict__ colsum,
+                                                          float* __restrict__ colsum2) {
     constexpr int BT = 64, BC = 64, LDV = BT + 4, LDU = BC;
     constexpr int RAW_SLOTS = 324, RAW_FLOATS = 12 * 64 * 4;
     extern __shared__ __attribute__((aligned(16))) float smem[];
@@ -199,9 +202,23 @@
             }
         }
     }
+    const int co = c0 + wc * 32 + l31;
+    float mk[EP ? 16 : 1][2];
+    if constexpr (EP) {
+#pragma unroll
+        for (int r = 0; r < 16; ++r) {
+            const int tl = wt * 32 + 4 * half + (r & 3) + 8 * (r >> 2);
+            const int base = tilebase[tl];
+            const int hw = tilehw[tl], oy = hw >> 16, ox = hw & 0xffff;
+            const bool in0 = base >= 0 && oy + ph < g.h, in1 = in0 && ox + 1 < g.w;
+            const long o = ((long)base + ph * g.w) * g.cout + co;
+            mk[r][0] = mask[in0 ? o : (long)co];
+            mk[r][1] = mask[in1 ? o + g.cout : (long)co];
+        }
+    }
     __syncthreads();
-    const int co = c0 + wc * 32 + l31;
     const float bv = bias ? bias[co] : 0.f;
+    float cs = 0.f;
 #pragma unroll
     for (int r = 0; r < 16; ++r) {
         const int tl = wt * 32 + 4 * half + (r & 3) + 8 * (r >> 2);
@@ -210,9 +227,34 @@
         const float y0 = keep[r][0] + xchg[(((ph ^ 1) * 16 + r) * 2 + 0) * 64 + lane];
         const float y1 = keep[r][1] + xchg[(((ph ^ 1) * 16 + r) * 2 + 1) * 64 + lane];
         if (base < 0 || oy + ph >= g.h) continue;
-        float* dst = Y + ((long)base + ph * g.w) * g.cout + co;
-        dst[0] = cn_apply_act(y0 + bv, act, slope);
-        if (ox + 1 < g.w) dst[g.cout] = cn_apply_act(y1 + bv, act, slope);
+        const long o = ((long)base + ph * g.w) * g.cout + co;
+        float* dst = Y + o;
+        if constexpr (EP) {
+            const float a0 = cn_apply_act(y0 + bv, act, slope) * act_deriv(mk[r][0], CN_ACT_RELU, 0.f);
+            dst[0] = a0;
+            cs += a0;
+            if (ox + 1 < g.w) {
+                const float a1 = cn_apply_act(y1 + bv, act, slope) * act_deriv(mk[r][1], CN_ACT_RELU, 0.f);
+                dst[g.cout] = a1;
+                cs += a1;
+            }
+        } else {
+            dst[0] = cn_apply_act(y0 + bv, act, slope);
+            if (ox + 1 < g.w) dst[g.cout] = cn_apply_act(y1 + bv, act, slope);
+        }
+    }
+    if constexpr (EP) {
+        if (colsum || colsum2) {
+            float* red = smem + 4 * 2 * 16 * 2 * 64;
+            const float t = cs + __shfl_xor(cs, 32);
+            if (half == 0) red[(ph * 2 + wt) * 64 + wc * 32 + l31] = t;
+            __syncthreads();
+            if (tid < 64) {
+                const float s_ = ((red[tid] + red[64 + tid]) + red[128 + tid]) + red[192 + tid];
+                if (colsum) unsafeAtomicAdd(colsum + c0 + tid, s_);
+                if (colsum2) unsafeAtomicAdd(colsum2 + c0 + tid, s_);
+            }
+        }
     }
 }
 
@@ -227,24 +269,43 @@
     return CN_OK;
 }
 
-extern "C" int cn_conv_fwd_wino(int n, int h, int w, int cin, int cout, const float* x, const float* u, const float* bias,
-                                float* y, int act, float slope, void* stream) {
-    CN_CHECK_ARG(x && u && y && n > 0 && h > 0 && w > 0, "conv_fwd_wino: bad args");
-    if (cin % (2 * WKB) || cout % 64) return CN_EUNSUPPORTED;
+namespace {
+
+template <bool EP>
+int wino_launch(int n, int h, int w, int cin, int cout, const float* x, const float* u, const float* bias, float* y, int act, float slope,
+                const float* mask, float* colsum, float* colsum2, void* stream) {
     CN_CHECK_ARG((double)n * h * w * (cin > cout ? cin : cout) * 4.0 < 2147483647.0 && 64.0 * cin * cout < 2147483647.0, "tensor exceeds 2^31 bytes (buffer descriptors, 32-bit offsets)");
     WinoGeom g{n, h, w, cin, cout, (h + 1) / 2, (w + 1) / 2, (h + 15) / 16, (w + 15) / 16};
     const long ntiles = (long)n * g.th * g.tw, nblk = (long)n * g.bh * g.bw;
     constexpr size_t lds = sizeof(float) * (2 * 16 * WKB * (68 + 64)) + sizeof(int) * 128;
     static bool attr_set = false;
     if (!attr_set) {
-        CN_HIP(hipFuncSetAttribute(reinterpret_cast<const void*>(wino_fwd_kernel), hipFuncAttributeMaxDynamicSharedMemorySize, (int)lds));
+        CN_HIP(hipFuncSetAttribute(reinterpret_cast<const void*>(wino_fwd_kernel<EP>), hipFuncAttributeMaxDynamicSharedMemorySize, (int)lds));
         attr_set = true;
     }
     hipStream_t s = (hipStream_t)stream;
     cn_prof_begin(s, 2.0 * 16.0 * (double)ntiles * cin * cout,
-                  4.0 * ((double)n * h * w * (cin + cout) + 16.0 * cin * cout), CN_FAM_WINO);
-    hipLaunchKernelGGL(wino_fwd_kernel, dim3((unsigned)(nblk * (cout / 64))), dim3(512), lds, s, g, x, u, bias, y, act, slope);
+                  4.0 * ((double)n * h * w * (cin + cout * (EP ? 2 : 1)) + 16.0 * cin * cout), CN_FAM_WINO);
+    hipLaunchKernelGGL(wino_fwd_kernel<EP>, dim3((unsigned)(nblk * (cout / 64))), dim3(512), lds, s, g, x, u, bias, y, act, slope, mask, colsum,
+                       colsum2);
     cn_prof_end(s);
     CN_LAUNCH_CHECK();
     return CN_OK;
 }
+
+}
+
+extern "C" int cn_conv_fwd_wino(int n, int h, int w, int cin, int cout, const float* x, const float* u, const float* bias,
+                                float* y, int act, float slope, void* stream) {
+    CN_CHECK_ARG(x && u && y && n > 0 && h > 0 && w > 0, "conv_fwd_wino: bad args");
+    if (cin % (2 * WKB) || cout % 64) return CN_EUNSUPPORTED;
+    return wino_launch<false>(n, h, w, cin, cout, x, u, bias, y, act, slope, nullptr, nullptr, nullptr, stream);
+}
+
+extern "C" int cn_conv_fwd_wino_ep(int n, int h, int w, int cin, int cout, const float* x, const float* u, float* y, const float* mask,
+                                   float* colsum, float* colsum2, void* stream) {
+    CN_CHECK_ARG(x && u && y && mask && n > 0 && h > 0 && w > 0, "conv_fwd_wino_ep: bad args");
+    if (cin % (2 * WKB) || cout % 64) return CN_EUNSUPPORTED;
+    if ((colsum || colsum2) && cn_det()) return CN_EUNSUPPORTED;
+    return wino_launch<true>(n, h, w, cin, cout, x, u, nullptr, y, CN_ACT_NONE, 0.f, mask, colsum, colsum2, stream);
+}
diff --git a/confignet_amd/dnn_models/real_encoder.py b/confignet_amd/dnn_models/real_encoder.py
--- a/confignet_amd/dnn_models/real_encoder.py
+++ b/confignet_amd/dnn_models/real_encoder.py
@@ -193,6 +193,7 @@
         return [w for w in self.weights[:-4] if w.requires_grad]
 
     folded_tape = True
+    fused_relu_bwd = True
 
     def _conv_bn(self, ci, x, coef, res=None, relu=True):
         kidx, _, spec = self._convs[ci]
@@ -340,24 +341,43 @@
             for bi in range(blocks_):
                 layout.append((ci, bi == 0))
                 ci += 4 if bi == 0 else 3
+        fused = enc.fused_relu_bwd
+
+        def dgrad_relu(gy_, ci_w, t_in_, y, cis, res=None):
+            sums = [gsh[offs[c]:offs[c + 1]] for c in cis if c is not None] if want_w else []
+            return ops.conv_dgrad_mask(gy_, wf[ci_w], geom(ci_w, t_in_), y, res=res, sums=sums, defer=sunk)
+
         pos = len(saved)
-        for first, has_sc in reversed(layout):
+        masked = False
+        for k in range(len(layout) - 1, -1, -1):
+            first, has_sc = layout[k]
             y1, y2, t_out = saved[pos - 3], saved[pos - 2], saved[pos - 1]
             pos -= 3
             t_in = saved[pos - 1]
             c1 = first + 1 if has_sc else first
-            gu3 = relu_bwd(c1 + 2, g, t_out, also=first if has_sc else None)
+            gu3 = g if masked else relu_bwd(c1 + 2, g, t_out, also=first if has_sc else None)
             wgrad(c1 + 2, y2, gu3)
-            gu2 = relu_bwd(c1 + 1, ops.conv_dgrad(gu3, wf[c1 + 2], geom(c1 + 2, y2)), y2)
+            if fused:
+                gu2 = dgrad_relu(gu3, c1 + 2, y2, y2, (c1 + 1,))
+            else:
+                gu2 = relu_bwd(c1 + 1, ops.conv_dgrad(gu3, wf[c1 + 2], geom(c1 + 2, y2)), y2)
             wgrad(c1 + 1, y1, gu2)
-            gu1 = relu_bwd(c1, ops.conv_dgrad(gu2, wf[c1 + 1], geom(c1 + 1, y1)), y1)
+            if fused:
+                gu1 = dgrad_relu(gu2, c1 + 1, y1, y1, (c1,))
+            else:
+                gu1 = relu_bwd(c1, ops.conv_dgrad(gu2, wf[c1 + 1], geom(c1 + 1, y1)), y1)
             wgrad(c1, t_in, gu1)
             if has_sc:
                 wgrad(first, t_in, gu3)
                 skip = ops.conv_dgrad(gu3, wf[first], geom(first, t_in))
             else:
                 skip = gu3
-            g = ops.conv_dgrad_res(gu1, wf[c1], geom(c1, t_in), skip)
+            masked = fused and k > 0
+            if masked:
+                pfirst, psc = layout[k - 1]
+                g = dgrad_relu(gu1, c1, t_in, t_in, ((pfirst + 1 if psc else pfirst) + 2, pfirst if psc else None), res=skip)
+            else:
+                g = ops.conv_dgrad_res(gu1, wf[c1], geom(c1, t_in), skip)
         x, y0, t = saved[0], saved[1], saved[2]
         g = ops.maxpool_bwd(y0, g, 3, 2, 1)
         gu0 = relu_bwd(0, g, y0)
diff --git a/confignet_amd/ops.py b/confignet_amd/ops.py
--- a/confignet_amd/ops.py
+++ b/confignet_amd/ops.py
@@ -502,6 +502,54 @@
     return nc_lin2(tuple(gu.shape), gu, None, res, None, None)
 
 
+MASK_EPILOGUE = True
+MASK_LOG = None
+
+
+def conv_dgrad_mask(gy, w, g, mask, res=None, sums=(), defer=True):
+    assert len(sums) <= 2
+    fused = None
+    if (MASK_EPILOGUE and not DETERMINISTIC and ACT_DTYPE == torch.float32 and gy.dtype == torch.float32 and mask.dtype == torch.float32
+            and (res is None or res.dtype == torch.float32) and DGRAD_FROM_W and not g.up and not _bf16_conv_ok(g)
+            and not _wino4_ok(g, g.cout, g.cin)):
+        gu = torch.empty(geom_in_shape(g, upsampled=True), device=gy.device, dtype=torch.float32)
+        assert tuple(gu.shape) == tuple(mask.shape), "conv_dgrad_mask: the mask has the shape of the data gradient"
+        s0 = _fptr(sums[0]) if len(sums) > 0 else None
+        s1 = _fptr(sums[1]) if len(sums) > 1 else None
+        if _wino_ok(g, g.cout, g.cin):
+            if res is None:
+                rc = lib.cn_conv_fwd_wino_ep(g.n, g.in_h, g.in_w, g.cout, g.cin, _ptr(_c(gy)), _ptr(_wino_filter(w, True)), _ptr(gu),
+                                             _ptr(_c(mask)), s0, s1, _stream())
+                fused = "wino"
+            else:
+                rc = CN_EUNSUPPORTED
+        else:
+            rc = lib.cn_conv_dgrad_w_mask(ctypes.byref(g), _ptr(_c(gy)), _fptr(_c(w)), None if res is None else _ptr(_c(res)),
+                                          _ptr(_c(mask)), _ptr(gu), s0, s1, _stream())
+            fused = "fwd2"
+        if rc == 0:
+            _log_mask(mask, ACT_RELU)
+            if sums and _SINK is not None:
+                _SINK.note_stream()
+            if fused == "wino":
+                prof_note_saved(wino_saved_flops(g))
+            if MASK_LOG is not None:
+                MASK_LOG.append(fused)
+            return gu
+        if rc != CN_EUNSUPPORTED:
+            check(rc, "cn_conv_fwd_wino_ep" if fused == "wino" else "cn_conv_dgrad_w_mask")
+        del gu
+    if MASK_LOG is not None:
+        MASK_LOG.append("pass")
+    gu = conv_dgrad(gy, w, g) if res is None else conv_dgrad_res(gy, w, g, res)
+    if not sums:
+        return act_bwd(gu, mask, ACT_RELU)
+    gu, part = act_bwd_partials(gu, mask, ACT_RELU)
+    for dst in sums:
+        sum_rows_into(part, dst, defer=defer)
+    return gu
+
+
 DGRAD_FROM_W = True
 MIXED_FIRST_LAYERS = True
 WGRAD_WRITE, WGRAD_ADD, WGRAD_ZEROED = 0, 1, 2
diff --git a/include/confignet_hip.h b/include/confignet_hip.h
--- a/include/confignet_hip.h
+++ b/include/confignet_hip.h
@@ -47,6 +47,8 @@
 int cn_conv_dgrad(const CnConvGeom* g, const float* gy, const float* w_tflip, float* gu, void* stream);
 int cn_conv_dgrad_w(const CnConvGeom* g, const float* gy, const float* w, float* gu, void* stream);
 int cn_conv_dgrad_w_res(const CnConvGeom* g, const float* gy, const float* w, const float* res, float* gu, void* stream);
+int cn_conv_dgrad_w_mask(const CnConvGeom* g, const float* gy, const float* w, const float* res, const float* mask, float* gu,
+                         float* colsum, float* colsum2, void* stream);
 int cn_conv_wgrad(const CnConvGeom* g, const float* x, const float* gy, float* gw, int accumulate, void* stream);
 size_t cn_conv_wgrad_workspace_bytes(const CnConvGeom* g);
 int cn_conv_wgrad_ws(const CnConvGeom* g, const float* x, const float* gy, float* gw, int accumulate, void* workspace,
@@ -109,6 +111,8 @@
 int cn_conv_wino_filter(const float* w, float* u, int cin, int cout, int dgrad, void* stream);
 int cn_conv_fwd_wino(int n, int h, int w, int cin, int cout, const float* x, const float* u, const float* bias, float* y,
                      int act, float slope, void* stream);
+int cn_conv_fwd_wino_ep(int n, int h, int w, int cin, int cout, const float* x, const float* u, float* y, const float* mask,
+                        float* colsum, float* colsum2, void* stream);
 int cn_conv_wino4_filter(const float* w, float* u, int cin, int cout, int dgrad, void* stream);
 int cn_conv_fwd_wino4(int n, int h, int w, int cin, int cout, const float* x, const float* u, const float* bias,
                       float* y, int act, float slope, void* stream);
@@ -120,6 +124,8 @@
                          int s_rows, float k, void* stream);
 int cn_conv_tune(int cfg, int splits, long wg_blocks);
 int cn_conv_fwd_plan(const CnConvGeom* g, int bt, int has_bias, int act, int has_res, int stats_mode, int x_dt, int y_dt, int out[8]);
+int cn_conv_fwd_plan_ep(const CnConvGeom* g, int bt, int has_bias, int act, int has_res, int stats_mode, int has_mask, int x_dt, int y_dt,
+                        int out[8]);
 int cn_conv_loop_select(int loop, int kb, int ns, int np);
 int cn_fwd2_col_block(int cfg, int bt, int gathered, int n, int kb, int np);
 int cn_sumpool2(const void* gu, void* gx, int nd, int n, int d, int h, int w, int c, int dt, void* stream);
```

Measured after the change: 451.1 images/sec (median of 6 runs). 1.6% higher.
